# OpenBMB/VisRAG

Hardware: AMD Instinct MI355X
Metric: page-images embedded/sec (VisRAG-Ret encode, 448x448, bf16 MFMA) + queries/sec@top-10 over 100k-page index (higher is better)
Workload: dtype bf16; 1 GPU; VisRAG-Ret (SigLIP-so400m 26 blk + resampler + MiniCPM-2B 40 layers) bf16 encode batch=32 page images 448x448 per GPU; index 100000 rows x 2304 sharded 1 way(s), 1000 queries top-10; batch_per_gpu=32, global_batch=32, parallelism=dp1 (pages sharded, no data-path collective)

## Files before the change

### visrag_amd/csrc/common.h

```cpp
#pragma once
#include <hip/hip_runtime.h>
#include <stdint.h>

typedef __bf16 bf16_t;
typedef __bf16 bf16x2 __attribute__((ext_vector_type(2)));
typedef __bf16 bf16x4 __attribute__((ext_vector_type(4)));
typedef __bf16 bf16x8 __attribute__((ext_vector_type(8)));
typedef float f32x2 __attribute__((ext_vector_type(2)));
typedef float f32x4 __attribute__((ext_vector_type(4)));
typedef uint32_t u32x4 __attribute__((ext_vector_type(4)));
typedef uint32_t u32x2 __attribute__((ext_vector_type(2)));

#define VR_WAVE 64

#define VR_LDS(p) ((__attribute__((address_space(3))) void*)(p))
#define VR_GLOBAL(p) ((const __attribute__((address_space(1))) void*)(p))

__device__ __forceinline__ float bf2f(bf16_t v) { return (float)v; }
__device__ __forceinline__ bf16_t f2bf(float v) { return (bf16_t)v; }

__device__ __forceinline__ float wave_sum(float v) {
#pragma unroll
    for (int o = 32; o > 0; o >>= 1) v += __shfl_xor(v, o, 64);
    return v;
}
__device__ __forceinline__ float wave_max(float v) {
#pragma unroll
    for (int o = 32; o > 0; o >>= 1) v = fmaxf(v, __shfl_xor(v, o, 64));
    return v;
}

__device__ __forceinline__ int xcd_remap(int bid, int nwg) {
    const int xcd = bid & 7, q = nwg >> 3, r = nwg & 7;
    const int base = (xcd < r) ? xcd * (q + 1) : r * (q + 1) + (xcd - r) * q;
    return base + (bid >> 3);
}

inline void set_max_dynamic_lds(const void* fn, int bytes, unsigned long long& done) {
    int dev = 0;
    if (hipGetDevice(&dev) != hipSuccess || dev < 0 || dev > 63) dev = 0;
    if (!((done >> dev) & 1ull)) {
        (void)hipFuncSetAttribute(fn, hipFuncAttributeMaxDynamicSharedMemorySize, bytes);
        done |= 1ull << dev;
    }
}
inline int device_cu_count() {
    static int cu_of[64] = {0};
    int dev = 0;
    if (hipGetDevice(&dev) != hipSuccess || dev < 0 || dev >= 64) dev = 0;
    if (!cu_of[dev]) {
        hipDeviceProp_t prop;
        cu_of[dev] = hipGetDeviceProperties(&prop, dev) == hipSuccess && prop.multiProcessorCount > 0 ? prop.multiProcessorCount : 256;
    }
    return cu_of[dev];
}
#define VR_WAIT_VM_BARRIER(N) asm volatile("s_waitcnt vmcnt(" #N ")\n\ts_barrier" ::: "memory")
```

### visrag_amd/csrc/encode.hip

```cpp
#include <hip/hip_runtime.h>

#include <algorithm>
#include <cmath>
#include <cstring>
#include <vector>

#include "model.h"

static int run_vision_group(vr_model_s* m, const uint8_t* const* dev_imgs_hostarray, int n, int H, int W,
                            const int32_t* rowmap_host , bool first_group, hipStream_t s) {
    const vr_config_t& c = m->c;
    const int P = c.patch_size, gh = H / P, gw = W / P, N = gh * gw;
    const int D = m->D, Dp = m->Dp, E = m->E, Q = m->Q;
    const int M = n * N;
    GridTables* g = nullptr;
    VRCHK(get_grid(m, gh, gw, &g));

    HIPCHK(hipMemcpyAsync(m->w_imgptr.p, dev_imgs_hostarray, (size_t)n * 8, hipMemcpyHostToDevice, s));
    int* cu = (int*)arena_take(m, (size_t)2 * (n + 1) * 4);
    for (int i = 0; i <= n; ++i) { cu[i] = i * N; cu[n + 1 + i] = i * Q; }
    HIPCHK(hipMemcpyAsync(m->w_cu.p, cu, (size_t)2 * (n + 1) * 4, hipMemcpyHostToDevice, s));
    HIPCHK(hipMemcpyAsync(m->w_rowmap.p, rowmap_host, (size_t)n * Q * 4, hipMemcpyHostToDevice, s));
    const int* cu_tok = m->w_cu.as<int>();
    const int* cu_qry = m->w_cu.as<int>() + (n + 1);

    float* h = m->w_hvit.as<float>();
    {
        GemmArgs a = gemm_args(nullptr, 0, m->patch, M, h, Dp);
        a.rowbias = g->vit_pos.as<float>(); a.rowbias_period = N; a.rowbias_ld = Dp; a.rowbias_cols = Dp;
        HIPCHK(launch_patch_embed((const uint8_t* const*)m->w_imgptr.p, n, H, W, P, a, m->Kpe, s));
    }
    if (first_group) VRCHK(tap_store(m, "vit_embed", h, N, D, Dp, false, s));
    const int ldqkv = pad128(3 * D);
    const int vit_hd = c.vit_dim / c.vit_heads;
    const int vit_qscale_n = D % 64 == 0 ? D : 0;
    const float vit_qscale = (1.0f / sqrtf((float)vit_hd)) * 1.44269504088896340736f;
    for (int l = 0; l < c.vit_depth; ++l) {
        const VitBlock& b = m->blocks[l];
        HIPCHK(launch_layernorm(h, M, D, Dp, b.n1w.v.as<float>(), b.n1b.v.as<float>(), c.vit_ln_eps, m->w_xn.p, Dp, s));
        VRCHK(prof_begin(m, VR_PROF_VIT_QKV, s));
        {
            GemmArgs a = gemm_args(m->w_xn.p, Dp, b.qkv, M, m->w_qkv.p, ldqkv);
            a.col_scale = vit_qscale; a.col_scale_n = vit_qscale_n;
            HIPCHK(launch_gemm(a, EPI_BF16, GEMM_VARIANT_AUTO, s));
        }
        VRCHK(prof_end(m, VR_PROF_VIT_QKV, 2.0 * M * D * 3 * D, s));
        {
            AttnArgs a{};
            a.q = m->w_qkv.p; a.ldq = ldqkv;
            a.k = (const char*)m->w_qkv.p + (size_t)D * 2; a.ldk = ldqkv;
            a.v = (const char*)m->w_qkv.p + (size_t)2 * D * 2; a.ldv = ldqkv;
            a.out = m->w_att.p; a.ldo = Dp; a.cu_q = cu_tok; a.cu_kv = cu_tok; a.B = n; a.heads = c.vit_heads;
            a.head_dim = vit_hd; a.max_q = N; a.causal = 0; a.q_shared = 0; a.scale = 1.0f / sqrtf((float)vit_hd); a.q_prescaled = vit_qscale_n > 0;
            VRCHK(prof_begin(m, VR_PROF_VIT_ATTN, s));
            HIPCHK(launch_attention(a, s));
            VRCHK(prof_end(m, VR_PROF_VIT_ATTN, 4.0 * n * (double)N * N * D, s));
        }
        VRCHK(prof_begin(m, VR_PROF_VIT_PROJ, s));
        {
            GemmArgs a = gemm_args(m->w_att.p, Dp, b.proj, M, h, Dp); a.resid = h;
            HIPCHK(launch_gemm(a, EPI_RESID, GEMM_VARIANT_AUTO, s));
        }
        VRCHK(prof_end(m, VR_PROF_VIT_PROJ, 2.0 * M * D * D, s));
        HIPCHK(launch_layernorm(h, M, D, Dp, b.n2w.v.as<float>(), b.n2b.v.as<float>(), c.vit_ln_eps, m->w_xn.p, Dp, s));
        VRCHK(prof_begin(m, VR_PROF_VIT_FC1, s));
        { GemmArgs a = gemm_args(m->w_xn.p, Dp, b.fc1, M, m->w_mlp.p, m->Fp); HIPCHK(launch_gemm(a, EPI_GELU, GEMM_VARIANT_AUTO, s)); }
        VRCHK(prof_end(m, VR_PROF_VIT_FC1, 2.0 * M * D * m->F, s));
        VRCHK(prof_begin(m, VR_PROF_VIT_FC2, s));
        {
            GemmArgs a = gemm_args(m->w_mlp.p, m->Fp, b.fc2, M, h, Dp); a.resid = h;
            HIPCHK(launch_gemm(a, EPI_RESID, GEMM_VARIANT_AUTO, s));
        }
        VRCHK(prof_end(m, VR_PROF_VIT_FC2, 2.0 * M * D * m->F, s));
        if (l == 0 && first_group) VRCHK(tap_store(m, "vit_block0", h, N, D, Dp, false, s));
    }
    HIPCHK(launch_layernorm(h, M, D, Dp, m->vit_nw.v.as<float>(), m->vit_nb.v.as<float>(), c.vit_ln_eps, m->w_xn.p, Dp, s));
    if (first_group) VRCHK(tap_store(m, "vit_out", m->w_xn.p, N, D, Dp, true, s));

    VRCHK(prof_begin(m, VR_PROF_RESAMPLER, s));
    { GemmArgs a = gemm_args(m->w_xn.p, Dp, m->r_kvproj, M, m->w_kv32.p, E); HIPCHK(launch_gemm(a, EPI_F32, GEMM_VARIANT_AUTO, s)); }
    HIPCHK(launch_layernorm(m->w_kv32.as<float>(), M, E, E, m->r_lnkv_w.v.as<float>(), m->r_lnkv_b.v.as<float>(),
                            c.resampler_ln_eps, m->w_xkv.p, E, s));
    {
        GemmArgs a = gemm_args(m->w_xkv.p, E, m->r_kv, M, m->w_KV.p, 2 * E);
        a.rowbias = g->pos_k.as<float>(); a.rowbias_period = N; a.rowbias_ld = E; a.rowbias_cols = E;
        HIPCHK(launch_gemm(a, EPI_BF16, GEMM_VARIANT_AUTO, s));
    }
    {
        AttnArgs a{};
        a.q = m->r_q.p; a.ldq = E; a.k = m->w_KV.p; a.ldk = 2 * E; a.v = (const char*)m->w_KV.p + (size_t)E * 2; a.ldv = 2 * E;
        a.out = m->w_ratt.p; a.ldo = E; a.cu_q = cu_qry; a.cu_kv = cu_tok; a.B = n; a.heads = E / 128; a.head_dim = 128;
        a.max_q = Q; a.causal = 0; a.q_shared = 1; a.scale = 1.0f / sqrtf(128.0f);
        HIPCHK(launch_attention(a, s));
    }
    const int R = n * Q;
    { GemmArgs a = gemm_args(m->w_ratt.p, E, m->r_out, R, m->w_rout.p, E); HIPCHK(launch_gemm(a, EPI_F32, GEMM_VARIANT_AUTO, s)); }
    HIPCHK(launch_layernorm(m->w_rout.as<float>(), R, E, E, m->r_lnpost_w.v.as<float>(), m->r_lnpost_b.v.as<float>(),
                            c.resampler_ln_eps, m->w_rln.p, E, s));
    if (first_group && m->taps_on) {
        GemmArgs a = gemm_args(m->w_rln.p, E, m->r_proj, Q, m->w_rout.p, E);
        HIPCHK(launch_gemm(a, EPI_F32, GEMM_VARIANT_AUTO, s));
        VRCHK(tap_store(m, "resampler_out", m->w_rout.p, Q, E, E, false, s));
    }
    {
        GemmArgs a = gemm_args(m->w_rln.p, E, m->r_proj, R, m->w_h.p, E);
        a.rowmap = m->w_rowmap.as<int>();
        HIPCHK(launch_gemm(a, EPI_F32, GEMM_VARIANT_AUTO, s));
    }
    VRCHK(prof_end(m, VR_PROF_RESAMPLER, 2.0 * M * D * E + 4.0 * M * E * (double)E + 4.0 * R * (double)N * E + 4.0 * R * E * (double)E, s));
    return VR_OK;
}

static int hp_gemm_tiles(vr_model_s* m, const void* a_hi, const void* a_lo, const Linear& L, const Linear& Llo, int lda, int T, float* out,
                         int ldo, bool into_resid, float alpha, hipStream_t s) {
    const size_t plane = (size_t)T * L.n_pad;
    const int n_planes = Llo.has_w ? 3 : 2;
    if (!L.has_b && (const char*)a_lo == (const char*)a_hi + (size_t)T * lda * 2 && m->w_hp_planes.reserve((size_t)n_planes * plane * 4) == VR_OK) {
        float* part = m->w_hp_planes.as<float>();
        {
            GemmArgs a = gemm_args(a_hi, lda, L, 2 * T, part, L.n_pad);
            a.bias = nullptr;
            HIPCHK(launch_gemm(a, EPI_F32, GEMM_VARIANT_AUTO, s));
        }
        if (Llo.has_w) {
            GemmArgs a = gemm_args(a_hi, lda, Llo, T, part + 2 * plane, L.n_pad);
            a.bias = nullptr;
            HIPCHK(launch_gemm(a, EPI_F32, GEMM_VARIANT_AUTO, s));
        }
        HIPCHK(launch_planes_sum(part, n_planes, plane, L.n_pad, T, std::min(L.n_pad, ldo), out, ldo, into_resid ? alpha : 1.0f, into_resid, s));
        return VR_OK;
    }
    {
        GemmArgs a = gemm_args(a_hi, lda, L, T, out, ldo);
        if (into_resid) { a.resid = out; a.alpha = alpha; }
        HIPCHK(launch_gemm(a, into_resid ? EPI_RESID : EPI_F32, GEMM_VARIANT_AUTO, s));
    }
    {
        GemmArgs a = gemm_args(a_lo, lda, L, T, out, ldo);
        a.bias = nullptr;
        a.resid = out; a.alpha = into_resid ? alpha : 1.0f;
        HIPCHK(launch_gemm(a, EPI_RESID, GEMM_VARIANT_AUTO, s));
    }
    if (Llo.has_w) {
        GemmArgs a = gemm_args(a_hi, lda, Llo, T, out, ldo);
        a.bias = nullptr;
        a.resid = out; a.alpha = into_resid ? alpha : 1.0f;
        HIPCHK(launch_gemm(a, EPI_RESID, GEMM_VARIANT_AUTO, s));
    }
    return VR_OK;
}

static int hp_gemm_stream(vr_model_s* m, const void* a_hi, const void* a_lo, const Linear& L, const Linear& Llo, int lda, int T, float* out,
                          int ldo, bool into_resid, float alpha, hipStream_t s) {
    const int ks = stream_ksplit(L.n_pad, L.k_pad);
    const size_t plane = (size_t)T * L.n_pad;
    const int n_pass = Llo.has_w ? 3 : 2;
    if ((size_t)n_pass * ks * plane * 4 > m->w_hp_part.bytes) return fail(VR_ERR_CAPACITY, "split-K planes exceed the workspace");
    float* part = m->w_hp_part.as<float>();
    for (int pass = 0; pass < n_pass; ++pass) {
        GemmArgs a = gemm_args(pass == 1 ? a_lo : a_hi, lda, pass == 2 ? Llo : L, T, part + (size_t)pass * ks * plane, L.n_pad);
        a.bias = nullptr;
        a.ksplit = ks; a.split_stride = plane;
        HIPCHK(launch_gemm_skinny(a, s));
    }
    HIPCHK(launch_planes_sum(part, n_pass * ks, plane, L.n_pad, T, std::min(L.n_pad, ldo), out, ldo, into_resid ? alpha : 1.0f, into_resid, s));
    return VR_OK;
}
static bool hp_stream_ok(const vr_model_s* m, int T) {
    if (T > 32) return false;
    for (const DecLayer& L : m->layers)
        for (const Linear* l : {&L.qkv, &L.o, &L.gu, &L.down})
            if (l->n_pad % 256 || l->k_pad % 64 || l->has_b) return false;
    return true;
}

static int run_decoder_hp(vr_model_s* m, int T, int B, int max_len, hipStream_t s) {
    (void)max_len;
    const vr_config_t& c = m->c;
    const int E = m->E, I = m->I, Ip = m->Ip;
    float* h = m->w_h.as<float>();
    float* qkv = m->w_hp_qkv.as<float>();
    float* att = m->w_hp_att.as<float>();
    float* gu = m->w_hp_gu.as<float>();
    const int ld_gu = pad128(2 * I);
    HIPCHK(launch_seq_of(m->w_seq.as<int>(), B, m->w_seqof.as<int>(), s));
    const bool stream = hp_stream_ok(m, T);
    void* const hi = m->w_hp_hi.p;
    auto lo = [&](int lda) -> void* { return (char*)hi + (size_t)T * lda * 2; };
    auto hp_gemm = [&](vr_model_s* mm, const Linear& L, const Linear& Llo, int lda, int TT, float* out, int ldo, bool into_resid,
                       float alpha, hipStream_t ss) -> int {
        return stream ? hp_gemm_stream(mm, hi, lo(lda), L, Llo, lda, TT, out, ldo, into_resid, alpha, ss)
                      : hp_gemm_tiles(mm, hi, lo(lda), L, Llo, lda, TT, out, ldo, into_resid, alpha, ss);
    };
    for (int l = 0; l < c.num_layers; ++l) {
        const DecLayer& L = m->layers[l];
        HIPCHK(launch_rmsnorm_split(h, T, E, L.ln1.v.as<float>(), c.rms_norm_eps, hi, lo(E), s));
        VRCHK(hp_gemm(m, L.qkv, L.qkv_lo, E, T, qkv, 3 * E, false, 1.0f, s));
        HIPCHK(launch_rope_f32(qkv, T, 3 * E, 2 * E, m->w_pos.as<int>(), m->rope.as<float>(), s));
        HIPCHK(launch_attn_f32(qkv, 3 * E, E, m->w_seqof.as<int>(), m->w_seq.as<int>(), T, c.num_heads, 1.0f / sqrtf(64.0f), att, s));
        HIPCHK(launch_split_bf16(att, hi, lo(E), (size_t)T * E, s));
        VRCHK(hp_gemm(m, L.o, L.o_lo, E, T, h, E, true, c.residual_scale, s));
        HIPCHK(launch_rmsnorm_split(h, T, E, L.ln2.v.as<float>(), c.rms_norm_eps, hi, lo(E), s));
        VRCHK(hp_gemm(m, L.gu, L.gu_lo, E, T, gu, ld_gu, false, 1.0f, s));
        HIPCHK(launch_swiglu_split(gu, T, ld_gu, I, Ip, hi, lo(Ip), s));
        VRCHK(hp_gemm(m, L.down, L.down_lo, Ip, T, h, E, true, c.residual_scale, s));
        if (l == 0) VRCHK(tap_store(m, "dec_layer0", h, T, E, E, false, s));
    }
    return VR_OK;
}


struct DecRoute { int ks; int proj_variant; bool proj_128w; };
static DecRoute dec_route(int T, int E, int Ip, bool taps_on) {
    DecRoute r{1, GEMM_VARIANT_256W, false};
    const long t192 = (long)((T + 255) / 256) * (E / 192);
    if (E % 192 == 0 && t192 * 2 <= 256 && t192 * 2 > 160 && E % 128 == 0 && Ip % 128 == 0) {
        r.ks = 2;
        r.proj_variant = GEMM_VARIANT_192W;
    } else {
        const long tiles = (long)((T + 255) / 256) * ((E + 255) / 256);
        for (int cand = DEC_KSPLIT_MAX; cand > 1; --cand)
            if (tiles * cand <= 256 && E % (cand * 64) == 0 && Ip % (cand * 64) == 0) { r.ks = cand; break; }
    }
    if (taps_on) r.ks = 1;
    const long t128 = (long)((T + 127) / 128) * (E / 192);
    r.proj_128w = E % 192 == 0 && t128 > 128 && t128 <= 256;
    if (r.proj_128w) r.ks = 1;
    return r;
}

extern "C" int vr_encode(vr_model_t m, const uint8_t* const* slices, const int32_t* slice_hw, int32_t n_slices,
                         int32_t slices_on_device, const int32_t* input_ids, const int32_t* seq_offsets, int32_t B,
                         const int32_t* vision_rows, float* out_reps, int32_t out_on_device, void* stream) {
    if (!m) return fail(VR_ERR_INVALID, "NULL model");
    m->arena_open = false;
    const int rc = encode_impl(m, slices, slice_hw, n_slices, slices_on_device, input_ids, seq_offsets, B, vision_rows,
                               out_reps, out_on_device, stream);
    arena_close(m, stream);
    return rc;
}

extern "C" int vr_encode_hidden(vr_model_t m, const uint8_t* const* slices, const int32_t* slice_hw, int32_t n_slices,
                                int32_t slices_on_device, const int32_t* input_ids, const int32_t* seq_offsets, int32_t B,
                                const int32_t* vision_rows, float* out_reps, int32_t out_on_device, float* out_hidden,
                                int32_t hidden_len, void* stream) {
    if (!m) return fail(VR_ERR_INVALID, "NULL model");
    if (!out_hidden || hidden_len <= 0) return fail(VR_ERR_INVALID, "out_hidden is NULL or hidden_len <= 0");
    m->arena_open = false;
    const int rc = encode_impl(m, slices, slice_hw, n_slices, slices_on_device, input_ids, seq_offsets, B, vision_rows,
                               out_reps, out_on_device, stream, out_hidden, hidden_len);
    arena_close(m, stream);
    return rc;
}

int encode_impl(vr_model_t m, const uint8_t* const* slices, const int32_t* slice_hw, int32_t n_slices,
                int32_t slices_on_device, const int32_t* input_ids, const int32_t* seq_offsets, int32_t B,
                const int32_t* vision_rows, float* out_reps, int32_t out_on_device, void* stream,
                float* out_hidden, int32_t hidden_len, const EncodeHook* hook) {
    if (!m->finalized) return fail(VR_ERR_STATE, "vr_model_finalize() has not succeeded");
    if (B <= 0 || !input_ids || !seq_offsets || !out_reps) return fail(VR_ERR_INVALID, "empty batch or NULL argument");
    if (n_slices > 0 && (!slices || !slice_hw || !vision_rows)) return fail(VR_ERR_INVALID, "NULL slice arguments");
    VRCHK(set_dev(m->device));
    hipStream_t s = (hipStream_t)stream;
    const vr_config_t& c = m->c;
    const int E = m->E, Q = m->Q;
    const int T = seq_offsets[B];
    if (seq_offsets[0] != 0) return fail(VR_ERR_INVALID, "seq_offsets[0] must be 0");
    if (B > c.max_seqs) return fail(VR_ERR_CAPACITY, "B=%d exceeds max_seqs=%d", B, c.max_seqs);
    if (T > c.max_tokens) return fail(VR_ERR_CAPACITY, "T=%d tokens exceed max_tokens=%d", T, c.max_tokens);
    for (int i = 0; i < B; ++i)
        if (seq_offsets[i + 1] <= seq_offsets[i]) return fail(VR_ERR_INVALID, "empty sequence %d", i);
    for (int t = 0; t < T; ++t)
        if (input_ids[t] < 0 || input_ids[t] >= c.vocab_size) return fail(VR_ERR_INVALID, "token id %d out of range at %d", input_ids[t], t);
    for (int i = 0; i < n_slices * Q; ++i)
        if (vision_rows[i] >= T) return fail(VR_ERR_INVALID, "vision row %d out of range", vision_rows[i]);

    VRCHK(arena_begin(m, (size_t)T * 4 + (size_t)(B + 1) * 4 + (size_t)n_slices * (Q * 4 + 8 + 64 * 3) + 4096));
    {
        int* a_ids = (int*)arena_take(m, (size_t)T * 4);
        int* a_seq = (int*)arena_take(m, (size_t)(B + 1) * 4);
        memcpy(a_ids, input_ids, (size_t)T * 4);
        memcpy(a_seq, seq_offsets, (size_t)(B + 1) * 4);
        HIPCHK(hipMemcpyAsync(m->w_ids.p, a_ids, (size_t)T * 4, hipMemcpyHostToDevice, s));
        HIPCHK(hipMemcpyAsync(m->w_seq.p, a_seq, (size_t)(B + 1) * 4, hipMemcpyHostToDevice, s));
    }
    int max_len = 0;
    for (int i = 0; i < B; ++i) max_len = std::max(max_len, seq_offsets[i + 1] - seq_offsets[i]);
    const bool hp = n_slices == 0 && c.text_split_precision != 0 && (c.text_split_precision == 1 || max_len <= c.text_split_precision) &&
                    !(hook && hook->bf16_route);
    if (hp && m->has_embed_lo)
        HIPCHK(launch_embed_gather_hp(m->w_ids.as<int>(), T, m->embed.p, m->embed_lo.p, E, c.scale_emb, m->w_h.as<float>(), s));
    else
        HIPCHK(launch_embed_gather(m->w_ids.as<int>(), T, m->embed.p, E, c.scale_emb, m->w_h.as<float>(), s));
    HIPCHK(launch_iota_pos(m->w_seq.as<int>(), B, m->w_pos.as<int>(), s));

    if (n_slices > 0) {
        size_t pix_total = 0;
        std::vector<size_t> pix_off(n_slices);
        for (int i = 0; i < n_slices; ++i) {
            const int H = slice_hw[2 * i], W = slice_hw[2 * i + 1];
            if (H <= 0 || W <= 0 || H % c.patch_size || W % c.patch_size)
                return fail(VR_ERR_INVALID, "slice %d: %dx%d is not a multiple of the patch size", i, H, W);
            if ((H / c.patch_size) * (W / c.patch_size) > c.max_patches)
                return fail(VR_ERR_CAPACITY, "slice %d has more than max_patches=%d patches", i, c.max_patches);
            pix_off[i] = pix_total;
            pix_total += ((size_t)H * W * 3 + 15) / 16 * 16;
        }
        std::vector<const uint8_t*> dev_ptr(n_slices);
        if (slices_on_device) {
            for (int i = 0; i < n_slices; ++i) dev_ptr[i] = slices[i];
        } else {
            if (m->w_pix.bytes < pix_total) VRCHK(m->w_pix.alloc(pix_total));
            for (int i = 0; i < n_slices; ++i) {
                const size_t nb = (size_t)slice_hw[2 * i] * slice_hw[2 * i + 1] * 3;
                HIPCHK(hipMemcpyAsync((char*)m->w_pix.p + pix_off[i], slices[i], nb, hipMemcpyHostToDevice, s));
                dev_ptr[i] = (const uint8_t*)m->w_pix.p + pix_off[i];
            }
        }
        std::vector<char> done(n_slices, 0);
        bool first = true;
        for (int i = 0; i < n_slices; ++i) {
            if (done[i]) continue;
            const int H = slice_hw[2 * i], W = slice_hw[2 * i + 1];
            const int N = (H / c.patch_size) * (W / c.patch_size);
            std::vector<int> idx;
            for (int j = i; j < n_slices; ++j)
                if (!done[j] && slice_hw[2 * j] == H && slice_hw[2 * j + 1] == W) { idx.push_back(j); done[j] = 1; }
            const int per_pass = std::max(1, (int)std::min<int64_t>(c.max_images, ((int64_t)c.max_images * c.max_patches) / N));
            for (size_t lo = 0; lo < idx.size(); lo += per_pass) {
                const int n = (int)std::min<size_t>(per_pass, idx.size() - lo);
                const uint8_t** ptrs = (const uint8_t**)arena_take(m, (size_t)n * 8);
                int32_t* rowmap = (int32_t*)arena_take(m, (size_t)n * Q * 4);
                for (int k = 0; k < n; ++k) {
                    ptrs[k] = dev_ptr[idx[lo + k]];
                    memcpy(rowmap + (size_t)k * Q, vision_rows + (size_t)idx[lo + k] * Q, (size_t)Q * 4);
                }
                VRCHK(run_vision_group(m, ptrs, n, H, W, rowmap, first, s));
                first = false;
            }
        }
    }
    VRCHK(tap_store(m, "inputs_embeds", m->w_h.p, T, E, E, false, s));

    float* h = m->w_h.as<float>();
    const int* seq = m->w_seq.as<int>();
    if (max_len > m->rope_len) return fail(VR_ERR_CAPACITY, "sequence of %d tokens exceeds the RoPE table", max_len);
    VRCHK(prof_begin(m, VR_PROF_DECODER, s));
    if (hp) {
        VRCHK(run_decoder_hp(m, T, B, max_len, s));
    } else {
    const DecRoute route = dec_route(T, E, m->Ip, m->taps_on);
    const int ks = route.ks;
    const size_t pstride = (size_t)T * E;
    float* part = m->w_part.as<float>();
    bool pend = false;
    auto proj = [&](const void* A, int lda, const Linear& L) -> int {
        if (route.proj_128w) {
            GemmArgs a = gemm_args(A, lda, L, T, h, E); a.resid = h; a.alpha = c.residual_scale;
            if (gemm128w_fits(a, 192)) { HIPCHK(launch_gemm(a, EPI_RESID, GEMM_VARIANT_128W_192, s)); return VR_OK; }
        }
        if (ks > 1) {
            GemmArgs a = gemm_args(A, lda, L, T, part, E);
            a.ksplit = ks; a.split_stride = pstride;
            HIPCHK(launch_gemm(a, EPI_F32, gemm256w_fits(a, route.proj_variant == GEMM_VARIANT_192W ? 192 : 256) ? route.proj_variant : GEMM_VARIANT_256IL, s));
            pend = true;
        } else {
            GemmArgs a = gemm_args(A, lda, L, T, h, E); a.resid = h; a.alpha = c.residual_scale;
            HIPCHK(launch_gemm(a, EPI_RESID, GEMM_VARIANT_AUTO, s));
        }
        return VR_OK;
    };
    auto norm = [&](const float* w) -> int {
        VRCHK(prof_begin(m, VR_PROF_DEC_NORM, s));
        struct End { vr_model_s* m; hipStream_t s; ~End() { (void)prof_end(m, VR_PROF_DEC_NORM, 0.0, s); } } end_{m, s};
        if (pend) {
            HIPCHK(launch_rmsnorm_accum(h, T, E, E, part, ks, pstride, E, c.residual_scale, w, c.rms_norm_eps, m->w_dxn.p, E, s));
            pend = false;
        } else {
            HIPCHK(launch_rmsnorm(h, T, E, E, w, c.rms_norm_eps, m->w_dxn.p, E, s));
        }
        return VR_OK;
    };
    double attn_flops = 0;
    for (int i = 0; i < B; ++i) { const double Li = seq_offsets[i + 1] - seq_offsets[i]; attn_flops += 4.0 * Li * Li * E; }
    for (int l = 0; l < c.num_layers; ++l) {
        const DecLayer& L = m->layers[l];
        VRCHK(norm(L.ln1.v.as<float>()));
        {
            GemmArgs a = gemm_args(m->w_dxn.p, E, L.qkv, T, m->w_dqkv.p, 3 * E);
            a.rope_pos = m->w_pos.as<int>(); a.rope_table = m->rope.as<float>(); a.rope_cols = 2 * E;
            VRCHK(prof_begin(m, VR_PROF_DEC_QKV, s));
            HIPCHK(launch_gemm(a, EPI_ROPE, GEMM_VARIANT_AUTO, s));
            VRCHK(prof_end(m, VR_PROF_DEC_QKV, 6.0 * T * (double)E * E, s));
        }
        if (hook && hook->layer) VRCHK(hook->layer(hook->ctx, l, m->w_dqkv.p, 3 * E, T, s));
        {
            VRCHK(prof_begin(m, VR_PROF_DEC_ATTN, s));
            AttnArgs a{};
            a.q = m->w_dqkv.p; a.ldq = 3 * E; a.k = (const char*)m->w_dqkv.p + (size_t)E * 2; a.ldk = 3 * E;
            a.v = (const char*)m->w_dqkv.p + (size_t)2 * E * 2; a.ldv = 3 * E;
            a.out = m->w_datt.p; a.ldo = E; a.cu_q = seq; a.cu_kv = seq; a.B = B; a.heads = c.num_heads; a.head_dim = 64;
            a.max_q = max_len; a.causal = 1; a.q_shared = 0; a.scale = 1.0f / sqrtf(64.0f);
            HIPCHK(launch_attention(a, s));
            VRCHK(prof_end(m, VR_PROF_DEC_ATTN, attn_flops, s));
        }
        VRCHK(prof_begin(m, VR_PROF_DEC_O, s));
        VRCHK(proj(m->w_datt.p, E, L.o));
        VRCHK(prof_end(m, VR_PROF_DEC_O, 2.0 * T * (double)E * E, s));
        VRCHK(norm(L.ln2.v.as<float>()));
        VRCHK(prof_begin(m, VR_PROF_DEC_GU, s));
        {
            GemmArgs a = gemm_args(m->w_dxn.p, E, L.gu, T, m->w_dact.p, m->Ip);
            HIPCHK(launch_gemm(a, EPI_SWIGLU, GEMM_VARIANT_AUTO, s));
        }
        VRCHK(prof_end(m, VR_PROF_DEC_GU, 4.0 * T * (double)E * m->I, s));
        VRCHK(prof_begin(m, VR_PROF_DEC_DOWN, s));
        VRCHK(proj(m->w_dact.p, m->Ip, L.down));
        VRCHK(prof_end(m, VR_PROF_DEC_DOWN, 2.0 * T * (double)E * m->I, s));
        if (l == 0) VRCHK(tap_store(m, "dec_layer0", h, T, E, E, false, s));
    }
    if (pend) {
        HIPCHK(launch_rmsnorm_accum(h, T, E, E, part, ks, pstride, E, c.residual_scale, nullptr, c.rms_norm_eps, nullptr, 0, s));
        pend = false;
    }
    }
    {
        double fl = 0;
        for (int i = 0; i < B; ++i) { const double Li = seq_offsets[i + 1] - seq_offsets[i]; fl += 4.0 * Li * Li * E; }
        fl = c.num_layers * (fl + (double)T * (8.0 * E * E + 6.0 * (double)E * m->I));
        VRCHK(prof_end(m, VR_PROF_DECODER, fl, s));
    }
    float* tap_hidden = nullptr;
    if (m->taps_on && (size_t)T * E * 4 <= m->w_kv32.bytes) tap_hidden = m->w_kv32.as<float>();
    if (out_hidden) {
        if (max_len > hidden_len) return fail(VR_ERR_INVALID, "hidden_len=%d is shorter than the longest sequence (%d)", hidden_len, max_len);
        if (!tap_hidden) {
            if ((size_t)T * E * 4 <= m->w_kv32.bytes) tap_hidden = m->w_kv32.as<float>();
            else { VRCHK(m->w_hidden.reserve((size_t)T * E * 4)); tap_hidden = m->w_hidden.as<float>(); }
        }
    }
    float* dst = out_on_device ? out_reps : m->w_out.as<float>();
    HIPCHK(launch_pool(h, seq, B, E, m->final_norm.v.as<float>(), c.rms_norm_eps, dst, tap_hidden, s, m->pool_mode));
    if (tap_hidden && m->taps_on) VRCHK(tap_store(m, "last_hidden", tap_hidden, T, E, E, false, s));
    if (out_hidden) {
        HIPCHK(hipMemsetAsync(out_hidden, 0, (size_t)B * hidden_len * E * 4, s));
        for (int i = 0; i < B; ++i)
            HIPCHK(hipMemcpyAsync(out_hidden + (size_t)i * hidden_len * E, tap_hidden + (size_t)seq_offsets[i] * E,
                                  (size_t)(seq_offsets[i + 1] - seq_offsets[i]) * E * 4, hipMemcpyDeviceToDevice, s));
    }
    if (!out_on_device) HIPCHK(hipMemcpyAsync(out_reps, dst, (size_t)B * E * 4, hipMemcpyDeviceToHost, s));
    if (!out_on_device || (n_slices > 0 && !slices_on_device)) HIPCHK(hipStreamSynchronize(s));
    return VR_OK;
}
```

### visrag_amd/csrc/engine_common.h

```cpp
#pragma once
#include <hip/hip_runtime.h>

#include <cstdarg>
#include <cstdio>
#include <initializer_list>
#include <string>
#include <vector>

#include "../../include/visrag_hip.h"
#include "kernels.h"
#include "pack.h"

using namespace vr;

inline thread_local std::string g_err;

static inline int fail(int code, const char* fmt, ...) {
    char buf[1024];
    va_list ap;
    va_start(ap, fmt);
    vsnprintf(buf, sizeof(buf), fmt, ap);
    va_end(ap);
    g_err = buf;
    return code;
}

#define HIPCHK(expr)                                                                         \
    do {                                                                                     \
        hipError_t e_ = (expr);                                                              \
        if (e_ != hipSuccess)                                                                \
            return fail(VR_ERR_HIP, "%s failed: %s (%s:%d)", #expr, hipGetErrorString(e_),   \
                        __FILE__, __LINE__);                                                 \
    } while (0)
#define VRCHK(expr)            \
    do {                       \
        int r_ = (expr);       \
        if (r_ != VR_OK) return r_; \
    } while (0)

static inline int skinny_ksplit(int n, int k, int max_split) {
    const int tiles = (n + 255) / 256, nk = k / 64;
    int best = 1;
    for (int d = 2; d <= max_split && tiles * d <= 256; ++d) {
        const int per = (nk + d - 1) / d;
        if (per >= 4 && (d - 1) * per < nk) best = d;
    }
    return best;
}
static inline int stream_ksplit(int n, int k) { return skinny_ksplit(n, k, 32); }

static inline int pad128(int x) { return (x + 127) / 128 * 128; }
static inline int64_t pad128l(int64_t x) { return (x + 127) / 128 * 128; }
static inline int pad256(int x) { return (x + 255) / 256 * 256; }
static inline int64_t pad256l(int64_t x) { return (x + 255) / 256 * 256; }

struct DevBuf {
    void* p = nullptr;
    size_t bytes = 0;
    bool owned = true;
    DevBuf() = default;
    DevBuf(const DevBuf& o) : p(o.p), bytes(o.bytes), owned(false) {}
    DevBuf& operator=(const DevBuf& o) {
        if (this != &o) { free(); p = o.p; bytes = o.bytes; owned = false; }
        return *this;
    }
    DevBuf(DevBuf&& o) noexcept : p(o.p), bytes(o.bytes), owned(o.owned) { o.p = nullptr; o.bytes = 0; o.owned = true; }
    DevBuf& operator=(DevBuf&& o) noexcept {
        if (this != &o) { free(); p = o.p; bytes = o.bytes; owned = o.owned; o.p = nullptr; o.bytes = 0; o.owned = true; }
        return *this;
    }
    ~DevBuf() { free(); }
    int alloc(size_t n) {
        free();
        if (n == 0) n = 16;
        hipError_t e = hipMalloc(&p, n);
        if (e != hipSuccess) { p = nullptr; return fail(VR_ERR_HIP, "hipMalloc(%zu) failed: %s", n, hipGetErrorString(e)); }
        bytes = n;
        e = hipMemset(p, 0, n);
        if (e != hipSuccess) return fail(VR_ERR_HIP, "hipMemset failed: %s", hipGetErrorString(e));
        e = hipStreamSynchronize(nullptr);
        if (e != hipSuccess) return fail(VR_ERR_HIP, "hipStreamSynchronize failed: %s", hipGetErrorString(e));
        return VR_OK;
    }
    int reserve(size_t n) {
        if (p && owned && bytes >= n) return VR_OK;
        free();
        if (n == 0) n = 16;
        hipError_t e = hipMalloc(&p, n);
        if (e != hipSuccess) { p = nullptr; return fail(VR_ERR_HIP, "hipMalloc(%zu) failed: %s", n, hipGetErrorString(e)); }
        bytes = n;
        return VR_OK;
    }
    void free() {
        if (p && owned) (void)hipFree(p);
        p = nullptr;
        bytes = 0;
        owned = true;
    }
    template <typename T> T* as() const { return reinterpret_cast<T*>(p); }
};

struct Linear {
    DevBuf w, b;
    int n = 0, k = 0, n_pad = 0, k_pad = 0;
    bool has_w = false, has_b = false;
};
struct Vec { DevBuf v; bool ok = false; };


static inline int set_dev(int dev) {
    HIPCHK(hipSetDevice(dev));
    return VR_OK;
}


struct Staged { const void* dev = nullptr; DevBuf tmp; };

static inline int stage(const void* data, size_t bytes, int on_device, Staged& st) {
    if (on_device) { st.dev = data; return VR_OK; }
    VRCHK(st.tmp.alloc(bytes));
    HIPCHK(hipMemcpy(st.tmp.p, data, bytes, hipMemcpyHostToDevice));
    st.dev = st.tmp.p;
    return VR_OK;
}

static inline int load_linear_part(Linear& L, int n_total, int k, const void* dev_src, int is_bf16, int rows, int src_ld,
                            int transpose, int blk, int blk_stride, int blk_off, int lo_part = 0) {
    if (!L.w.p) {
        L.n = n_total; L.k = k; L.n_pad = pad128(n_total); L.k_pad = pad128(k);
        VRCHK(L.w.alloc((size_t)pad256(n_total) * L.k_pad * 2));
    } else if (L.n != n_total || L.k != k) {
        return fail(VR_ERR_INVALID, "inconsistent shapes for a packed weight");
    }
    HIPCHK(launch_pack_weight(dev_src, is_bf16, rows, k, src_ld, transpose, L.w.p, L.k_pad, blk, blk_stride, blk_off, 0, lo_part));
    HIPCHK(hipDeviceSynchronize());
    L.has_w = true;
    return VR_OK;
}

static inline int load_bias_part(Linear& L, int n_total, const void* dev_src, int is_bf16, int rows, int off) {
    if (!L.b.p) VRCHK(L.b.alloc((size_t)pad256(n_total) * 4));
    HIPCHK(launch_to_f32(dev_src, is_bf16, L.b.as<float>() + off, rows, 0));
    HIPCHK(hipDeviceSynchronize());
    L.has_b = true;
    return VR_OK;
}

static inline int load_vec(Vec& v, const void* dev_src, int is_bf16, int n, int n_alloc) {
    VRCHK(v.v.alloc((size_t)n_alloc * 4));
    HIPCHK(launch_to_f32(dev_src, is_bf16, v.v.as<float>(), n, 0));
    HIPCHK(hipDeviceSynchronize());
    v.ok = true;
    return VR_OK;
}

static inline int to_host_f32(const void* dev_src, int is_bf16, size_t n, std::vector<float>& out) {
    DevBuf t;
    VRCHK(t.alloc(n * 4));
    HIPCHK(launch_to_f32(dev_src, is_bf16, t.as<float>(), n, 0));
    out.resize(n);
    HIPCHK(hipMemcpy(out.data(), t.p, n * 4, hipMemcpyDeviceToHost));
    t.free();
    return VR_OK;
}

static inline bool shape_is(const int64_t* s, int nd, std::initializer_list<int64_t> want) {
    if (nd != (int)want.size()) return false;
    int i = 0;
    for (int64_t w : want) if (s[i++] != w) return false;
    return true;
}
```

### visrag_amd/csrc/hp_text.hip

```cpp
#include "common.h"
#include "kernels.h"

namespace vr {

constexpr int HP_MAXV = 10;

__device__ __forceinline__ void split_store4(const f32x4 y, bf16_t* hi, bf16_t* lo) {
    bf16x4 h, l;
#pragma unroll
    for (int r = 0; r < 4; ++r) {
        h[r] = f2bf(y[r]);
        l[r] = f2bf(y[r] - bf2f(h[r]));
    }
    *reinterpret_cast<bf16x4*>(hi) = h;
    *reinterpret_cast<bf16x4*>(lo) = l;
}

__global__ __launch_bounds__(256) void rmsnorm_split_kernel(const float* __restrict__ x, int rows, int dim,
                                                            const float* __restrict__ w, float eps,
                                                            bf16_t* __restrict__ hi, bf16_t* __restrict__ lo) {
    const int lane = threadIdx.x & 63;
    const int row = blockIdx.x * 4 + (threadIdx.x >> 6);
    if (row >= rows) return;
    const int nv = dim >> 2;
    const f32x4* xr = reinterpret_cast<const f32x4*>(x + (size_t)row * dim);
    f32x4 v[HP_MAXV];
    float s = 0.f;
#pragma unroll
    for (int i = 0; i < HP_MAXV; ++i) {
        const int c = lane + i * 64;
        v[i] = (c < nv) ? xr[c] : f32x4{0.f, 0.f, 0.f, 0.f};
        s += v[i][0] * v[i][0] + v[i][1] * v[i][1] + v[i][2] * v[i][2] + v[i][3] * v[i][3];
    }
    s = wave_sum(s);
    const float rstd = rsqrtf(s / dim + eps);
#pragma unroll
    for (int i = 0; i < HP_MAXV; ++i) {
        const int c = lane + i * 64;
        if (c < nv) {
            const f32x4 y = v[i] * rstd * reinterpret_cast<const f32x4*>(w)[c];
            split_store4(y, hi + (size_t)row * dim + c * 4, lo + (size_t)row * dim + c * 4);
        }
    }
}

hipError_t launch_rmsnorm_split(const float* x, int rows, int dim, const float* w, float eps, void* hi, void* lo, hipStream_t s) {
    if (rows <= 0) return hipSuccess;
    if (dim % 4 || dim > 64 * 4 * HP_MAXV) return hipErrorInvalidValue;
    hipLaunchKernelGGL(rmsnorm_split_kernel, dim3((rows + 3) / 4), dim3(256), 0, s, x, rows, dim, w, eps, (bf16_t*)hi, (bf16_t*)lo);
    return hipGetLastError();
}

__global__ __launch_bounds__(256) void rope_f32_kernel(float* __restrict__ qkv, int T, int ld, int rope_cols,
                                                       const int* __restrict__ pos, const float* __restrict__ table) {
    const int t = blockIdx.x;
    const float* tab = table + (size_t)pos[t] * 64;
    float* row = qkv + (size_t)t * ld;
    for (int i = threadIdx.x; i < rope_cols / 2; i += 256) {
        const int head = i >> 5, c = i & 31;
        float* p = row + head * 64 + c;
        const float x1 = p[0], x2 = p[32], cs = tab[c], sn = tab[32 + c];
        p[0] = x1 * cs - x2 * sn;
        p[32] = x2 * cs + x1 * sn;
    }
}

hipError_t launch_rope_f32(float* qkv, int T, int ld, int rope_cols, const int* pos, const float* table, hipStream_t s) {
    if (T <= 0) return hipSuccess;
    if (rope_cols % 64) return hipErrorInvalidValue;
    hipLaunchKernelGGL(rope_f32_kernel, dim3(T), dim3(256), 0, s, qkv, T, ld, rope_cols, pos, table);
    return hipGetLastError();
}

__global__ __launch_bounds__(256) void attn_f32_kernel(const float* __restrict__ qkv, int ld, int E,
                                                       const int* __restrict__ seq_of, const int* __restrict__ seq_offsets,
                                                       int T, int heads, float scale, float* __restrict__ out) {
    const int lane = threadIdx.x & 63;
    const int w = blockIdx.x * 4 + (threadIdx.x >> 6);
    if (w >= T * heads) return;
    const int t = w / heads, h = w % heads;
    const int t0 = seq_offsets[seq_of[t]];
    const int n_keys = t - t0 + 1;
    const float* qrow = qkv + (size_t)t * ld + h * 64;
    f32x4 q[16];
#pragma unroll
    for (int i = 0; i < 16; ++i) q[i] = reinterpret_cast<const f32x4*>(qrow)[i];
    float m = -INFINITY, l = 0.f, acc = 0.f;
    for (int j0 = 0; j0 < n_keys; j0 += 64) {
        const int j = j0 + lane;
        float sc = -INFINITY;
        if (j < n_keys) {
            const f32x4* kr = reinterpret_cast<const f32x4*>(qkv + (size_t)(t0 + j) * ld + E + h * 64);
            float a = 0.f;
#pragma unroll
            for (int i = 0; i < 16; ++i) {
                const f32x4 kv = kr[i];
                a += q[i][0] * kv[0] + q[i][1] * kv[1] + q[i][2] * kv[2] + q[i][3] * kv[3];
            }
            sc = a * scale;
        }
        const float mn = fmaxf(m, wave_max(sc));
        const float p = (j < n_keys) ? expf(sc - mn) : 0.f;
        const float corr = expf(m - mn);
        l = l * corr + wave_sum(p);
        acc *= corr;
        const int nj = min(64, n_keys - j0);
        const float* vbase = qkv + (size_t)(t0 + j0) * ld + 2 * E + h * 64 + lane;
        for (int jj = 0; jj < nj; ++jj) acc += __shfl(p, jj, 64) * vbase[(size_t)jj * ld];
        m = mn;
    }
    out[(size_t)t * E + h * 64 + lane] = acc / l;
}

hipError_t launch_attn_f32(const float* qkv, int ld, int E, const int* seq_of, const int* seq_offsets, int T, int heads,
                           float scale, float* out, hipStream_t s) {
    if (T <= 0) return hipSuccess;
    if (E != heads * 64) return hipErrorInvalidValue;
    const long waves = (long)T * heads;
    hipLaunchKernelGGL(attn_f32_kernel, dim3((unsigned)((waves + 3) / 4)), dim3(256), 0, s, qkv, ld, E, seq_of, seq_offsets, T,
                       heads, scale, out);
    return hipGetLastError();
}

__global__ __launch_bounds__(256) void swiglu_split_kernel(const float* __restrict__ gu, int ld_gu, int I, int ld_act,
                                                           bf16_t* __restrict__ hi, bf16_t* __restrict__ lo) {
    const int t = blockIdx.x;
    const float* row = gu + (size_t)t * ld_gu;
    for (int c4 = threadIdx.x; c4 < ld_act / 4; c4 += 256) {
        const int c = c4 * 4;
        f32x4 y = {0.f, 0.f, 0.f, 0.f};
        if (c < I) {
            const int blk = c >> 4, o = c & 15;
            const f32x4 g = *reinterpret_cast<const f32x4*>(row + blk * 32 + o);
            const f32x4 u = *reinterpret_cast<const f32x4*>(row + blk * 32 + 16 + o);
#pragma unroll
            for (int r = 0; r < 4; ++r) y[r] = g[r] / (1.0f + expf(-g[r])) * u[r];
        }
        split_store4(y, hi + (size_t)t * ld_act + c, lo + (size_t)t * ld_act + c);
    }
}

hipError_t launch_swiglu_split(const float* gu, int T, int ld_gu, int I, int ld_act, void* hi, void* lo, hipStream_t s) {
    if (T <= 0) return hipSuccess;
    if (I % 16 || ld_act % 4 || ld_act < I) return hipErrorInvalidValue;
    hipLaunchKernelGGL(swiglu_split_kernel, dim3(T), dim3(256), 0, s, gu, ld_gu, I, ld_act, (bf16_t*)hi, (bf16_t*)lo);
    return hipGetLastError();
}

__global__ __launch_bounds__(256) void embed_gather_hp_kernel(const int* __restrict__ ids, const bf16_t* __restrict__ table_hi,
                                                              const bf16_t* __restrict__ table_lo, int dim, float scale,
                                                              float* __restrict__ out) {
    const int t = blockIdx.x;
    const size_t off = (size_t)ids[t] * dim;
    float* dst = out + (size_t)t * dim;
    for (int c = threadIdx.x * 4; c < dim; c += 1024) {
        const bf16x4 a = *reinterpret_cast<const bf16x4*>(table_hi + off + c);
        const bf16x4 b = *reinterpret_cast<const bf16x4*>(table_lo + off + c);
        f32x4 o;
#pragma unroll
        for (int r = 0; r < 4; ++r) o[r] = (bf2f(a[r]) + bf2f(b[r])) * scale;
        *reinterpret_cast<f32x4*>(dst + c) = o;
    }
}

hipError_t launch_embed_gather_hp(const int* ids, int T, const void* table_hi, const void* table_lo, int dim, float scale,
                                  float* out, hipStream_t s) {
    if (T <= 0) return hipSuccess;
    if (dim % 4) return hipErrorInvalidValue;
    hipLaunchKernelGGL(embed_gather_hp_kernel, dim3(T), dim3(256), 0, s, ids, (const bf16_t*)table_hi, (const bf16_t*)table_lo,
                       dim, scale, out);
    return hipGetLastError();
}

__global__ void seq_of_kernel(const int* __restrict__ seq_offsets, int* __restrict__ seq_of) {
    const int b = blockIdx.x;
    for (int t = seq_offsets[b] + threadIdx.x; t < seq_offsets[b + 1]; t += blockDim.x) seq_of[t] = b;
}

hipError_t launch_seq_of(const int* seq_offsets, int B, int* seq_of, hipStream_t s) {
    if (B <= 0) return hipSuccess;
    hipLaunchKernelGGL(seq_of_kernel, dim3(B), dim3(256), 0, s, seq_offsets, seq_of);
    return hipGetLastError();
}

__global__ __launch_bounds__(256) void planes_sum_kernel(const float* __restrict__ parts, int n_parts, size_t stride, int ldp, int N,
                                                         float* __restrict__ out, int ldo, float alpha, int accumulate) {
    const int t = blockIdx.y;
    const int n = (blockIdx.x * 256 + threadIdx.x) * 4;
    if (n >= N) return;
    const float* p0 = parts + (size_t)t * ldp + n;
    f32x4 a = *reinterpret_cast<const f32x4*>(p0);
    for (int p = 1; p < n_parts; ++p) a += *reinterpret_cast<const f32x4*>(p0 + (size_t)p * stride);
    float* o = out + (size_t)t * ldo + n;
    f32x4 r = a * alpha;
    if (accumulate) r += *reinterpret_cast<const f32x4*>(o);
    *reinterpret_cast<f32x4*>(o) = r;
}

hipError_t launch_planes_sum(const float* parts, int n_parts, size_t stride, int ldp, int T, int N, float* out, int ldo, float alpha,
                             bool accumulate, hipStream_t s) {
    if (T <= 0 || n_parts <= 0) return hipSuccess;
    if (N % 4 || ldp % 4 || ldo % 4) return hipErrorInvalidValue;
    hipLaunchKernelGGL(planes_sum_kernel, dim3((N / 4 + 255) / 256, T), dim3(256), 0, s, parts, n_parts, stride, ldp, N, out, ldo, alpha,
                       accumulate ? 1 : 0);
    return hipGetLastError();
}

}
```

### visrag_amd/csrc/index.hip

```cpp
#include <hip/hip_runtime.h>

#include <algorithm>
#include <cmath>
#include <vector>

#include "engine_common.h"

constexpr int CERT_WORDS = 32, CERT_FLAG = 2, CERT_FLAG2 = 3, CERT_STATS = 4, CERT_NSTATS = 6;
struct vr_index_s {
    int device = 0, dim = 0;
    int64_t cap = 0, n = 0;
    DevBuf f32, bf16;
    DevBuf q32, qbf, cs, ci, ck, os, oi, ok, thr, sbuf;
    int64_t qcap = 0, ccap = 0, kcap = 0;
    DevBuf cert, flags, flagq;
    int64_t fcap = 0;
    int* huge_seen = nullptr;
    float eps_rel = -2.f;
    bool prof_on = false;
    hipEvent_t prof_ev[SEARCH_PROF_EVENTS] = {};
    double prof_ms[SEARCH_PROF_EVENTS - 1] = {};
    int64_t prof_calls = 0;
};

extern "C" int vr_index_create(int device_id, int32_t dim, int64_t capacity, vr_index_t* out) {
    if (!out || dim <= 0 || capacity <= 0) return fail(VR_ERR_INVALID, "bad index arguments");
    if (dim % 64 || dim > 2560) return fail(VR_ERR_INVALID, "dim %d must be a multiple of 64 and <= 2560", dim);
    if (capacity >= ((int64_t)1 << 31) - 256) return fail(VR_ERR_INVALID, "capacity too large for 32-bit row ids");
    VRCHK(set_dev(device_id));
    vr_index_s* ix = new vr_index_s();
    ix->device = device_id; ix->dim = dim; ix->cap = capacity;
    const int64_t cp = pad256l(capacity);
    int r = ix->f32.alloc((size_t)cp * dim * 4);
    if (r == VR_OK) r = ix->bf16.alloc((size_t)cp * dim * 2);
    if (r == VR_OK) r = ix->cert.alloc(CERT_WORDS * 4);
    if (r == VR_OK && hipHostMalloc((void**)&ix->huge_seen, 64, hipHostMallocDefault) != hipSuccess) r = fail(VR_ERR_HIP, "hipHostMalloc");
    if (r != VR_OK) { ix->f32.free(); ix->bf16.free(); ix->cert.free(); delete ix; return r; }
    *ix->huge_seen = 0;
    *out = ix;
    return VR_OK;
}

extern "C" int vr_index_destroy(vr_index_t ix) {
    if (!ix) return VR_OK;
    (void)hipSetDevice(ix->device);
    (void)hipDeviceSynchronize();
    for (DevBuf* b : {&ix->f32, &ix->bf16, &ix->q32, &ix->qbf, &ix->cs, &ix->ci, &ix->ck, &ix->os, &ix->oi, &ix->ok, &ix->thr,
                      &ix->sbuf, &ix->cert, &ix->flags, &ix->flagq})
        b->free();
    for (hipEvent_t e : ix->prof_ev) if (e) (void)hipEventDestroy(e);
    if (ix->huge_seen) (void)hipHostFree(ix->huge_seen);
    delete ix;
    return VR_OK;
}

extern "C" int vr_index_reset(vr_index_t ix) {
    if (!ix) return fail(VR_ERR_INVALID, "NULL index");
    VRCHK(set_dev(ix->device));
    HIPCHK(hipDeviceSynchronize());
    HIPCHK(hipMemset(ix->cert.p, 0, 8));
    ix->n = 0;
    if (ix->huge_seen) *ix->huge_seen = 0;
    return VR_OK;
}

extern "C" int vr_index_size(vr_index_t ix, int64_t* n) {
    if (!ix || !n) return fail(VR_ERR_INVALID, "NULL argument");
    *n = ix->n;
    return VR_OK;
}

extern "C" int vr_index_add(vr_index_t ix, const float* reps, int64_t n, int32_t on_device, void* stream) {
    if (!ix || (!reps && n > 0) || n < 0) return fail(VR_ERR_INVALID, "bad arguments");
    if (n == 0) return VR_OK;
    if (ix->n + n > ix->cap) return fail(VR_ERR_CAPACITY, "index capacity %lld exceeded", (long long)ix->cap);
    VRCHK(set_dev(ix->device));
    hipStream_t s = (hipStream_t)stream;
    float* dst = ix->f32.as<float>() + (size_t)ix->n * ix->dim;
    HIPCHK(hipMemcpyAsync(dst, reps, (size_t)n * ix->dim * 4, on_device ? hipMemcpyDeviceToDevice : hipMemcpyHostToDevice, s));
    HIPCHK(launch_f32_to_bf16(dst, (char*)ix->bf16.p + (size_t)ix->n * ix->dim * 2, (size_t)n * ix->dim, s));
    HIPCHK(launch_row_norm_max(dst, n, ix->dim, ix->cert.as<float>(), s));
    if (!on_device) HIPCHK(hipStreamSynchronize(s));
    ix->n += n;
    return VR_OK;
}

extern "C" int vr_index_set_search_eps(vr_index_t ix, float eps_rel) {
    if (!ix) return fail(VR_ERR_INVALID, "NULL index");
    if (eps_rel != eps_rel) ix->eps_rel = -2.f;
    else ix->eps_rel = eps_rel < 0.f ? -1.f : eps_rel;
    return VR_OK;
}

extern "C" int vr_index_search_stats(vr_index_t ix, int64_t* out6, int32_t reset) {
    if (!ix || !out6) return fail(VR_ERR_INVALID, "NULL argument");
    VRCHK(set_dev(ix->device));
    HIPCHK(hipDeviceSynchronize());
    unsigned w[CERT_NSTATS];
    HIPCHK(hipMemcpy(w, ix->cert.as<unsigned>() + CERT_STATS, CERT_NSTATS * 4, hipMemcpyDeviceToHost));
    for (int i = 0; i < CERT_NSTATS; ++i) out6[i] = w[i];
    if (reset) HIPCHK(hipMemset(ix->cert.as<unsigned>() + CERT_STATS, 0, CERT_NSTATS * 4));
    return VR_OK;
}

struct SearchPlan { bool stream; int own, sweep, n_chunks, tiles_per_chunk; };
static SearchPlan search_plan(int64_t n_docs, int nq, int dim) {
    SearchPlan p{};
    p.stream = search_uses_stream(nq, dim);
    p.own = p.stream ? 0 : search_prepass_owned(n_docs, nq, dim);
    p.sweep = p.stream ? search_stream_chunks() : search_num_chunks(n_docs - (p.own ? (int64_t)SEARCH_PRE_SPOTS * 256 : 0), nq);
    p.n_chunks = p.sweep + p.own;
    const int64_t tile = search_uses_256(nq) ? 256 : 128;
    const int64_t tiles = (n_docs + tile - 1) / tile - (p.own ? SEARCH_PRE_SPOTS : 0);
    p.tiles_per_chunk = p.stream ? 0 : (int)((tiles + p.sweep - 1) / p.sweep);
    return p;
}

extern "C" int vr_index_search_plan(vr_index_t ix, int32_t nq, int32_t* out5) {
    if (!ix || !out5 || nq <= 0) return fail(VR_ERR_INVALID, "bad arguments");
    const SearchPlan p = search_plan(ix->n, nq, ix->dim);
    out5[0] = p.n_chunks; out5[1] = p.own; out5[2] = p.sweep; out5[3] = p.tiles_per_chunk;
    out5[4] = (ix->huge_seen && __atomic_load_n(ix->huge_seen, __ATOMIC_RELAXED) != 0) ? 1 : 0;
    return VR_OK;
}

extern "C" int vr_index_error_model(vr_index_t ix, float* out4) {
    if (!ix || !out4) return fail(VR_ERR_INVALID, "NULL argument");
    VRCHK(set_dev(ix->device));
    HIPCHK(hipDeviceSynchronize());
    HIPCHK(hipMemcpy(out4, ix->cert.p, 8, hipMemcpyDeviceToHost));
    out4[2] = search_acc_rel(ix->dim);
    out4[3] = search_default_eps_rel(ix->dim);
    return VR_OK;
}

extern "C" int vr_index_set_search_profile(vr_index_t ix, int32_t enable) {
    if (!ix) return fail(VR_ERR_INVALID, "NULL index");
    VRCHK(set_dev(ix->device));
    if (enable)
        for (hipEvent_t& e : ix->prof_ev) if (!e) HIPCHK(hipEventCreate(&e));
    ix->prof_on = enable != 0;
    for (double& m : ix->prof_ms) m = 0;
    ix->prof_calls = 0;
    return VR_OK;
}

extern "C" int vr_index_get_search_profile(vr_index_t ix, double* ms5, int64_t* calls) {
    if (!ix || !ms5 || !calls) return fail(VR_ERR_INVALID, "NULL argument");
    for (int i = 0; i < SEARCH_PROF_EVENTS - 1; ++i) ms5[i] = ix->prof_ms[i];
    *calls = ix->prof_calls;
    return VR_OK;
}

static int search_impl(vr_index_t ix, const float* queries, int32_t nq, int32_t k, float* out_scores, int64_t* out_ids,
                       unsigned long long* out_keys, int64_t id_offset, int32_t on_device, void* stream) {
    const bool keys_out = out_keys != nullptr;
    if (!ix || !queries || nq <= 0 || (!keys_out && (!out_scores || !out_ids))) return fail(VR_ERR_INVALID, "bad arguments");
    const bool bigk = k > 26;
    if (k <= 0 || k > search_bigk_max()) return fail(VR_ERR_INVALID, "k=%d unsupported (1..%d)", k, search_bigk_max());
    if (keys_out && (id_offset < 0 || id_offset + ix->n >= ((int64_t)1 << 32) - 1))
        return fail(VR_ERR_INVALID, "id_offset %lld + %lld rows do not fit 32-bit global ids", (long long)id_offset, (long long)ix->n);
    const int kp = bigk ? 0 : search_kprime(k);
    VRCHK(set_dev(ix->device));
    hipStream_t s = (hipStream_t)stream;
    const int dim = ix->dim;
    const int64_t ldS = pad256l(std::max<int64_t>(ix->n, 1));
    int64_t qblk = bigk ? 256 : 4096;
    const int64_t nqp = pad256l(std::min<int64_t>(nq, qblk));
    const int64_t slots = bigk ? 256 : std::min<int64_t>(nqp, std::max<int64_t>(16, (((int64_t)1 << 27) / ldS) / 16 * 16));
    if (ix->qcap < nqp) {
        VRCHK(ix->qbf.alloc((size_t)nqp * dim * 2));
        VRCHK(ix->thr.alloc((size_t)nqp * 8));
        ix->qcap = nqp;
    }
    const float* q32 = queries;
    if (!on_device) {
        VRCHK(ix->q32.reserve((size_t)nq * dim * 4));
        HIPCHK(hipMemcpyAsync(ix->q32.p, queries, (size_t)nq * dim * 4, hipMemcpyHostToDevice, s));
        q32 = ix->q32.as<float>();
    }
    float* os = out_scores; int64_t* oi = out_ids; unsigned long long* ok = out_keys;
    if (!on_device) {
        if (keys_out) { VRCHK(ix->ok.reserve((size_t)nq * k * 8)); ok = ix->ok.as<unsigned long long>(); }
        else {
            VRCHK(ix->os.reserve((size_t)nq * k * 4));
            VRCHK(ix->oi.reserve((size_t)nq * k * 8));
            os = ix->os.as<float>(); oi = ix->oi.as<int64_t>();
        }
    }
    if (ix->n == 0) {
        if (keys_out) HIPCHK(hipMemsetAsync(ok, 0, (size_t)nq * k * 8, s));
        else {
            std::vector<float> sc((size_t)nq * k, -INFINITY);
            std::vector<int64_t> id((size_t)nq * k, -1);
            HIPCHK(hipMemcpyAsync(os, sc.data(), sc.size() * 4, hipMemcpyHostToDevice, s));
            HIPCHK(hipMemcpyAsync(oi, id.data(), id.size() * 8, hipMemcpyHostToDevice, s));
            HIPCHK(hipStreamSynchronize(s));
        }
    } else {
        if (ix->fcap < nqp) {
            VRCHK(ix->flags.alloc((size_t)nqp * 12));
            VRCHK(ix->flagq.alloc((size_t)(nqp + 256) * dim * 2));
            ix->fcap = nqp;
        }
        VRCHK(ix->sbuf.reserve((size_t)slots * ldS * 4));
        for (int64_t q0 = 0; q0 < nq; q0 += qblk) {
            const int nb = (int)std::min<int64_t>(qblk, nq - q0);
            const int64_t nbp = pad256l(nb);
            const bool prof = ix->prof_on && !bigk;
            if (prof) HIPCHK(hipEventRecord(ix->prof_ev[0], s));
            const bool conv_in_kernel = !bigk && search_uses_stream(nb, dim);
            if (!conv_in_kernel)
                HIPCHK(launch_f32_to_bf16_pad(q32 + (size_t)q0 * dim, ix->qbf.p, (size_t)nb * dim, (size_t)nbp * dim, s,
                                              ix->cert.as<int>() + CERT_FLAG));
            if (prof) HIPCHK(hipEventRecord(ix->prof_ev[1], s));
            SearchArgs a{};
            a.index_bf16 = ix->bf16.p; a.index_f32 = ix->f32.as<float>(); a.n_docs = ix->n; a.dim = dim;
            a.q_bf16 = ix->qbf.p; a.q_f32 = q32 + (size_t)q0 * dim; a.nq = nb; a.k = k;
            a.convert_q = conv_in_kernel ? 1 : 0;
            if (conv_in_kernel) { a.score_rows = ix->sbuf.as<float>(); a.ld_scores = (size_t)ldS; }
            const bool huge_seen = ix->huge_seen && __atomic_load_n(ix->huge_seen, __ATOMIC_RELAXED) != 0;
            const bool exact_small = conv_in_kernel && huge_seen;
            const bool exact_big = !conv_in_kernel && (bigk || huge_seen || !ix->huge_seen);
            a.exact_follows = (exact_small || exact_big) ? 1 : 0;
            a.huge_seen = ix->huge_seen;
            a.eps_data = ix->eps_rel == -2.f ? 1 : 0;
            a.eps_rel = a.eps_data ? 0.f : ix->eps_rel;
            a.acc_rel = search_acc_rel(dim);
            a.dmax = ix->cert.as<float>();
            a.flag_count = ix->cert.as<int>() + CERT_FLAG; a.flag_list = ix->flags.as<int>();
            a.flag2_count = ix->cert.as<int>() + CERT_FLAG2; a.flag2_list = ix->flags.as<int>() + ix->fcap;
            a.flag_tau = ix->flags.as<float>() + 2 * ix->fcap; a.flag_q = ix->flagq.p;
            a.stats = ix->cert.as<unsigned>() + CERT_STATS;
            if (keys_out) { a.out_keys = ok + (size_t)q0 * k; a.id_offset = id_offset; }
            else { a.out_scores = os + (size_t)q0 * k; a.out_ids = oi + (size_t)q0 * k; }
            a.prof_ev = prof ? ix->prof_ev : nullptr;
            if (bigk) {
                GemmArgs g{};
                g.A = ix->qbf.p; g.lda = dim;
                g.W = ix->bf16.p; g.ldw = dim; g.M = nb; g.N = (int)pad128l(ix->n); g.K = dim;
                g.out = ix->sbuf.p; g.ldo = (int)ldS; g.alpha = 1.0f;
                HIPCHK(launch_gemm(g, EPI_F32, GEMM_VARIANT_AUTO, s));
                HIPCHK(launch_search_bigk(a, ix->sbuf.as<float>(), (size_t)ldS, 0, nb, s));
            } else {
                const SearchPlan plan = search_plan(ix->n, nb, dim);
                a.pre_own_chunks = plan.own;
                a.n_chunks = plan.n_chunks;
                a.thr_init = ix->thr.as<float>();
                a.thr_cert = ix->thr.as<float>() + ix->qcap;
                const int64_t need = std::max<int64_t>(nbp * a.n_chunks * kp, nbp * search_prepass_floats());
                if (ix->ccap < need) {
                    VRCHK(ix->cs.alloc((size_t)need * 4));
                    VRCHK(ix->ci.alloc((size_t)need * 4));
                    ix->ccap = need;
                }
                a.cand_scores = ix->cs.as<float>(); a.cand_ids = ix->ci.as<int>();
                if (search_uses_256(nb)) {
                    const int64_t kneed = nbp * a.n_chunks * 128;
                    if (ix->kcap < kneed) { VRCHK(ix->ck.alloc((size_t)kneed * 8)); ix->kcap = kneed; }
                    a.cand_keys = ix->ck.as<unsigned long long>();
                }
                HIPCHK(launch_search(a, s));
            }
            if (prof) HIPCHK(hipEventRecord(ix->prof_ev[4], s));
            if ((a.eps_data || a.eps_rel >= 0.f) && !a.score_rows) {
                for (int64_t f0 = 0; f0 < nb; f0 += slots) {
                    const int ns = (int)std::min<int64_t>(slots, nb - f0);
                    GemmArgs g{};
                    g.A = (const char*)ix->flagq.p + (size_t)f0 * dim * 2; g.lda = dim;
                    g.W = ix->bf16.p; g.ldw = dim; g.M = ns; g.N = (int)pad128l(ix->n); g.K = dim;
                    g.out = ix->sbuf.p; g.ldo = (int)ldS; g.alpha = 1.0f;
                    g.m_dev = a.flag_count; g.m_sub = (int)f0;
                    HIPCHK(launch_gemm(g, EPI_F32, GEMM_VARIANT_256IL, s));
                    HIPCHK(launch_band_select(a, ix->sbuf.as<float>(), (size_t)ldS, (int)f0, ns, s));
                }
                SearchArgs ax = a;
                ax.flag_count = a.flag2_count; ax.flag_list = a.flag2_list;
                for (int64_t f0 = 0; exact_big && f0 < nb; f0 += slots) {
                    const int ns = (int)std::min<int64_t>(slots, nb - f0);
                    HIPCHK(launch_exact_scores(a.index_f32, a.n_docs, dim, a.q_f32, ax.flag_list, ax.flag_count, (int)f0, ns,
                                               ix->sbuf.as<float>(), (size_t)ldS, s));
                    HIPCHK(launch_exact_select(ax, ix->sbuf.as<float>(), (size_t)ldS, (int)f0, ns, s));
                }
            }
            if ((a.eps_data || a.eps_rel >= 0.f) && a.score_rows && exact_small) {
                SearchArgs ax = a;
                ax.flag_count = a.flag2_count; ax.flag_list = a.flag2_list;
                HIPCHK(launch_exact_scores(a.index_f32, a.n_docs, dim, a.q_f32, ax.flag_list, ax.flag_count, 0, nb, ix->sbuf.as<float>(), (size_t)ldS, s));
                HIPCHK(launch_exact_select(ax, ix->sbuf.as<float>(), (size_t)ldS, 0, nb, s));
            }
            if (prof) {
                HIPCHK(hipEventRecord(ix->prof_ev[5], s));
                HIPCHK(hipEventSynchronize(ix->prof_ev[5]));
                for (int i = 0; i + 1 < SEARCH_PROF_EVENTS; ++i) {
                    float ms = 0.f;
                    HIPCHK(hipEventElapsedTime(&ms, ix->prof_ev[i], ix->prof_ev[i + 1]));
                    ix->prof_ms[i] += ms;
                }
                ix->prof_calls += 1;
            }
        }
    }
    if (!on_device) {
        if (keys_out) HIPCHK(hipMemcpyAsync(out_keys, ok, (size_t)nq * k * 8, hipMemcpyDeviceToHost, s));
        else {
            HIPCHK(hipMemcpyAsync(out_scores, os, (size_t)nq * k * 4, hipMemcpyDeviceToHost, s));
            HIPCHK(hipMemcpyAsync(out_ids, oi, (size_t)nq * k * 8, hipMemcpyDeviceToHost, s));
        }
        HIPCHK(hipStreamSynchronize(s));
    }
    return VR_OK;
}

extern "C" int vr_index_search(vr_index_t ix, const float* queries, int32_t nq, int32_t k, float* out_scores,
                               int64_t* out_ids, int32_t on_device, void* stream) {
    return search_impl(ix, queries, nq, k, out_scores, out_ids, nullptr, 0, on_device, stream);
}

extern "C" int vr_index_search_keys(vr_index_t ix, const float* queries, int32_t nq, int32_t k, int64_t id_offset,
                                    uint64_t* out_keys, int32_t on_device, void* stream) {
    if (!out_keys) return fail(VR_ERR_INVALID, "out_keys is NULL");
    return search_impl(ix, queries, nq, k, nullptr, nullptr, (unsigned long long*)out_keys, id_offset, on_device, stream);
}

extern "C" int vr_topk_merge(int device_id, const float* scores, const int64_t* ids, int32_t n_parts, int32_t nq,
                             int32_t k, float* out_scores, int64_t* out_ids, void* stream) {
    if (!scores || !ids || !out_scores || !out_ids || n_parts <= 0 || nq <= 0) return fail(VR_ERR_INVALID, "bad arguments");
    VRCHK(set_dev(device_id));
    HIPCHK(launch_topk_merge(scores, ids, n_parts, nq, k, out_scores, out_ids, (hipStream_t)stream));
    return VR_OK;
}

extern "C" int vr_topk_merge_keys(int device_id, const uint64_t* keys, int32_t n_parts, int32_t nq, int32_t k,
                                  float* out_scores, int64_t* out_ids, void* stream) {
    if (!keys || !out_scores || !out_ids || n_parts <= 0 || nq <= 0) return fail(VR_ERR_INVALID, "bad arguments");
    VRCHK(set_dev(device_id));
    HIPCHK(launch_topk_merge_keys((const unsigned long long*)keys, n_parts, nq, k, out_scores, out_ids, (hipStream_t)stream));
    return VR_OK;
}
```

### visrag_amd/csrc/kernels.h

```cpp
#pragma once
#include <hip/hip_runtime.h>
#include <stdint.h>

namespace vr {

enum GemmEpilogue { EPI_BF16 = 0, EPI_GELU = 1, EPI_F32 = 2, EPI_RESID = 3, EPI_SWIGLU = 4, EPI_ROPE = 5 };
enum GemmVariant { GEMM_VARIANT_GLDS = 0, GEMM_VARIANT_AUTO = 3, GEMM_VARIANT_192 = 7, GEMM_VARIANT_256IL = 9, GEMM_VARIANT_256W = 12,
                   GEMM_VARIANT_192W = 13, GEMM_VARIANT_128W_192 = 14, GEMM_VARIANT_128W_256 = 15 };

struct GemmArgs {
    const void* A; int lda;
    const void* W; int ldw;
    int M, N, K;
    const float* bias;
    const float* resid;
    float alpha;
    void* out; int ldo;
    const int* rowmap;
    const float* rowbias;
    int rowbias_period, rowbias_ld, rowbias_cols;
    const int* rope_pos;
    const float* rope_table;
    int rope_cols;
    int raster_gm;
    int ksplit;
    size_t split_stride;
    float col_scale; int col_scale_n;
    const int* m_dev; int m_sub;
};
hipError_t launch_gemm(const GemmArgs& a, int epilogue, int variant, hipStream_t s);
hipError_t launch_gemm192(const GemmArgs& a, int epilogue, hipStream_t s);
hipError_t launch_gemm256w(const GemmArgs& a, int epilogue, hipStream_t s);
bool gemm256w_fits(const GemmArgs& a, int tile_cols);
hipError_t launch_gemm192w(const GemmArgs& a, int epilogue, hipStream_t s);
hipError_t launch_gemm128w(const GemmArgs& a, int epilogue, int tile_cols, hipStream_t s);
bool gemm128w_fits(const GemmArgs& a, int tile_cols);

struct SkinnyCombine { const void* part; const float* lse; int S; int heads; int group; const int* S_dev; };
hipError_t launch_gemm_skinny(const GemmArgs& a, hipStream_t s, bool swiglu = false, const struct SkinnyCombine* combine = nullptr);
hipError_t launch_swiglu_sum(const float* parts, int n_parts, size_t plane_stride, int ldp, int M, int I, void* act, int lda,
                             hipStream_t s);

hipError_t launch_layernorm(const float* x, int rows, int dim, int ldx, const float* w, const float* b,
                            float eps, void* out, int ldo, hipStream_t s);
hipError_t launch_rmsnorm_accum(float* x, int rows, int dim, int ldx, const float* partial, int nsplit,
                                size_t split_stride, int ldp, float alpha, const float* w, float eps, void* out,
                                int ldo, hipStream_t s);
hipError_t launch_rmsnorm(const float* x, int rows, int dim, int ldx, const float* w, float eps,
                          void* out, int ldo, hipStream_t s);

struct AttnArgs {
    const void* q; int ldq;
    const void* k; int ldk;
    const void* v; int ldv;
    void* out; int ldo;
    const int* cu_q;
    const int* cu_kv;
    int B, heads, head_dim, max_q;
    int causal, q_shared;
    float scale;
    int kv_group;
    const int* kv_end;
    const int* q_in_rows;
    int q_head_stride;
    int q_prescaled;
    float* lse;
};
hipError_t launch_attention(const AttnArgs& a, hipStream_t s);

constexpr int CHAT_MAX_ROWS = 16;
constexpr int CHAT_ATT_SPLITS = 8;
constexpr int CHAT_KEYS = 256;
constexpr int CHAT_SEL_WGS = 64;
constexpr int CHAT_TOPK_MAX = 64;
enum ChatSelMode { CHAT_SEL_GREEDY = 0, CHAT_SEL_BEAM = 1, CHAT_SEL_SAMPLE = 2 };
struct ChatStep {
    int n, groups;
    int row[CHAT_MAX_ROWS], slot[CHAT_MAX_ROWS], tail[CHAT_MAX_ROWS], pos[CHAT_MAX_ROWS], token[CHAT_MAX_ROWS];
    int g_lo[CHAT_MAX_ROWS + 1], plen[CHAT_MAX_ROWS];
    int gsplit[CHAT_MAX_ROWS], rsplit[CHAT_MAX_ROWS];
};
struct ChatCaps { int slots, len, rows, tail; };
struct ChatMove { int n; int src[CHAT_MAX_ROWS], dst[CHAT_MAX_ROWS], len[CHAT_MAX_ROWS]; };
struct ChatSel {
    int n, groups;
    int lrow[CHAT_MAX_ROWS], srow[CHAT_MAX_ROWS], g_lo[CHAT_MAX_ROWS + 1];
    float bscore[CHAT_MAX_ROWS];
};
hipError_t launch_chat_embed(const ChatStep& st, const void* table, int E, float scale, float* h, unsigned* seen, int words, hipStream_t s);
hipError_t launch_chat_qkv(const ChatStep& st, const float* parts, int n_parts, size_t plane, int ldp, const float* rope, int E, int heads,
                           void* q_out, void* tails, int l, int max_rows, int max_new, hipStream_t s);
hipError_t launch_chat_attn(const ChatStep& st, const void* q, const void* prompt, const void* tails, int l, int E, int heads,
                            const ChatCaps& cap, int S_max, float* po, float* pml, void* att, hipStream_t s);
hipError_t launch_chat_prompt_kv(const void* qkv, int ld, int T, int E, void* kdst, void* vdst, hipStream_t s);
hipError_t launch_chat_move(const ChatMove& mv, void* tails, void* scratch, int layers, int max_rows, int max_new, int E, int max_tail,
                            unsigned* seen, unsigned* seen_scratch, int words, hipStream_t s);
hipError_t launch_chat_select(const ChatSel& sel, int mode, const float* logits, int ld, int V, const unsigned* seen, int words, float pen,
                              float temperature, int K, int kout, unsigned long long seed, unsigned step, float* lse,
                              unsigned long long* part, float* o_score, int* o_tok, int* o_par, hipStream_t s);

constexpr int GEN_ATT_SPLITS = 16;
struct GenState {
    int token;
    int pos[3];
    int len;
    int step;
    int splits;
    int pad;
    int cu_q[GEN_ATT_SPLITS + 1], cu_kv[GEN_ATT_SPLITS + 1];
};
struct GenBatch {
    int token[16];
    int pos[3][16];
    int cache_row[16];
    int splits[16];
    int cu_q[16 * GEN_ATT_SPLITS + 1];
    int kv_lo[16 * GEN_ATT_SPLITS], kv_hi[16 * GEN_ATT_SPLITS];
    int q_in[16 * GEN_ATT_SPLITS];
    int sampled[16];
};
hipError_t launch_decode_begin(GenState* st, int q_rows, hipStream_t s);
struct PersistLayer {
    const void *wqkv, *wo, *wgu, *wd;
    const float* bqkv;
    const float *g1, *g2;
    void *kc, *vc;
};
struct PersistArgs {
    const PersistLayer* layers; int n_layers;
    int E, QKV, QD, KVD, H, KV, Ip, N2;
    int ldw_qkv, ldw_o, ldw_gu, ldw_d;
    int ks_qkv, ks_o, ks_d;
    float eps;
    const float* g_final;
    float* h; void* xn;
    float* planes; void* act; void* attp; float* lse; float* ss;
    const GenState* st; const float* inv_freq; int sec_t, sec_h;
    unsigned long long* sync;
    unsigned* abort_host;
};
hipError_t launch_decode_persist(const PersistArgs& a, int grid, hipStream_t s);
int decode_persist_occupancy();
hipError_t launch_mrope_cache(const void* src_bf16, const float* parts, int n_parts, size_t plane_stride, const float* bias,
                              int ld, int T, int H, int KV, const int* pos3, int pos_stride, int sec_t, int sec_h,
                              const float* inv_freq, void* q_out, int ldq, void* k_cache, void* v_cache, int ld_cache,
                              int cache_row0, int* cu_kv, hipStream_t s, const int* row0_dev = nullptr,
                              const int* cache_rows = nullptr);
hipError_t launch_rope2d_table(const int* pos_h, const int* pos_w, int T, int sec_h, const float* freq, void* cs, hipStream_t s);
hipError_t launch_rope2d_inplace(void* qkv, int ld, int T, int n_slots, int hh, const void* cs, hipStream_t s);
hipError_t launch_mark_seen(const int* ids, int n, unsigned* seen, int vocab, hipStream_t s);
hipError_t launch_sample(const float* logits, int vocab, unsigned* seen, float penalty, float temperature,
                         unsigned long long seed, unsigned step, int* token_out, unsigned long long* scratch64, hipStream_t s,
                         GenState* st = nullptr, int step_from_state = 0, int advance = 0);
hipError_t launch_scatter_rows(const float* src, const int* row_idx, int n, int dim, float* dst, int ld, hipStream_t s);
hipError_t launch_gather_rows_bf16(const float* src, const int* row_idx, int n, int dim, void* dst, int ld, hipStream_t s);
hipError_t launch_patch_rows_u8(const uint8_t* const* pages, const int* page_w, const int* img, const int* ph, const int* pw, int n,
                                int P, int tp, const float* mean3, const float* std3, void* dst, int ld, hipStream_t s);
hipError_t launch_attn_combine(const void* part, const float* lse, int S, int heads, int group, void* out, hipStream_t s,
                               const int* S_dev = nullptr,
                               int n_rows = 1, int ld_out = 0);

hipError_t launch_patch_embed(const uint8_t* const* imgs, int n_imgs, int H, int W, int P, const GemmArgs& g, int Kreal,
                              hipStream_t s);
hipError_t launch_embed_gather(const int* ids, int T, const void* table, int dim, float scale,
                               float* out, hipStream_t s);
hipError_t launch_pool(const float* h, const int* seq_offsets, int B, int dim, const float* norm_w,
                       float eps, float* out, float* tap_hidden, hipStream_t s, int mode = 0);
hipError_t launch_f32_to_bf16(const float* in, void* out, size_t n, hipStream_t s);
hipError_t launch_f32_to_bf16_pad(const float* in, void* out, size_t n, size_t n_total, hipStream_t s,
                                  int* zero_word = nullptr);
hipError_t launch_split_bf16(const float* in, void* hi, void* lo, size_t n, hipStream_t s);
hipError_t launch_iota_pos(const int* seq_offsets, int B, int* pos, hipStream_t s);
hipError_t launch_any_nonzero16(const void* p, size_t n, int* flag, hipStream_t s);

hipError_t launch_rmsnorm_split(const float* x, int rows, int dim, const float* w, float eps, void* hi, void* lo, hipStream_t s);
hipError_t launch_rope_f32(float* qkv, int T, int ld, int rope_cols, const int* pos, const float* table, hipStream_t s);
hipError_t launch_attn_f32(const float* qkv, int ld, int E, const int* seq_of, const int* seq_offsets, int T, int heads,
                           float scale, float* out, hipStream_t s);
hipError_t launch_swiglu_split(const float* gu, int T, int ld_gu, int I, int ld_act, void* hi, void* lo, hipStream_t s);
hipError_t launch_embed_gather_hp(const int* ids, int T, const void* table_hi, const void* table_lo, int dim, float scale,
                                  float* out, hipStream_t s);
hipError_t launch_seq_of(const int* seq_offsets, int B, int* seq_of, hipStream_t s);
hipError_t launch_planes_sum(const float* parts, int n_parts, size_t stride, int ldp, int T, int N, float* out, int ldo, float alpha,
                             bool accumulate, hipStream_t s);

hipError_t launch_synth_pages(uint8_t* out, int n, int size, long long seed, long long first, hipStream_t s);

}
#include <vector>
namespace vr {
int resize_coeffs(int in_size, int out_size, std::vector<int>& bounds, std::vector<int>& kk);
hipError_t launch_resize_h(const uint8_t* in, int in_w, int rows, uint8_t* out, int out_w, const int* bounds,
                           const int* kk, int ksize, hipStream_t s);
hipError_t launch_resize_v(const uint8_t* in, int w, uint8_t* out, int out_h, const int* bounds, const int* kk,
                           int ksize, hipStream_t s);

struct SearchArgs {
    const void* index_bf16;
    const float* index_f32;
    int64_t n_docs;
    int dim;
    const void* q_bf16;
    int convert_q;
    const float* q_f32;
    int nq, k;
    float* cand_scores; int* cand_ids; int n_chunks;
    float* out_scores; int64_t* out_ids;
    float* thr_init;
    int pre_own_chunks;
    float* thr_cert;
    unsigned long long* cand_keys;
    float* score_rows; size_t ld_scores;
    int exact_follows;
    int* huge_seen;
    const float* thr_used;
    float eps_rel;
    int eps_data;
    float acc_rel;
    const float* dmax;
    int* flag_count; int* flag_list;
    float* flag_tau;
    void* flag_q;
    int* flag2_count; int* flag2_list;
    unsigned* stats;
    unsigned long long* out_keys; int64_t id_offset;
    hipEvent_t* prof_ev;
};
constexpr int SEARCH_PROF_EVENTS = 6;
int search_kprime(int k);
int search_num_chunks(int64_t n_docs, int nq);
int search_prepass_owned(int64_t n_docs, int nq, int dim);
constexpr int SEARCH_PRE_SPOTS = 16;
int search_prepass_floats();
hipError_t launch_search(const SearchArgs& a, hipStream_t s);
bool search_uses_stream(int nq, int dim);
int search_stream_chunks();
hipError_t launch_search_stream(const SearchArgs& a, int kp, hipStream_t s);
bool search_uses_256(int nq);
hipError_t launch_sweep256(const SearchArgs& a, int kp, const float* thr, hipStream_t s);
bool sweep256w_ok(const SearchArgs& a);
hipError_t launch_sweep256w(const SearchArgs& a, int kp, const float* thr, hipStream_t s);
int search_bigk_max();
hipError_t launch_search_bigk(const SearchArgs& a, const float* S, size_t ldS, int q0, int nq_block, hipStream_t s);
hipError_t launch_topk_merge_big(const float* scores, const int64_t* ids, int n_parts, int nq, int k,
                                 float* out_scores, int64_t* out_ids, hipStream_t s);
hipError_t launch_topk_merge(const float* scores, const int64_t* ids, int n_parts, int nq, int k,
                             float* out_scores, int64_t* out_ids, hipStream_t s);
hipError_t launch_topk_merge_keys(const unsigned long long* keys, int n_parts, int nq, int k, float* out_scores,
                                  int64_t* out_ids, hipStream_t s);
hipError_t launch_exact_scores(const float* index_f32, int64_t n_docs, int dim, const float* q_f32, const int* flag_list,
                               const int* flag_count, int sub, int max_slots, float* S, size_t ldS, hipStream_t s);
hipError_t launch_exact_select(const SearchArgs& a, const float* S, size_t ldS, int sub, int max_slots, hipStream_t s);
int search_band_max();
hipError_t launch_band_select(const SearchArgs& a, const float* S, size_t ldS, int sub, int max_slots, hipStream_t s);
hipError_t launch_row_norm_max(const float* rows, int64_t n, int dim, float* dmax, hipStream_t s);
float search_default_eps_rel(int dim);
float search_acc_rel(int dim);

}
```

### visrag_amd/csrc/misc.hip

```cpp
#include "common.h"
#include "kernels.h"

namespace vr {

__global__ __launch_bounds__(256) void embed_gather_kernel(const int* __restrict__ ids, int T,
                                                           const bf16_t* __restrict__ table, int dim,
                                                           float scale, float* __restrict__ out) {
    const int t = blockIdx.x;
    const bf16_t* src = table + (size_t)ids[t] * dim;
    float* dst = out + (size_t)t * dim;
    for (int c = threadIdx.x * 4; c < dim; c += 1024) {
        const bf16x4 v = *reinterpret_cast<const bf16x4*>(src + c);
        f32x4 o;
#pragma unroll
        for (int r = 0; r < 4; ++r) o[r] = bf2f(v[r]) * scale;
        *reinterpret_cast<f32x4*>(dst + c) = o;
    }
}

hipError_t launch_embed_gather(const int* ids, int T, const void* table, int dim, float scale,
                               float* out, hipStream_t s) {
    if (T <= 0) return hipSuccess;
    if (dim % 4) return hipErrorInvalidValue;
    hipLaunchKernelGGL(embed_gather_kernel, dim3(T), dim3(256), 0, s, ids, T, (const bf16_t*)table, dim,
                       scale, out);
    return hipGetLastError();
}

constexpr int POOL_MAXV = 10;

__global__ __launch_bounds__(256) void pool_kernel(const float* __restrict__ h,
                                                   const int* __restrict__ seq_offsets, int dim,
                                                   const float* __restrict__ norm_w, float eps,
                                                   float* __restrict__ out, float* __restrict__ tap, int mode) {
    __shared__ float red[4][64 * 4 * POOL_MAXV];
    __shared__ float red_s[4];
    const int b = blockIdx.x, lane = threadIdx.x & 63, wave = threadIdx.x >> 6;
    const int t0 = seq_offsets[b], L = seq_offsets[b + 1] - t0;
    const int nv = dim >> 2;
    f32x4 acc[POOL_MAXV], ww[POOL_MAXV];
#pragma unroll
    for (int i = 0; i < POOL_MAXV; ++i) {
        acc[i] = f32x4{0.f, 0.f, 0.f, 0.f};
        const int c = lane + i * 64;
        ww[i] = (c < nv) ? reinterpret_cast<const f32x4*>(norm_w)[c] : f32x4{0.f, 0.f, 0.f, 0.f};
    }
    for (int t = wave; t < L; t += 4) {
        const f32x4* xr = reinterpret_cast<const f32x4*>(h + (size_t)(t0 + t) * dim);
        f32x4 v[POOL_MAXV];
        float ss = 0.f;
#pragma unroll
        for (int i = 0; i < POOL_MAXV; ++i) {
            const int c = lane + i * 64;
            v[i] = (c < nv) ? xr[c] : f32x4{0.f, 0.f, 0.f, 0.f};
            ss += v[i][0] * v[i][0] + v[i][1] * v[i][1] + v[i][2] * v[i][2] + v[i][3] * v[i][3];
        }
        ss = wave_sum(ss);
        const float rstd = rsqrtf(ss / dim + eps);
        const float wt = mode == 0 ? (float)(t + 1) : mode == 1 ? 1.0f : mode == 2 ? (t == L - 1 ? 1.0f : 0.0f) : (t == 0 ? 1.0f : 0.0f);
#pragma unroll
        for (int i = 0; i < POOL_MAXV; ++i) {
            const f32x4 y = v[i] * rstd * ww[i];
            acc[i] += y * wt;
            const int c = lane + i * 64;
            if (tap && c < nv) reinterpret_cast<f32x4*>(tap + (size_t)(t0 + t) * dim)[c] = y;
        }
    }
#pragma unroll
    for (int i = 0; i < POOL_MAXV; ++i)
#pragma unroll
        for (int r = 0; r < 4; ++r) red[wave][(lane + i * 64) * 4 + r] = acc[i][r];
    __syncthreads();
    const float denom = mode == 0 ? 0.5f * (float)L * (float)(L + 1) : mode == 1 ? (float)L : 1.0f;
    float sq = 0.f;
    float vals[POOL_MAXV];
#pragma unroll
    for (int i = 0; i < POOL_MAXV; ++i) {
        const int c = threadIdx.x + i * 256;
        float v = 0.f;
        if (c < dim) v = (red[0][c] + red[1][c] + red[2][c] + red[3][c]) / denom;
        vals[i] = v;
        sq += v * v;
    }
    sq = wave_sum(sq);
    if (lane == 0) red_s[wave] = sq;
    __syncthreads();
    const float nrm = fmaxf(sqrtf(red_s[0] + red_s[1] + red_s[2] + red_s[3]), 1e-12f);
#pragma unroll
    for (int i = 0; i < POOL_MAXV; ++i) {
        const int c = threadIdx.x + i * 256;
        if (c < dim) out[(size_t)b * dim + c] = vals[i] / nrm;
    }
}

hipError_t launch_pool(const float* h, const int* seq_offsets, int B, int dim, const float* norm_w,
                       float eps, float* out, float* tap_hidden, hipStream_t s, int mode) {
    if (B <= 0) return hipSuccess;
    if (dim % 4 || dim > 64 * 4 * POOL_MAXV || mode < 0 || mode > 3) return hipErrorInvalidValue;
    hipLaunchKernelGGL(pool_kernel, dim3(B), dim3(256), 0, s, h, seq_offsets, dim, norm_w, eps, out,
                       tap_hidden, mode);
    return hipGetLastError();
}

__global__ void f32_to_bf16_kernel(const float* __restrict__ in, bf16_t* __restrict__ out, size_t n) {
    size_t i = ((size_t)blockIdx.x * blockDim.x + threadIdx.x) * 4;
    const size_t stride = (size_t)gridDim.x * blockDim.x * 4;
    for (; i + 3 < n; i += stride) {
        const f32x4 v = *reinterpret_cast<const f32x4*>(in + i);
        bf16x4 o;
#pragma unroll
        for (int r = 0; r < 4; ++r) o[r] = f2bf(v[r]);
        *reinterpret_cast<bf16x4*>(out + i) = o;
    }
    if (blockIdx.x == 0 && threadIdx.x == 0)
        for (size_t j = n & ~(size_t)3; j < n; ++j) out[j] = f2bf(in[j]);
}

hipError_t launch_f32_to_bf16(const float* in, void* out, size_t n, hipStream_t s) {
    if (n == 0) return hipSuccess;
    const int blocks = (int)min((size_t)2048, (n / 4 + 255) / 256 + 1);
    hipLaunchKernelGGL(f32_to_bf16_kernel, dim3(blocks), dim3(256), 0, s, in, (bf16_t*)out, n);
    return hipGetLastError();
}

__global__ void f32_to_bf16_pad_kernel(const float* __restrict__ in, bf16_t* __restrict__ out, size_t n, size_t n_total,
                                       int* __restrict__ zero_word) {
    if (zero_word && blockIdx.x == 0 && threadIdx.x < 2) zero_word[threadIdx.x] = 0;
    size_t i = ((size_t)blockIdx.x * blockDim.x + threadIdx.x) * 4;
    const size_t stride = (size_t)gridDim.x * blockDim.x * 4;
    for (; i < n_total; i += stride) {
        bf16x4 o = {(bf16_t)0.f, (bf16_t)0.f, (bf16_t)0.f, (bf16_t)0.f};
        if (i < n) {
            const f32x4 v = *reinterpret_cast<const f32x4*>(in + i);
#pragma unroll
            for (int r = 0; r < 4; ++r) o[r] = f2bf(v[r]);
        }
        *reinterpret_cast<bf16x4*>(out + i) = o;
    }
}

hipError_t launch_f32_to_bf16_pad(const float* in, void* out, size_t n, size_t n_total, hipStream_t s, int* zero_word) {
    if (n_total == 0) return hipSuccess;
    if ((n | n_total) & 3) return hipErrorInvalidValue;
    const int blocks = (int)min((size_t)2048, (n_total / 4 + 255) / 256);
    hipLaunchKernelGGL(f32_to_bf16_pad_kernel, dim3(blocks), dim3(256), 0, s, in, (bf16_t*)out, n, n_total, zero_word);
    return hipGetLastError();
}

__global__ void split_bf16_kernel(const float* __restrict__ in, bf16_t* __restrict__ hi,
                                  bf16_t* __restrict__ lo, size_t n) {
    size_t i = (size_t)blockIdx.x * blockDim.x + threadIdx.x;
    const size_t stride = (size_t)gridDim.x * blockDim.x;
    for (; i < n; i += stride) {
        const float v = in[i];
        const bf16_t h = f2bf(v);
        hi[i] = h;
        lo[i] = f2bf(v - bf2f(h));
    }
}

hipError_t launch_split_bf16(const float* in, void* hi, void* lo, size_t n, hipStream_t s) {
    if (n == 0) return hipSuccess;
    const int blocks = (int)min((size_t)2048, (n + 255) / 256);
    hipLaunchKernelGGL(split_bf16_kernel, dim3(blocks), dim3(256), 0, s, in, (bf16_t*)hi, (bf16_t*)lo, n);
    return hipGetLastError();
}

__global__ void iota_pos_kernel(const int* __restrict__ seq_offsets, int* __restrict__ pos) {
    const int b = blockIdx.x;
    const int t0 = seq_offsets[b], L = seq_offsets[b + 1] - t0;
    for (int t = threadIdx.x; t < L; t += blockDim.x) pos[t0 + t] = t;
}

hipError_t launch_iota_pos(const int* seq_offsets, int B, int* pos, hipStream_t s) {
    if (B <= 0) return hipSuccess;
    hipLaunchKernelGGL(iota_pos_kernel, dim3(B), dim3(256), 0, s, seq_offsets, pos);
    return hipGetLastError();
}

__global__ void any_nonzero16_kernel(const uint16_t* __restrict__ p, size_t n, int* __restrict__ flag) {
    int any = 0;
    for (size_t i = (size_t)blockIdx.x * blockDim.x + threadIdx.x; i < n; i += (size_t)gridDim.x * blockDim.x)
        any |= (p[i] & 0x7FFFu) != 0;
    if (__any(any) && (threadIdx.x & 63) == 0) atomicOr(flag, 1);
}

hipError_t launch_any_nonzero16(const void* p, size_t n, int* flag, hipStream_t s) {
    if (n == 0) return hipSuccess;
    const int blocks = (int)min((size_t)2048, (n + 255) / 256);
    hipLaunchKernelGGL(any_nonzero16_kernel, dim3(blocks), dim3(256), 0, s, (const uint16_t*)p, n, flag);
    return hipGetLastError();
}

}
```

### visrag_amd/csrc/model.h

```cpp
#pragma once
#include <algorithm>
#include <map>
#include <string>
#include <utility>
#include <vector>

#include "engine_common.h"

struct VitBlock {
    Vec n1w, n1b, n2w, n2b; Linear qkv, proj, fc1, fc2;
};
struct DecLayer {
    Vec ln1, ln2; Linear qkv, o, gu, down; int parts_qkv = 0, parts_gu = 0;
    Linear qkv_lo, o_lo, gu_lo, down_lo;
};

struct GridTables {
    int gh = 0, gw = 0;
    DevBuf vit_pos;
    DevBuf pos_k;
};

struct Tap { std::vector<float> data; int64_t rows = 0, cols = 0; };

struct vr_model_s {
    int device = 0;
    vr_config_t c{};
    bool finalized = false, taps_on = false;
    int pool_mode = 0;
    bool borrowed = false;
    int D = 0, Dp = 0, F = 0, Fp = 0, E = 0, I = 0, Ip = 0, Kpe = 0, Kpe_p = 0, Q = 0;
    Linear patch;
    std::vector<float> pos_embed_host;
    std::vector<VitBlock> blocks;
    Vec vit_nw, vit_nb;
    Linear r_kvproj, r_kv, r_out, r_proj;
    Vec r_lnq_w, r_lnq_b, r_lnkv_w, r_lnkv_b, r_lnpost_w, r_lnpost_b;
    std::vector<float> r_query_host, r_wq_host, r_bq_host;
    bool has_query = false, has_inproj = false, has_inproj_b = false, has_pos = false;
    DevBuf r_q;
    DevBuf embed;  bool has_embed = false;
    DevBuf embed_lo; bool has_embed_lo = false;
    std::vector<DecLayer> layers;
    Vec final_norm;
    DevBuf rope;
    int rope_len = 0;
    std::map<std::pair<int, int>, GridTables> grids;
    int64_t Mcap = 0, Tcap = 0, Rcap = 0;
    DevBuf w_hvit, w_xn, w_qkv, w_att, w_mlp, w_kv32, w_xkv, w_KV, w_ratt, w_rout, w_rln;
    DevBuf w_h, w_dxn, w_dqkv, w_datt, w_dact, w_part;
    DevBuf w_cu, w_ids, w_seq, w_pos, w_rowmap, w_imgptr, w_pix, w_out;
    DevBuf w_hp_hi, w_hp_planes, w_hp_qkv, w_hp_att, w_hp_gu, w_seqof;
    DevBuf w_hp_part;
    DevBuf w_hidden;
    std::map<std::string, Tap> taps;
    bool prof_on = false;
    int prof_level = 0;
    struct ProfClass { std::vector<hipEvent_t> ev; size_t used = 0; double ms = 0, flops = 0; int64_t launches = 0; };
    ProfClass prof[VR_PROF_CLASSES];
    char* arena = nullptr; size_t arena_cap = 0, arena_used = 0;
    hipEvent_t arena_ev = nullptr; bool arena_pending = false, arena_open = false;
};

static inline int arena_begin(vr_model_s* m, size_t need) {
    if (m->arena_pending) { HIPCHK(hipEventSynchronize(m->arena_ev)); m->arena_pending = false; }
    if (!m->arena_ev) HIPCHK(hipEventCreateWithFlags(&m->arena_ev, hipEventDisableTiming));
    if (m->arena_cap < need) {
        if (m->arena) (void)hipHostFree(m->arena);
        m->arena = nullptr; m->arena_cap = 0;
        const size_t cap = std::max(need, (size_t)4 << 20);
        HIPCHK(hipHostMalloc((void**)&m->arena, cap, hipHostMallocDefault));
        m->arena_cap = cap;
    }
    m->arena_used = 0;
    m->arena_open = true;
    return VR_OK;
}
static inline void arena_close(vr_model_s* m, void* stream) {
    if (m->arena_open && m->arena_ev) {
        if (hipEventRecord(m->arena_ev, (hipStream_t)stream) == hipSuccess) m->arena_pending = true;
        else (void)hipStreamSynchronize((hipStream_t)stream);
    }
    m->arena_open = false;
}
static inline void* arena_take(vr_model_s* m, size_t bytes) {
    void* p = m->arena + m->arena_used;
    m->arena_used += (bytes + 63) / 64 * 64;
    return p;
}

static inline int prof_begin(vr_model_s* m, int cls, hipStream_t s) {
    if (!m->prof_on || (cls >= VR_PROF_DEC_QKV) != (m->prof_level == 2)) return VR_OK;
    auto& p = m->prof[cls];
    if (p.used + 2 > p.ev.size()) {
        for (int i = 0; i < 64; ++i) { hipEvent_t e; HIPCHK(hipEventCreate(&e)); p.ev.push_back(e); }
    }
    HIPCHK(hipEventRecord(p.ev[p.used], s));
    return VR_OK;
}
static inline int prof_end(vr_model_s* m, int cls, double flops, hipStream_t s) {
    if (!m->prof_on || (cls >= VR_PROF_DEC_QKV) != (m->prof_level == 2)) return VR_OK;
    auto& p = m->prof[cls];
    HIPCHK(hipEventRecord(p.ev[p.used + 1], s));
    p.used += 2; p.launches += 1; p.flops += flops;
    return VR_OK;
}
static inline int prof_collect(vr_model_s* m) {
    HIPCHK(hipDeviceSynchronize());
    for (auto& p : m->prof) {
        for (size_t i = 0; i + 1 < p.used; i += 2) {
            float ms = 0.f;
            HIPCHK(hipEventElapsedTime(&ms, p.ev[i], p.ev[i + 1]));
            p.ms += ms;
        }
        p.used = 0;
    }
    return VR_OK;
}

constexpr int DEC_KSPLIT_MAX = 3;

static inline GemmArgs gemm_args(const void* A, int lda, const Linear& L, int M, void* out, int ldo) {
    GemmArgs a{};
    a.A = A; a.lda = lda; a.W = L.w.p; a.ldw = L.k_pad; a.M = M; a.N = L.n_pad; a.K = L.k_pad;
    a.bias = L.has_b ? L.b.as<float>() : nullptr;
    a.out = out; a.ldo = ldo; a.alpha = 1.0f;
    return a;
}

struct EncodeHook {
    bool bf16_route = false;
    int (*layer)(void* ctx, int l, const void* qkv, int ldqkv, int T, hipStream_t s) = nullptr;
    void* ctx = nullptr;
};

std::vector<float> rope_table_host(float theta, int len);
int get_grid(vr_model_s* m, int gh, int gw, GridTables** out);
int tap_store(vr_model_s* m, const char* name, const void* dev, int64_t rows, int64_t cols, int64_t ld, bool is_bf16, hipStream_t s);
int encode_impl(vr_model_t m, const uint8_t* const* slices, const int32_t* slice_hw, int32_t n_slices,
                int32_t slices_on_device, const int32_t* input_ids, const int32_t* seq_offsets, int32_t B,
                const int32_t* vision_rows, float* out_reps, int32_t out_on_device, void* stream,
                float* out_hidden = nullptr, int32_t hidden_len = 0, const EncodeHook* hook = nullptr);
```

### visrag_amd/csrc/model.hip

```cpp
#include <hip/hip_runtime.h>

#include <algorithm>
#include <cmath>
#include <cstdio>
#include <cstring>

#include "model.h"

extern "C" const char* vr_version(void) { return "visrag_hip 0.1.0 (gfx950)"; }
extern "C" const char* vr_last_error(void) { return g_err.c_str(); }
extern "C" int vr_device_count(int* count) {
    if (!count) return fail(VR_ERR_INVALID, "count is NULL");
    HIPCHK(hipGetDeviceCount(count));
    return VR_OK;
}

extern "C" int vr_model_create(int device_id, const vr_config_t* cfg, vr_model_t* out) {
    if (!cfg || !out) return fail(VR_ERR_INVALID, "cfg/out is NULL");
    const vr_config_t& c = *cfg;
    if (c.vit_dim % c.vit_heads || c.vit_dim / c.vit_heads != 72)
        return fail(VR_ERR_INVALID, "ViT head_dim must be 72 (vit_dim %d / heads %d)", c.vit_dim, c.vit_heads);
    if (c.hidden_size % 128) return fail(VR_ERR_INVALID, "hidden_size %d must be a multiple of 128", c.hidden_size);
    if (c.hidden_size % c.num_heads || c.hidden_size / c.num_heads != 64)
        return fail(VR_ERR_INVALID, "decoder head_dim must be 64");
    if (c.intermediate_size % 64) return fail(VR_ERR_INVALID, "intermediate_size must be a multiple of 64");
    if (c.query_num != 64) return fail(VR_ERR_INVALID, "query_num must be 64");
    if (c.vit_dim % 4 || c.hidden_size > 2560 || c.vit_dim > 2560) return fail(VR_ERR_INVALID, "dims out of range");
    if (c.max_images <= 0 || c.max_patches <= 0 || c.max_tokens <= 0 || c.max_seqs <= 0)
        return fail(VR_ERR_INVALID, "workspace limits must be positive");
    VRCHK(set_dev(device_id));
    vr_model_s* m = new vr_model_s();
    m->device = device_id;
    m->c = c;
    m->D = c.vit_dim; m->Dp = pad128(c.vit_dim);
    m->F = c.vit_hidden; m->Fp = pad128(c.vit_hidden);
    m->E = c.hidden_size; m->I = c.intermediate_size; m->Ip = pad128(c.intermediate_size);
    m->Kpe = 3 * c.patch_size * c.patch_size; m->Kpe_p = pad128(m->Kpe);
    m->Q = c.query_num;
    m->blocks.resize(c.vit_depth);
    m->layers.resize(c.num_layers);
    *out = m;
    return VR_OK;
}

extern "C" int vr_model_destroy(vr_model_t m) {
    if (!m) return VR_OK;
    (void)hipSetDevice(m->device);
    (void)hipDeviceSynchronize();
    if (!m->borrowed) {
        auto fl = [](Linear& l) { l.w.free(); l.b.free(); };
        fl(m->patch); fl(m->r_kvproj); fl(m->r_kv); fl(m->r_out); fl(m->r_proj);
        for (auto& b : m->blocks) {
            fl(b.qkv); fl(b.proj); fl(b.fc1); fl(b.fc2); b.n1w.v.free(); b.n1b.v.free(); b.n2w.v.free(); b.n2b.v.free();
        }
        for (auto& l : m->layers) { fl(l.qkv); fl(l.o); fl(l.gu); fl(l.down); fl(l.qkv_lo); fl(l.o_lo); fl(l.gu_lo); fl(l.down_lo); l.ln1.v.free(); l.ln2.v.free(); }
        for (Vec* v : {&m->vit_nw, &m->vit_nb, &m->r_lnq_w, &m->r_lnq_b, &m->r_lnkv_w, &m->r_lnkv_b, &m->r_lnpost_w, &m->r_lnpost_b, &m->final_norm}) v->v.free();
        for (DevBuf* b : {&m->r_q, &m->embed, &m->embed_lo, &m->rope}) b->free();
    }
    for (auto& g : m->grids) { g.second.vit_pos.free(); g.second.pos_k.free(); }
    for (auto& pc : m->prof) for (hipEvent_t e : pc.ev) (void)hipEventDestroy(e);
    if (m->arena) (void)hipHostFree(m->arena);
    if (m->arena_ev) (void)hipEventDestroy(m->arena_ev);
    for (DevBuf* b : {&m->w_hvit, &m->w_xn, &m->w_qkv, &m->w_att, &m->w_mlp,
                      &m->w_kv32, &m->w_xkv, &m->w_KV, &m->w_ratt, &m->w_rout, &m->w_rln, &m->w_h, &m->w_dxn, &m->w_part, &m->w_dqkv,
                      &m->w_datt, &m->w_dact, &m->w_cu, &m->w_ids, &m->w_seq, &m->w_pos, &m->w_rowmap, &m->w_imgptr,
                      &m->w_pix, &m->w_out, &m->w_hp_hi, &m->w_hp_planes, &m->w_hp_qkv, &m->w_hp_att, &m->w_hp_gu, &m->w_seqof, &m->w_hp_part, &m->w_hidden})
        b->free();
    delete m;
    return VR_OK;
}

extern "C" int vr_model_load_weight(vr_model_t m, const char* name_c, const void* data, const int64_t* shape,
                                    int32_t ndim, int32_t dtype, int32_t on_device) {
    if (!m || !name_c || !data || !shape) return fail(VR_ERR_INVALID, "NULL argument");
    if (dtype != VR_DTYPE_F32 && dtype != VR_DTYPE_BF16) return fail(VR_ERR_INVALID, "bad dtype %d", dtype);
    VRCHK(set_dev(m->device));
    const std::string name(name_c);
    const int bf = dtype == VR_DTYPE_BF16;
    size_t numel = 1;
    for (int i = 0; i < ndim; ++i) numel *= (size_t)shape[i];
    const vr_config_t& c = m->c;
    const int D = m->D, F = m->F, E = m->E, I = m->I;
    auto bad_shape = [&]() { return fail(VR_ERR_INVALID, "unexpected shape for %s", name_c); };

    if (name.rfind("llm.lm_head.", 0) == 0 || name.rfind("vpm.attn_pool.", 0) == 0 ||
        name == "resampler.pos_embed" || name.find("rotary_emb") != std::string::npos)
        return VR_OK;

    Staged st;
    VRCHK(stage(data, numel * (bf ? 2 : 4), on_device, st));
    const void* src = st.dev;
    m->finalized = false;

    if (name == "vpm.patch_embed.proj.weight") {
        if (!shape_is(shape, ndim, {D, 3, c.patch_size, c.patch_size})) return bad_shape();
        Linear& L = m->patch;
        if (!L.w.p) { L.n = D; L.k = m->Kpe; L.n_pad = pad128(D); L.k_pad = pad128(m->Kpe); VRCHK(L.w.alloc((size_t)pad256(D) * L.k_pad * 2)); }
        HIPCHK(launch_pack_patch_weight(src, bf, D, c.patch_size, L.w.p, L.k_pad, 0));
        HIPCHK(hipDeviceSynchronize());
        L.has_w = true;
        return VR_OK;
    }
    if (name == "vpm.patch_embed.proj.bias") { if (numel != (size_t)D) return bad_shape(); return load_bias_part(m->patch, D, src, bf, D, 0); }
    if (name == "vpm.pos_embed") {
        if (numel != (size_t)c.vit_pos_grid * c.vit_pos_grid * D) return bad_shape();
        m->has_pos = true;
        m->grids.clear();
        return to_host_f32(src, bf, numel, m->pos_embed_host);
    }
    if (name == "vpm.norm.weight") { if (numel != (size_t)D) return bad_shape(); return load_vec(m->vit_nw, src, bf, D, m->Dp); }
    if (name == "vpm.norm.bias") { if (numel != (size_t)D) return bad_shape(); return load_vec(m->vit_nb, src, bf, D, m->Dp); }
    if (name.rfind("vpm.blocks.", 0) == 0) {
        int n = -1, off = 0;
        if (sscanf(name.c_str(), "vpm.blocks.%d.%n", &n, &off) < 1) return fail(VR_ERR_INVALID, "bad key %s", name_c);
        if (n >= c.vit_depth) return VR_OK;
        const std::string sub = name.substr(off);
        VitBlock& b = m->blocks[n];
        if (sub == "norm1.weight") { if (numel != (size_t)D) return bad_shape(); return load_vec(b.n1w, src, bf, D, m->Dp); }
        if (sub == "norm1.bias") { if (numel != (size_t)D) return bad_shape(); return load_vec(b.n1b, src, bf, D, m->Dp); }
        if (sub == "norm2.weight") { if (numel != (size_t)D) return bad_shape(); return load_vec(b.n2w, src, bf, D, m->Dp); }
        if (sub == "norm2.bias") { if (numel != (size_t)D) return bad_shape(); return load_vec(b.n2b, src, bf, D, m->Dp); }
        if (sub == "attn.qkv.weight") { if (!shape_is(shape, ndim, {3 * D, D})) return bad_shape(); return load_linear_part(b.qkv, 3 * D, D, src, bf, 3 * D, D, 0, 3 * D, 0, 0); }
        if (sub == "attn.qkv.bias") { if (numel != (size_t)3 * D) return bad_shape(); return load_bias_part(b.qkv, 3 * D, src, bf, 3 * D, 0); }
        if (sub == "attn.proj.weight") { if (!shape_is(shape, ndim, {D, D})) return bad_shape(); return load_linear_part(b.proj, D, D, src, bf, D, D, 0, D, 0, 0); }
        if (sub == "attn.proj.bias") { if (numel != (size_t)D) return bad_shape(); return load_bias_part(b.proj, D, src, bf, D, 0); }
        if (sub == "mlp.fc1.weight") { if (!shape_is(shape, ndim, {F, D})) return bad_shape(); return load_linear_part(b.fc1, F, D, src, bf, F, D, 0, F, 0, 0); }
        if (sub == "mlp.fc1.bias") { if (numel != (size_t)F) return bad_shape(); return load_bias_part(b.fc1, F, src, bf, F, 0); }
        if (sub == "mlp.fc2.weight") { if (!shape_is(shape, ndim, {D, F})) return bad_shape(); return load_linear_part(b.fc2, D, F, src, bf, D, F, 0, D, 0, 0); }
        if (sub == "mlp.fc2.bias") { if (numel != (size_t)D) return bad_shape(); return load_bias_part(b.fc2, D, src, bf, D, 0); }
        return fail(VR_ERR_INVALID, "unknown ViT key %s", name_c);
    }
    if (name.rfind("resampler.", 0) == 0) {
        const std::string sub = name.substr(10);
        if (sub == "query") { if (!shape_is(shape, ndim, {m->Q, E})) return bad_shape(); m->has_query = true; return to_host_f32(src, bf, numel, m->r_query_host); }
        if (sub == "kv_proj.weight") { if (!shape_is(shape, ndim, {E, D})) return bad_shape(); return load_linear_part(m->r_kvproj, E, D, src, bf, E, D, 0, E, 0, 0); }
        if (sub == "attn.in_proj_weight") {
            if (!shape_is(shape, ndim, {3 * E, E})) return bad_shape();
            std::vector<float> all;
            VRCHK(to_host_f32(src, bf, (size_t)E * E, all));
            m->r_wq_host.swap(all);
            m->has_inproj = true;
            const char* kv_src = (const char*)src + (size_t)E * E * (bf ? 2 : 4);
            return load_linear_part(m->r_kv, 2 * E, E, kv_src, bf, 2 * E, E, 0, 2 * E, 0, 0);
        }
        if (sub == "attn.in_proj_bias") {
            if (numel != (size_t)3 * E) return bad_shape();
            VRCHK(to_host_f32(src, bf, (size_t)E, m->r_bq_host));
            m->has_inproj_b = true;
            const char* kv_src = (const char*)src + (size_t)E * (bf ? 2 : 4);
            return load_bias_part(m->r_kv, 2 * E, kv_src, bf, 2 * E, 0);
        }
        if (sub == "attn.out_proj.weight") { if (!shape_is(shape, ndim, {E, E})) return bad_shape(); return load_linear_part(m->r_out, E, E, src, bf, E, E, 0, E, 0, 0); }
        if (sub == "attn.out_proj.bias") { if (numel != (size_t)E) return bad_shape(); return load_bias_part(m->r_out, E, src, bf, E, 0); }
        if (sub == "proj") { if (!shape_is(shape, ndim, {E, E})) return bad_shape(); return load_linear_part(m->r_proj, E, E, src, bf, E, E, 1, E, 0, 0); }
        Vec* v = nullptr;
        if (sub == "ln_q.weight") v = &m->r_lnq_w; else if (sub == "ln_q.bias") v = &m->r_lnq_b;
        else if (sub == "ln_kv.weight") v = &m->r_lnkv_w; else if (sub == "ln_kv.bias") v = &m->r_lnkv_b;
        else if (sub == "ln_post.weight") v = &m->r_lnpost_w; else if (sub == "ln_post.bias") v = &m->r_lnpost_b;
        if (!v) return fail(VR_ERR_INVALID, "unknown resampler key %s", name_c);
        if (numel != (size_t)E) return bad_shape();
        return load_vec(*v, src, bf, E, E);
    }
    if (name == "llm.model.embed_tokens.weight") {
        if (!shape_is(shape, ndim, {c.vocab_size, E})) return bad_shape();
        VRCHK(m->embed.alloc(numel * 2));
        HIPCHK(launch_pack_weight(src, bf, c.vocab_size, E, E, 0, m->embed.p, E, c.vocab_size, 0, 0, 0));
        m->has_embed_lo = false;
        if (!bf && c.text_split_precision) {
            VRCHK(m->embed_lo.alloc(numel * 2));
            HIPCHK(launch_pack_weight(src, bf, c.vocab_size, E, E, 0, m->embed_lo.p, E, c.vocab_size, 0, 0, 0, 1));
            m->has_embed_lo = true;
        }
        HIPCHK(hipDeviceSynchronize());
        m->has_embed = true;
        return VR_OK;
    }
    if (name == "llm.model.norm.weight") { if (numel != (size_t)E) return bad_shape(); return load_vec(m->final_norm, src, bf, E, E); }
    if (name.rfind("llm.model.layers.", 0) == 0) {
        int n = -1, off = 0;
        if (sscanf(name.c_str(), "llm.model.layers.%d.%n", &n, &off) < 1) return fail(VR_ERR_INVALID, "bad key %s", name_c);
        if (n >= c.num_layers) return fail(VR_ERR_INVALID, "layer index %d out of range", n);
        const std::string sub = name.substr(off);
        DecLayer& l = m->layers[n];
        if (sub == "input_layernorm.weight") { if (numel != (size_t)E) return bad_shape(); return load_vec(l.ln1, src, bf, E, E); }
        if (sub == "post_attention_layernorm.weight") { if (numel != (size_t)E) return bad_shape(); return load_vec(l.ln2, src, bf, E, E); }
        const bool lo = !bf && c.text_split_precision;
        for (int part = 0; part < 3; ++part) {
            static const char* nm[3] = {"self_attn.q_proj.weight", "self_attn.k_proj.weight", "self_attn.v_proj.weight"};
            if (sub == nm[part]) {
                if (!shape_is(shape, ndim, {E, E})) return bad_shape();
                l.parts_qkv |= 1 << part;
                if (lo) VRCHK(load_linear_part(l.qkv_lo, 3 * E, E, src, bf, E, E, 0, E, 0, part * E, 1));
                return load_linear_part(l.qkv, 3 * E, E, src, bf, E, E, 0, E, 0, part * E);
            }
        }
        if (sub == "self_attn.o_proj.weight") {
            if (!shape_is(shape, ndim, {E, E})) return bad_shape();
            if (lo) VRCHK(load_linear_part(l.o_lo, E, E, src, bf, E, E, 0, E, 0, 0, 1));
            return load_linear_part(l.o, E, E, src, bf, E, E, 0, E, 0, 0);
        }
        if (sub == "mlp.gate_proj.weight" || sub == "mlp.up_proj.weight") {
            if (!shape_is(shape, ndim, {I, E})) return bad_shape();
            const int up = sub == "mlp.up_proj.weight";
            l.parts_gu |= 1 << up;
            if (lo) VRCHK(load_linear_part(l.gu_lo, 2 * I, E, src, bf, I, E, 0, 16, 32, up * 16, 1));
            return load_linear_part(l.gu, 2 * I, E, src, bf, I, E, 0, 16, 32, up * 16);
        }
        if (sub == "mlp.down_proj.weight") {
            if (!shape_is(shape, ndim, {E, I})) return bad_shape();
            if (lo) VRCHK(load_linear_part(l.down_lo, E, I, src, bf, E, I, 0, E, 0, 0, 1));
            return load_linear_part(l.down, E, I, src, bf, E, I, 0, E, 0, 0);
        }
        return fail(VR_ERR_INVALID, "unknown decoder key %s", name_c);
    }
    return fail(VR_ERR_INVALID, "unknown weight key %s", name_c);
}

static void sincos_2d_host(int E, int gh, int gw, std::vector<float>& out) {
    const int half = E / 2, quarter = half / 2;
    out.assign((size_t)gh * gw * E, 0.f);
    std::vector<float> omega(quarter);
    for (int i = 0; i < quarter; ++i) {
        float o = (float)i / ((float)half / 2.0f);
        omega[i] = 1.0f / powf(10000.0f, o);
    }
    for (int y = 0; y < gh; ++y)
        for (int x = 0; x < gw; ++x) {
            float* row = out.data() + ((size_t)y * gw + x) * E;
            for (int i = 0; i < quarter; ++i) {
                const float a = (float)x * omega[i], b = (float)y * omega[i];
                row[i] = sinf(a); row[quarter + i] = cosf(a);
                row[half + i] = sinf(b); row[half + quarter + i] = cosf(b);
            }
        }
}

static inline float cubic_aa(float x) {
    const float a = -0.5f;
    x = fabsf(x);
    if (x < 1.0f) return ((a + 2.0f) * x - (a + 3.0f)) * x * x + 1.0f;
    if (x < 2.0f) return (((x - 5.0f) * x + 8.0f) * x - 4.0f) * a;
    return 0.0f;
}
static void aa_weights(int in, int out, std::vector<int>& xmin, std::vector<int>& xsize, std::vector<float>& w, int& maxk) {
    const float scale = (float)in / (float)out;
    const float support = (scale >= 1.0f) ? 2.0f * scale : 2.0f;
    const float invscale = (scale >= 1.0f) ? 1.0f / scale : 1.0f;
    maxk = (int)ceilf(support) * 2 + 1;
    xmin.resize(out); xsize.resize(out); w.assign((size_t)out * maxk, 0.f);
    for (int i = 0; i < out; ++i) {
        const float center = scale * ((float)i + 0.5f);
        int lo = std::max(0, (int)(center - support + 0.5f));
        int hi = std::min(in, (int)(center + support + 0.5f));
        xmin[i] = lo; xsize[i] = hi - lo;
        float tot = 0.f;
        for (int j = 0; j < xsize[i]; ++j) {
            const float ww = cubic_aa(((float)(j + lo) - center + 0.5f) * invscale);
            w[(size_t)i * maxk + j] = ww; tot += ww;
        }
        for (int j = 0; j < xsize[i]; ++j) w[(size_t)i * maxk + j] /= tot;
    }
}
static void resample_pos_host(const std::vector<float>& pe, int gi, int D, int gh, int gw, std::vector<float>& out) {
    out.assign((size_t)gh * gw * D, 0.f);
    if (gh == gi && gw == gi) { out = pe; return; }
    std::vector<int> xm, xs, ym, ys; std::vector<float> xw, yw; int xk, yk;
    aa_weights(gi, gw, xm, xs, xw, xk);
    aa_weights(gi, gh, ym, ys, yw, yk);
    std::vector<float> tmp((size_t)gi * gw * D, 0.f);
    for (int y = 0; y < gi; ++y)
        for (int x = 0; x < gw; ++x) {
            float* o = tmp.data() + ((size_t)y * gw + x) * D;
            for (int j = 0; j < xs[x]; ++j) {
                const float ww = xw[(size_t)x * xk + j];
                const float* s = pe.data() + ((size_t)y * gi + xm[x] + j) * D;
                for (int d = 0; d < D; ++d) o[d] += ww * s[d];
            }
        }
    for (int y = 0; y < gh; ++y)
        for (int x = 0; x < gw; ++x) {
            float* o = out.data() + ((size_t)y * gw + x) * D;
            for (int j = 0; j < ys[y]; ++j) {
                const float ww = yw[(size_t)y * yk + j];
                const float* s = tmp.data() + ((size_t)(ym[y] + j) * gw + x) * D;
                for (int d = 0; d < D; ++d) o[d] += ww * s[d];
            }
        }
}

std::vector<float> rope_table_host(float theta, int len) {
    std::vector<float> tab((size_t)len * 64);
    float inv[32];
    for (int i = 0; i < 32; ++i) inv[i] = 1.0f / powf(theta, (float)(2 * i) / 64.0f);
    for (int p = 0; p < len; ++p)
        for (int i = 0; i < 32; ++i) {
            const float a = (float)p * inv[i];
            tab[(size_t)p * 64 + i] = cosf(a);
            tab[(size_t)p * 64 + 32 + i] = sinf(a);
        }
    return tab;
}

static int alloc_workspace(vr_model_s* m) {
    const vr_config_t& c = m->c;
    const int64_t M = pad256l((int64_t)c.max_images * c.max_patches);
    const int64_t T = pad256l(c.max_tokens);
    const int64_t R = pad256l((int64_t)c.max_images * m->Q);
    m->Mcap = M; m->Tcap = T; m->Rcap = R;
    const int E = m->E, Dp = m->Dp;
    VRCHK(m->w_hvit.alloc((size_t)M * Dp * 4));
    VRCHK(m->w_xn.alloc((size_t)M * Dp * 2));
    VRCHK(m->w_qkv.alloc((size_t)M * pad128(3 * m->D) * 2));
    VRCHK(m->w_att.alloc((size_t)M * Dp * 2));
    VRCHK(m->w_mlp.alloc((size_t)M * m->Fp * 2));
    VRCHK(m->w_kv32.alloc((size_t)M * E * 4));
    VRCHK(m->w_xkv.alloc((size_t)M * E * 2));
    VRCHK(m->w_KV.alloc((size_t)M * 2 * E * 2));
    VRCHK(m->w_ratt.alloc((size_t)R * E * 2));
    VRCHK(m->w_rout.alloc((size_t)R * E * 4));
    VRCHK(m->w_rln.alloc((size_t)R * E * 2));
    VRCHK(m->w_h.alloc((size_t)T * E * 4));
    VRCHK(m->w_dxn.alloc((size_t)T * E * 2));
    VRCHK(m->w_part.alloc((size_t)DEC_KSPLIT_MAX * T * E * 4));
    VRCHK(m->w_dqkv.alloc((size_t)T * 3 * E * 2));
    VRCHK(m->w_datt.alloc((size_t)T * E * 2));
    VRCHK(m->w_dact.alloc((size_t)T * m->Ip * 2));
    VRCHK(m->w_cu.alloc((size_t)(c.max_images + c.max_seqs + 8) * 2 * 4));
    VRCHK(m->w_ids.alloc((size_t)T * 4));
    VRCHK(m->w_seq.alloc((size_t)(c.max_seqs + 1) * 4));
    VRCHK(m->w_pos.alloc((size_t)T * 4));
    VRCHK(m->w_rowmap.alloc((size_t)R * 4));
    VRCHK(m->w_imgptr.alloc((size_t)c.max_images * 8));
    VRCHK(m->w_out.alloc((size_t)c.max_seqs * E * 4));
    if (c.text_split_precision) {
        const int Kmax = std::max(E, m->Ip);
        VRCHK(m->w_hp_hi.alloc((size_t)2 * T * Kmax * 2));
        VRCHK(m->w_hp_qkv.alloc((size_t)T * 3 * E * 4));
        VRCHK(m->w_hp_att.alloc((size_t)T * E * 4));
        VRCHK(m->w_hp_gu.alloc((size_t)T * pad128(2 * m->I) * 4));
        VRCHK(m->w_seqof.alloc((size_t)T * 4));
        VRCHK(m->w_hp_part.alloc((size_t)3 * 32 * 65536 * 4));
    }
    return VR_OK;
}

extern "C" int vr_model_finalize(vr_model_t m) {
    if (!m) return fail(VR_ERR_INVALID, "NULL model");
    VRCHK(set_dev(m->device));
    const vr_config_t& c = m->c;
    const int E = m->E;
    auto need = [&](bool ok, const char* what) { return ok ? VR_OK : fail(VR_ERR_STATE, "missing weight: %s", what); };
    VRCHK(need(m->patch.has_w && m->patch.has_b, "vpm.patch_embed.proj"));
    VRCHK(need(m->has_pos, "vpm.pos_embed"));
    VRCHK(need(m->vit_nw.ok && m->vit_nb.ok, "vpm.norm"));
    for (int n = 0; n < c.vit_depth; ++n) {
        const VitBlock& b = m->blocks[n];
        const bool ok = b.n1w.ok && b.n1b.ok && b.n2w.ok && b.n2b.ok && b.qkv.has_w && b.qkv.has_b && b.proj.has_w &&
                        b.proj.has_b && b.fc1.has_w && b.fc1.has_b && b.fc2.has_w && b.fc2.has_b;
        if (!ok) return fail(VR_ERR_STATE, "missing weight in vpm.blocks.%d", n);
    }
    VRCHK(need(m->has_query && m->has_inproj && m->has_inproj_b, "resampler.query / attn.in_proj"));
    VRCHK(need(m->r_kvproj.has_w && m->r_kv.has_w && m->r_kv.has_b && m->r_out.has_w && m->r_out.has_b && m->r_proj.has_w,
               "resampler linear weights"));
    VRCHK(need(m->r_lnq_w.ok && m->r_lnq_b.ok && m->r_lnkv_w.ok && m->r_lnkv_b.ok && m->r_lnpost_w.ok && m->r_lnpost_b.ok,
               "resampler layer norms"));
    VRCHK(need(m->has_embed && m->final_norm.ok, "llm.model.embed_tokens / norm"));
    for (int n = 0; n < c.num_layers; ++n) {
        const DecLayer& l = m->layers[n];
        const bool ok = l.ln1.ok && l.ln2.ok && l.parts_qkv == 7 && l.parts_gu == 3 && l.o.has_w && l.down.has_w;
        if (!ok) return fail(VR_ERR_STATE, "missing weight in llm.model.layers.%d", n);
    }
    {
        const int Q = m->Q;
        std::vector<float> lw(E), lb(E), pq;
        HIPCHK(hipMemcpy(lw.data(), m->r_lnq_w.v.p, (size_t)E * 4, hipMemcpyDeviceToHost));
        HIPCHK(hipMemcpy(lb.data(), m->r_lnq_b.v.p, (size_t)E * 4, hipMemcpyDeviceToHost));
        const int g = (int)lround(sqrt((double)Q));
        sincos_2d_host(E, g, g, pq);
        std::vector<float> x((size_t)Q * E), out((size_t)Q * E);
        for (int q = 0; q < Q; ++q) {
            const float* s = m->r_query_host.data() + (size_t)q * E;
            double mu = 0; for (int i = 0; i < E; ++i) mu += s[i]; mu /= E;
            double var = 0; for (int i = 0; i < E; ++i) { const double d = s[i] - mu; var += d * d; } var /= E;
            const float rstd = (float)(1.0 / sqrt(var + (double)c.resampler_ln_eps));
            for (int i = 0; i < E; ++i) x[(size_t)q * E + i] = ((float)(s[i] - mu)) * rstd * lw[i] + lb[i] + pq[(size_t)q * E + i];
        }
        for (int q = 0; q < Q; ++q)
            for (int n = 0; n < E; ++n) {
                const float* wr = m->r_wq_host.data() + (size_t)n * E;
                const float* xr = x.data() + (size_t)q * E;
                float acc = 0.f;
                for (int i = 0; i < E; ++i) acc += xr[i] * wr[i];
                out[(size_t)q * E + n] = acc + m->r_bq_host[n];
            }
        DevBuf t;
        VRCHK(t.alloc(out.size() * 4));
        HIPCHK(hipMemcpy(t.p, out.data(), out.size() * 4, hipMemcpyHostToDevice));
        VRCHK(m->r_q.alloc((size_t)pad128(Q) * E * 2));
        HIPCHK(launch_f32_to_bf16(t.as<float>(), m->r_q.p, out.size(), 0));
        HIPCHK(hipDeviceSynchronize());
        t.free();
    }
    {
        m->rope_len = std::max(c.max_tokens, 16);
        const std::vector<float> tab = rope_table_host(c.rope_theta, m->rope_len);
        VRCHK(m->rope.alloc(tab.size() * 4));
        HIPCHK(hipMemcpy(m->rope.p, tab.data(), tab.size() * 4, hipMemcpyHostToDevice));
    }
    if (c.text_split_precision) {
        DevBuf flag;
        VRCHK(flag.alloc(4));
        for (auto& l : m->layers)
            for (Linear* L : {&l.qkv_lo, &l.o_lo, &l.gu_lo, &l.down_lo})
                if (L->has_w) HIPCHK(launch_any_nonzero16(L->w.p, L->w.bytes / 2, flag.as<int>(), 0));
        int any = 0;
        HIPCHK(hipMemcpy(&any, flag.p, 4, hipMemcpyDeviceToHost));
        if (!any)
            for (auto& l : m->layers)
                for (Linear* L : {&l.qkv_lo, &l.o_lo, &l.gu_lo, &l.down_lo}) { L->w.free(); L->has_w = false; }
        if (m->has_embed_lo) {
            HIPCHK(hipMemset(flag.p, 0, 4));
            HIPCHK(launch_any_nonzero16(m->embed_lo.p, m->embed_lo.bytes / 2, flag.as<int>(), 0));
            HIPCHK(hipMemcpy(&any, flag.p, 4, hipMemcpyDeviceToHost));
            if (!any) { m->embed_lo.free(); m->has_embed_lo = false; }
        }
    }
    if (!m->w_h.p) VRCHK(alloc_workspace(m));
    m->finalized = true;
    return VR_OK;
}


int get_grid(vr_model_s* m, int gh, int gw, GridTables** out) {
    auto key = std::make_pair(gh, gw);
    auto it = m->grids.find(key);
    if (it != m->grids.end()) { *out = &it->second; return VR_OK; }
    const int N = gh * gw, D = m->D, Dp = m->Dp, E = m->E;
    GridTables g;
    g.gh = gh; g.gw = gw;
    {
        std::vector<float> rs, padded((size_t)N * Dp, 0.f);
        resample_pos_host(m->pos_embed_host, m->c.vit_pos_grid, D, gh, gw, rs);
        for (int r = 0; r < N; ++r) memcpy(padded.data() + (size_t)r * Dp, rs.data() + (size_t)r * D, (size_t)D * 4);
        VRCHK(g.vit_pos.alloc(padded.size() * 4));
        HIPCHK(hipMemcpy(g.vit_pos.p, padded.data(), padded.size() * 4, hipMemcpyHostToDevice));
    }
    {
        std::vector<float> sc;
        sincos_2d_host(E, gh, gw, sc);
        const int Np = pad128(N);
        DevBuf f32, hi, lo, tmp;
        VRCHK(f32.alloc((size_t)Np * E * 4));
        VRCHK(hi.alloc((size_t)Np * E * 2));
        VRCHK(lo.alloc((size_t)Np * E * 2));
        VRCHK(tmp.alloc((size_t)Np * E * 4));
        VRCHK(g.pos_k.alloc((size_t)Np * E * 4));
        HIPCHK(hipMemcpy(f32.p, sc.data(), sc.size() * 4, hipMemcpyHostToDevice));
        HIPCHK(launch_split_bf16(f32.as<float>(), hi.p, lo.p, (size_t)N * E, 0));
        GemmArgs a{};
        a.A = hi.p; a.lda = E; a.W = m->r_kv.w.p; a.ldw = m->r_kv.k_pad; a.M = N; a.N = E; a.K = E;
        a.out = tmp.p; a.ldo = E; a.alpha = 1.f;
        HIPCHK(launch_gemm(a, EPI_F32, GEMM_VARIANT_GLDS, 0));
        a.A = lo.p; a.resid = tmp.as<float>(); a.out = g.pos_k.p;
        HIPCHK(launch_gemm(a, EPI_RESID, GEMM_VARIANT_GLDS, 0));
        HIPCHK(hipDeviceSynchronize());
        f32.free(); hi.free(); lo.free(); tmp.free();
    }
    auto ins = m->grids.emplace(key, std::move(g));
    *out = &ins.first->second;
    return VR_OK;
}

int tap_store(vr_model_s* m, const char* name, const void* dev, int64_t rows, int64_t cols, int64_t ld, bool is_bf16, hipStream_t s) {
    if (!m->taps_on) return VR_OK;
    HIPCHK(hipStreamSynchronize(s));
    Tap& t = m->taps[name];
    t.rows = rows; t.cols = cols;
    t.data.resize((size_t)rows * cols);
    const size_t esz = is_bf16 ? 2 : 4;
    std::vector<char> raw((size_t)rows * ld * esz);
    HIPCHK(hipMemcpy(raw.data(), dev, raw.size(), hipMemcpyDeviceToHost));
    for (int64_t r = 0; r < rows; ++r)
        for (int64_t cc = 0; cc < cols; ++cc) {
            if (is_bf16) {
                uint16_t b; memcpy(&b, raw.data() + ((size_t)r * ld + cc) * 2, 2);
                uint32_t u = (uint32_t)b << 16; float f; memcpy(&f, &u, 4);
                t.data[(size_t)r * cols + cc] = f;
            } else {
                float f; memcpy(&f, raw.data() + ((size_t)r * ld + cc) * 4, 4);
                t.data[(size_t)r * cols + cc] = f;
            }
        }
    return VR_OK;
}

extern "C" int vr_model_set_pooling(vr_model_t m, int32_t mode) {
    if (!m) return fail(VR_ERR_INVALID, "NULL model");
    if (mode < VR_POOL_WMEAN || mode > VR_POOL_CLS) return fail(VR_ERR_INVALID, "pooling mode %d: 0 wmean, 1 mean, 2 lasttoken, 3 cls", mode);
    m->pool_mode = mode;
    return VR_OK;
}

extern "C" int vr_model_set_taps(vr_model_t m, int32_t enable) {
    if (!m) return fail(VR_ERR_INVALID, "NULL model");
    m->taps_on = enable != 0;
    if (!enable) m->taps.clear();
    return VR_OK;
}

extern "C" int vr_model_tap(vr_model_t m, const char* name, float* out, int64_t rows, int64_t cols) {
    if (!m || !name || !out) return fail(VR_ERR_INVALID, "NULL argument");
    auto it = m->taps.find(name);
    if (it == m->taps.end()) return fail(VR_ERR_STATE, "tap %s not recorded (enable taps, then encode)", name);
    const Tap& t = it->second;
    if (rows > t.rows || cols != t.cols) return fail(VR_ERR_INVALID, "tap %s is [%lld][%lld]", name, (long long)t.rows, (long long)t.cols);
    memcpy(out, t.data.data(), (size_t)rows * cols * 4);
    return VR_OK;
}

extern "C" int vr_model_clone(vr_model_t src, vr_model_t* out) {
    if (!src || !out) return fail(VR_ERR_INVALID, "src/out is NULL");
    if (!src->finalized) return fail(VR_ERR_STATE, "vr_model_clone before vr_model_finalize");
    VRCHK(set_dev(src->device));
    vr_model_s* m = new vr_model_s(*src);
    m->borrowed = true;
    for (DevBuf* b : {&m->w_hvit, &m->w_xn, &m->w_qkv, &m->w_att, &m->w_mlp, &m->w_kv32, &m->w_xkv, &m->w_KV,
                      &m->w_ratt, &m->w_rout, &m->w_rln, &m->w_h, &m->w_dxn, &m->w_part, &m->w_dqkv, &m->w_datt, &m->w_dact,
                      &m->w_cu, &m->w_ids, &m->w_seq, &m->w_pos, &m->w_rowmap, &m->w_imgptr, &m->w_pix, &m->w_out,
                      &m->w_hp_hi, &m->w_hp_planes, &m->w_hp_qkv, &m->w_hp_att, &m->w_hp_gu, &m->w_seqof, &m->w_hp_part, &m->w_hidden}) {
        b->free();
    }
    m->grids.clear();
    m->taps.clear(); m->taps_on = false;
    m->prof_on = false;
    for (auto& pc : m->prof) { pc.ev.clear(); pc.used = 0; pc.ms = 0; pc.flops = 0; pc.launches = 0; }
    m->arena = nullptr; m->arena_cap = 0; m->arena_used = 0; m->arena_ev = nullptr; m->arena_pending = false; m->arena_open = false;
    const int r = alloc_workspace(m);
    if (r != VR_OK) { (void)vr_model_destroy(m); return r; }
    *out = m;
    return VR_OK;
}

extern "C" int vr_model_set_profile(vr_model_t m, int32_t enable) {
    if (!m) return fail(VR_ERR_INVALID, "NULL model");
    VRCHK(set_dev(m->device));
    VRCHK(prof_collect(m));
    m->prof_on = enable != 0;
    m->prof_level = enable == 2 ? 2 : (enable ? 1 : 0);
    for (auto& p : m->prof) { p.ms = 0; p.flops = 0; p.launches = 0; p.used = 0; }
    return VR_OK;
}

extern "C" int vr_model_get_profile(vr_model_t m, int32_t cls, double* total_ms, int64_t* launches, double* total_flops) {
    if (!m || cls < 0 || cls >= VR_PROF_CLASSES || !total_ms || !launches || !total_flops)
        return fail(VR_ERR_INVALID, "bad profile arguments");
    VRCHK(set_dev(m->device));
    VRCHK(prof_collect(m));
    *total_ms = m->prof[cls].ms; *launches = m->prof[cls].launches; *total_flops = m->prof[cls].flops;
    return VR_OK;
}
```

### visrag_amd/csrc/patch_embed.hip

```cpp
#include "gemm_core.h"
#include "gemm_epilogue.h"
#include "kernels.h"

namespace vr {

struct PatchArgs {
    const uint8_t* const* imgs;
    int H, W, P, gw, N;
    GemmArgs g;
    int Kreal;
};

__global__ __launch_bounds__(256) void patch_embed_kernel(PatchArgs a) {
    extern __shared__ __attribute__((aligned(16))) char smem[];
    const GemmArgs& p = a.g;
    const int tiles_n = p.N / GEMM_BN;
    const int tiles_m = (p.M + GEMM_BM - 1) / GEMM_BM;
    const int t = xcd_remap(blockIdx.x, tiles_m * tiles_n);
    const int m0 = (t / tiles_n) * GEMM_BM, n0 = (t % tiles_n) * GEMM_BN;
    const int tid = threadIdx.x, lane = tid & 63, wave = tid >> 6;
    const int wm = wave >> 1, wn = wave & 1;
    const int rowbytes = a.W * 3, seg = a.P * 3;

    const int kc = tid & 7;
    const uint8_t* pbase[4];
    bool rok[4];
#pragma unroll
    for (int i = 0; i < 4; ++i) {
        const int row = (tid >> 3) + 32 * i;
        const int m = min(m0 + row, p.M - 1);
        rok[i] = m0 + row < p.M;
        const int img = m / a.N, pp = m % a.N;
        const int py = pp / a.gw, px = pp % a.gw;
        pbase[i] = a.imgs[img] + (size_t)(py * a.P) * rowbytes + px * seg;
    }
    uint8_t px8[4][8];
    auto load_pixels = [&](int k0) {
#pragma unroll
        for (int e = 0; e < 8; ++e) {
            const int k = k0 + kc * 8 + e;
            const int kk = min(k, a.Kreal - 1);
            const int off = (kk / seg) * rowbytes + (kk % seg);
#pragma unroll
            for (int i = 0; i < 4; ++i) px8[i][e] = pbase[i][off];
        }
    };
    auto write_tile = [&](char* tile, int k0) {
#pragma unroll
        for (int i = 0; i < 4; ++i) {
            const int row = (tid >> 3) + 32 * i;
            bf16x8 v;
#pragma unroll
            for (int e = 0; e < 8; ++e) {
                const float f = ((float)px8[i][e] / 255.0f - 0.5f) / 0.5f;
                v[e] = (rok[i] && k0 + kc * 8 + e < a.Kreal) ? f2bf(f) : (bf16_t)0.f;
            }
            *reinterpret_cast<bf16x8*>(tile + row * 128 + ((kc ^ (row & 7)) << 4)) = v;
        }
    };

    gemm_acc_t acc;
    gemm_zero(acc);
    const bf16_t* Wp = (const bf16_t*)p.W;
    const int nk = p.K / GEMM_BK;
    load_pixels(0);
    stage_glds(Wp, p.ldw, n0, 0, smem + GEMM_TILE_BYTES, wave, lane);
    write_tile(smem, 0);
    for (int kt = 0; kt < nk; ++kt) {
        char* cur = smem + (kt & 1) * 2 * GEMM_TILE_BYTES;
        char* nxt = smem + ((kt + 1) & 1) * 2 * GEMM_TILE_BYTES;
        __syncthreads();
        if (kt + 1 < nk) {
            load_pixels((kt + 1) * GEMM_BK);
            stage_glds(Wp, p.ldw, n0, (kt + 1) * GEMM_BK, nxt + GEMM_TILE_BYTES, wave, lane);
        }
        gemm_compute_tile(acc, cur, cur + GEMM_TILE_BYTES, wm, wn, lane);
        if (kt + 1 < nk) write_tile(nxt, (kt + 1) * GEMM_BK);
    }
#pragma unroll
    for (int i = 0; i < 4; ++i)
        gemm_epilogue_row<EPI_F32>(acc[i], p, m0 + wm * 64 + i * 16 + (lane & 15), n0 + wn * 64, lane >> 4);
}

hipError_t launch_patch_embed(const uint8_t* const* imgs, int n_imgs, int H, int W, int P, const GemmArgs& g, int Kreal,
                              hipStream_t s) {
    if (n_imgs <= 0) return hipSuccess;
    if (H % P || W % P || g.N % GEMM_BN || g.K % GEMM_BK || Kreal != 3 * P * P || Kreal > g.K || g.rowmap || g.ksplit > 1)
        return hipErrorInvalidValue;
    PatchArgs a{};
    a.imgs = imgs; a.H = H; a.W = W; a.P = P; a.gw = W / P; a.N = (H / P) * (W / P); a.g = g; a.Kreal = Kreal;
    const int tiles = (g.N / GEMM_BN) * ((g.M + GEMM_BM - 1) / GEMM_BM);
    static unsigned long long attr = 0;
    set_max_dynamic_lds((const void*)patch_embed_kernel, GEMM_SMEM_BYTES, attr);
    hipLaunchKernelGGL(patch_embed_kernel, dim3(tiles), dim3(256), GEMM_SMEM_BYTES, s, a);
    return hipGetLastError();
}

}
```

### visrag_amd/csrc/search_exact.hip

```cpp
#include "kernels.h"
#include "search_common.h"

namespace vr {

constexpr int EX_QB = 8;
constexpr int EX_ROWS = 64;

__global__ __launch_bounds__(256) void exact_scores_kernel(const float* __restrict__ index_f32, int64_t n_docs, int dim,
                                                           const float* __restrict__ q_f32,
                                                           const int* __restrict__ flag_list,
                                                           const int* __restrict__ flag_count, int sub, int max_slots,
                                                           float* __restrict__ S, size_t ldS) {
    extern __shared__ __attribute__((aligned(16))) char smem[];
    const int nf = min(flag_count[0] - sub, max_slots);
    if (nf <= 0) return;
    flag_list += sub;
    f32x4* qs = reinterpret_cast<f32x4*>(smem);
    const int tid = threadIdx.x, lane = tid & 63, wave = tid >> 6;
    const int nv = dim >> 2;
    for (int f0 = 0; f0 < nf; f0 += EX_QB) {
        const int nb = min(EX_QB, nf - f0);
        __syncthreads();
        for (int e = tid; e < nb * nv; e += 256) {
            const int b = e / nv, c = e % nv;
            qs[b * nv + c] = reinterpret_cast<const f32x4*>(q_f32 + (size_t)flag_list[f0 + b] * dim)[c];
        }
        __syncthreads();
        auto row_at = [&](int i) -> int64_t {
            return ((int64_t)blockIdx.x + (int64_t)(i >> 4) * gridDim.x) * EX_ROWS + wave * 16 + (i & 15);
        };
        auto load_row = [&](f32x4 (&dv)[MERGE_MAXV], int64_t row) {
            if (row >= n_docs) return;
            const f32x4* dr = reinterpret_cast<const f32x4*>(index_f32 + (size_t)row * dim);
#pragma unroll
            for (int i = 0; i < MERGE_MAXV; ++i) {
                const int c = lane + i * 64;
                dv[i] = (c < nv) ? dr[c] : f32x4{0.f, 0.f, 0.f, 0.f};
            }
        };
        auto score_row = [&](const f32x4 (&dv)[MERGE_MAXV], int64_t row) {
            for (int b = 0; b < nb; ++b) {
                float a = 0.f;
#pragma unroll
                for (int i = 0; i < MERGE_MAXV; ++i) {
                    const int c = lane + i * 64;
                    if (c < nv) a = dot_chunk(qs[b * nv + c], dv[i], a);
                }
                a = wave_sum(a);
                if (lane == 0) S[(size_t)(f0 + b) * ldS + row] = a;
            }
        };
        f32x4 dA[MERGE_MAXV], dB[MERGE_MAXV];
        load_row(dA, row_at(0));
        for (int i = 0; row_at(i) < n_docs; i += 2) {
            load_row(dB, row_at(i + 1));
            score_row(dA, row_at(i));
            if (row_at(i + 1) >= n_docs) break;
            load_row(dA, row_at(i + 2));
            score_row(dB, row_at(i + 1));
        }
    }
}

hipError_t launch_exact_scores(const float* index_f32, int64_t n_docs, int dim, const float* q_f32, const int* flag_list,
                               const int* flag_count, int sub, int max_slots, float* S, size_t ldS, hipStream_t s) {
    if (n_docs <= 0 || max_slots <= 0) return hipSuccess;
    if (dim % 4 || dim > 64 * 4 * MERGE_MAXV) return hipErrorInvalidValue;
    const int lds = EX_QB * dim * 4;
    static unsigned long long attr = 0;
    set_max_dynamic_lds((const void*)exact_scores_kernel, EX_QB * 64 * 4 * MERGE_MAXV * 4, attr);
    int64_t blocks = (n_docs + EX_ROWS - 1) / EX_ROWS;
    if (blocks > 512) blocks = 512;
    hipLaunchKernelGGL(exact_scores_kernel, dim3((unsigned)blocks), dim3(256), lds, s, index_f32, n_docs, dim, q_f32,
                       flag_list, flag_count, sub, max_slots, S, ldS);
    return hipGetLastError();
}

__global__ __launch_bounds__(256) void row_norm_max_kernel(const float* __restrict__ rows, int64_t n, int dim,
                                                           float* __restrict__ dmax) {
    const int lane = threadIdx.x & 63, wave = threadIdx.x >> 6;
    const int nv = dim >> 2;
    float m = 0.f, mr = 0.f;
    for (int64_t r = (int64_t)blockIdx.x * 4 + wave; r < n; r += (int64_t)gridDim.x * 4) {
        const f32x4* x = reinterpret_cast<const f32x4*>(rows + (size_t)r * dim);
        float ss = 0.f, rr = 0.f;
        for (int c = lane; c < nv; c += 64) {
            const f32x4 v = x[c];
#pragma unroll
            for (int e = 0; e < 4; ++e) {
                const float d = bf16_resid(v[e]);
                ss = __builtin_fmaf(v[e], v[e], ss);
                rr = __builtin_fmaf(d, d, rr);
            }
        }
        m = fmaxf(m, wave_sum(ss));
        mr = fmaxf(mr, wave_sum(rr));
    }
    if (lane == 0 && m > 0.f) atomicMax(reinterpret_cast<unsigned*>(dmax), __float_as_uint(sqrtf(m) * 1.00001f));
    if (lane == 0 && mr > 0.f) atomicMax(reinterpret_cast<unsigned*>(dmax) + 1, __float_as_uint(sqrtf(mr) * 1.00001f));
}

hipError_t launch_row_norm_max(const float* rows, int64_t n, int dim, float* dmax, hipStream_t s) {
    if (n <= 0) return hipSuccess;
    if (dim % 4) return hipErrorInvalidValue;
    const int64_t nb4 = (n + 3) / 4;
    const int blocks = (int)(nb4 < 2048 ? nb4 : 2048);
    hipLaunchKernelGGL(row_norm_max_kernel, dim3(blocks), dim3(256), 0, s, rows, n, dim, dmax);
    return hipGetLastError();
}

float search_acc_rel(int dim) { return (float)(2 * dim + 128) * 0x1p-24f; }
float search_default_eps_rel(int dim) {
    return 0x1p-7f + 0x1p-16f + search_acc_rel(dim) * (1.f + 0x1p-8f) * (1.f + 0x1p-8f);
}

}
```

Measured before the change: 713.8 pages/s.

## Batch front-end uploads, fuse iota into embed gather, rewrite patch-embed kernel

Packs token ids, sequence offsets, image pointers, cu tables and rowmaps into one host staging buffer and uploads them with a single copy, so several small H2D copies per call go away. Pixel uploads now happen after the embed gather is queued. The position iota kernel is folded into the embed-gather launch as extra blocks, and index row-add fuses copy, bf16 conversion and norm-max into one kernel. The patch-embed GEMM is rewritten to keep the whole pixel A-panel in LDS and stream multi-stage weight tiles across all N tiles, with templated bias and position-bias epilogues. This adds LDS pressure and some new size constraints.

```diff
diff --git a/visrag_amd/csrc/common.h b/visrag_amd/csrc/common.h
--- a/visrag_amd/csrc/common.h
+++ b/visrag_amd/csrc/common.h
@@ -30,6 +30,11 @@
     return v;
 }
 
+__device__ __forceinline__ void iota_pos_block(const int* __restrict__ seq_offsets, int b, int* __restrict__ pos) {
+    const int t0 = seq_offsets[b], L = seq_offsets[b + 1] - t0;
+    for (int t = threadIdx.x; t < L; t += blockDim.x) pos[t0 + t] = t;
+}
+
 __device__ __forceinline__ int xcd_remap(int bid, int nwg) {
     const int xcd = bid & 7, q = nwg >> 3, r = nwg & 7;
     const int base = (xcd < r) ? xcd * (q + 1) : r * (q + 1) + (xcd - r) * q;
diff --git a/visrag_amd/csrc/encode.hip b/visrag_amd/csrc/encode.hip
--- a/visrag_amd/csrc/encode.hip
+++ b/visrag_amd/csrc/encode.hip
@@ -7,20 +7,33 @@
 
 #include "model.h"
 
-static int run_vision_group(vr_model_s* m, const uint8_t* const* dev_imgs_hostarray, int n, int H, int W,
-                            const int32_t* rowmap_host , bool first_group, hipStream_t s) {
+struct VisionPass { int H, W; std::vector<int> idx; };
+static void fill_vision_front(char* host, const FrontLayout& f, const VisionPass& vp, const std::vector<const uint8_t*>& dev_ptr,
+                              const int32_t* vision_rows, int N, int Q) {
+    const int n = (int)vp.idx.size();
+    const uint8_t** ptrs = (const uint8_t**)(host + f.imgptr);
+    int* cu = (int*)(host + f.cu);
+    int32_t* rowmap = (int32_t*)(host + f.rowmap);
+    for (int k = 0; k < n; ++k) {
+        ptrs[k] = dev_ptr[vp.idx[k]];
+        memcpy(rowmap + (size_t)k * Q, vision_rows + (size_t)vp.idx[k] * Q, (size_t)Q * 4);
+    }
+    for (int i = 0; i <= n; ++i) { cu[i] = i * N; cu[n + 1 + i] = i * Q; }
+}
+static void view_vision_front(vr_model_s* m, const FrontLayout& f, int n, int Q) {
+    char* d = (char*)m->w_front.p;
+    m->w_imgptr.view(d + f.imgptr, (size_t)n * 8);
+    m->w_cu.view(d + f.cu, (size_t)2 * (n + 1) * 4);
+    m->w_rowmap.view(d + f.rowmap, (size_t)n * Q * 4);
+}
+
+static int run_vision_group(vr_model_s* m, int n, int H, int W, bool first_group, hipStream_t s) {
     const vr_config_t& c = m->c;
     const int P = c.patch_size, gh = H / P, gw = W / P, N = gh * gw;
     const int D = m->D, Dp = m->Dp, E = m->E, Q = m->Q;
     const int M = n * N;
     GridTables* g = nullptr;
     VRCHK(get_grid(m, gh, gw, &g));
-
-    HIPCHK(hipMemcpyAsync(m->w_imgptr.p, dev_imgs_hostarray, (size_t)n * 8, hipMemcpyHostToDevice, s));
-    int* cu = (int*)arena_take(m, (size_t)2 * (n + 1) * 4);
-    for (int i = 0; i <= n; ++i) { cu[i] = i * N; cu[n + 1 + i] = i * Q; }
-    HIPCHK(hipMemcpyAsync(m->w_cu.p, cu, (size_t)2 * (n + 1) * 4, hipMemcpyHostToDevice, s));
-    HIPCHK(hipMemcpyAsync(m->w_rowmap.p, rowmap_host, (size_t)n * Q * 4, hipMemcpyHostToDevice, s));
     const int* cu_tok = m->w_cu.as<int>();
     const int* cu_qry = m->w_cu.as<int>() + (n + 1);
 
@@ -275,28 +288,11 @@
     for (int i = 0; i < n_slices * Q; ++i)
         if (vision_rows[i] >= T) return fail(VR_ERR_INVALID, "vision row %d out of range", vision_rows[i]);
 
-    VRCHK(arena_begin(m, (size_t)T * 4 + (size_t)(B + 1) * 4 + (size_t)n_slices * (Q * 4 + 8 + 64 * 3) + 4096));
-    {
-        int* a_ids = (int*)arena_take(m, (size_t)T * 4);
-        int* a_seq = (int*)arena_take(m, (size_t)(B + 1) * 4);
-        memcpy(a_ids, input_ids, (size_t)T * 4);
-        memcpy(a_seq, seq_offsets, (size_t)(B + 1) * 4);
-        HIPCHK(hipMemcpyAsync(m->w_ids.p, a_ids, (size_t)T * 4, hipMemcpyHostToDevice, s));
-        HIPCHK(hipMemcpyAsync(m->w_seq.p, a_seq, (size_t)(B + 1) * 4, hipMemcpyHostToDevice, s));
-    }
-    int max_len = 0;
-    for (int i = 0; i < B; ++i) max_len = std::max(max_len, seq_offsets[i + 1] - seq_offsets[i]);
-    const bool hp = n_slices == 0 && c.text_split_precision != 0 && (c.text_split_precision == 1 || max_len <= c.text_split_precision) &&
-                    !(hook && hook->bf16_route);
-    if (hp && m->has_embed_lo)
-        HIPCHK(launch_embed_gather_hp(m->w_ids.as<int>(), T, m->embed.p, m->embed_lo.p, E, c.scale_emb, m->w_h.as<float>(), s));
-    else
-        HIPCHK(launch_embed_gather(m->w_ids.as<int>(), T, m->embed.p, E, c.scale_emb, m->w_h.as<float>(), s));
-    HIPCHK(launch_iota_pos(m->w_seq.as<int>(), B, m->w_pos.as<int>(), s));
-
+    std::vector<VisionPass> passes;
+    std::vector<const uint8_t*> dev_ptr(n_slices);
+    std::vector<size_t> pix_off(n_slices);
     if (n_slices > 0) {
         size_t pix_total = 0;
-        std::vector<size_t> pix_off(n_slices);
         for (int i = 0; i < n_slices; ++i) {
             const int H = slice_hw[2 * i], W = slice_hw[2 * i + 1];
             if (H <= 0 || W <= 0 || H % c.patch_size || W % c.patch_size)
@@ -306,19 +302,13 @@
             pix_off[i] = pix_total;
             pix_total += ((size_t)H * W * 3 + 15) / 16 * 16;
         }
-        std::vector<const uint8_t*> dev_ptr(n_slices);
         if (slices_on_device) {
             for (int i = 0; i < n_slices; ++i) dev_ptr[i] = slices[i];
         } else {
             if (m->w_pix.bytes < pix_total) VRCHK(m->w_pix.alloc(pix_total));
-            for (int i = 0; i < n_slices; ++i) {
-                const size_t nb = (size_t)slice_hw[2 * i] * slice_hw[2 * i + 1] * 3;
-                HIPCHK(hipMemcpyAsync((char*)m->w_pix.p + pix_off[i], slices[i], nb, hipMemcpyHostToDevice, s));
-                dev_ptr[i] = (const uint8_t*)m->w_pix.p + pix_off[i];
-            }
+            for (int i = 0; i < n_slices; ++i) dev_ptr[i] = (const uint8_t*)m->w_pix.p + pix_off[i];
         }
         std::vector<char> done(n_slices, 0);
-        bool first = true;
         for (int i = 0; i < n_slices; ++i) {
             if (done[i]) continue;
             const int H = slice_hw[2 * i], W = slice_hw[2 * i + 1];
@@ -328,17 +318,60 @@
                 if (!done[j] && slice_hw[2 * j] == H && slice_hw[2 * j + 1] == W) { idx.push_back(j); done[j] = 1; }
             const int per_pass = std::max(1, (int)std::min<int64_t>(c.max_images, ((int64_t)c.max_images * c.max_patches) / N));
             for (size_t lo = 0; lo < idx.size(); lo += per_pass) {
-                const int n = (int)std::min<size_t>(per_pass, idx.size() - lo);
-                const uint8_t** ptrs = (const uint8_t**)arena_take(m, (size_t)n * 8);
-                int32_t* rowmap = (int32_t*)arena_take(m, (size_t)n * Q * 4);
-                for (int k = 0; k < n; ++k) {
-                    ptrs[k] = dev_ptr[idx[lo + k]];
-                    memcpy(rowmap + (size_t)k * Q, vision_rows + (size_t)idx[lo + k] * Q, (size_t)Q * 4);
-                }
-                VRCHK(run_vision_group(m, ptrs, n, H, W, rowmap, first, s));
-                first = false;
+                const size_t n = std::min<size_t>(per_pass, idx.size() - lo);
+                passes.push_back(VisionPass{H, W, std::vector<int>(idx.begin() + lo, idx.begin() + lo + n)});
             }
         }
+    }
+
+    const size_t n_first = passes.empty() ? 0 : passes[0].idx.size();
+    const FrontLayout f0 = front_layout((size_t)T, (size_t)B, n_first, (size_t)Q);
+    const size_t front_bytes = passes.empty() ? f0.imgptr : f0.end;
+    size_t arena_need = front_bytes + 64;
+    for (size_t i = 1; i < passes.size(); ++i) {
+        const FrontLayout f = front_layout((size_t)T, (size_t)B, passes[i].idx.size(), (size_t)Q);
+        arena_need += f.end - f.imgptr;
+    }
+    VRCHK(arena_begin(m, arena_need));
+    auto patches_of = [&](const VisionPass& vp) { return (vp.H / c.patch_size) * (vp.W / c.patch_size); };
+    {
+        char* fh = (char*)arena_take(m, front_bytes);
+        char* fd = (char*)m->w_front.p;
+        memcpy(fh, input_ids, (size_t)T * 4);
+        memcpy(fh + f0.seq, seq_offsets, (size_t)(B + 1) * 4);
+        if (!passes.empty()) fill_vision_front(fh, f0, passes[0], dev_ptr, vision_rows, patches_of(passes[0]), Q);
+        HIPCHK(hipMemcpyAsync(fd, fh, front_bytes, hipMemcpyHostToDevice, s));
+        m->w_ids.view(fd, (size_t)T * 4);
+        m->w_seq.view(fd + f0.seq, (size_t)(B + 1) * 4);
+    }
+    int max_len = 0;
+    for (int i = 0; i < B; ++i) max_len = std::max(max_len, seq_offsets[i + 1] - seq_offsets[i]);
+    const bool hp = n_slices == 0 && c.text_split_precision != 0 && (c.text_split_precision == 1 || max_len <= c.text_split_precision) &&
+                    !(hook && hook->bf16_route);
+    if (hp && m->has_embed_lo)
+        HIPCHK(launch_embed_gather_hp(m->w_ids.as<int>(), T, m->embed.p, m->embed_lo.p, E, c.scale_emb, m->w_h.as<float>(), s,
+                                      m->w_seq.as<int>(), B, m->w_pos.as<int>()));
+    else
+        HIPCHK(launch_embed_gather(m->w_ids.as<int>(), T, m->embed.p, E, c.scale_emb, m->w_h.as<float>(), s, m->w_seq.as<int>(), B,
+                                   m->w_pos.as<int>()));
+
+    if (n_slices > 0 && !slices_on_device) {
+        for (int i = 0; i < n_slices; ++i) {
+            const size_t nb = (size_t)slice_hw[2 * i] * slice_hw[2 * i + 1] * 3;
+            HIPCHK(hipMemcpyAsync((char*)m->w_pix.p + pix_off[i], slices[i], nb, hipMemcpyHostToDevice, s));
+        }
+    }
+    for (size_t i = 0; i < passes.size(); ++i) {
+        const VisionPass& vp = passes[i];
+        const int n = (int)vp.idx.size();
+        const FrontLayout f = front_layout((size_t)T, (size_t)B, (size_t)n, (size_t)Q);
+        if (i > 0) {
+            char* gh = (char*)arena_take(m, f.end - f.imgptr) - f.imgptr;
+            fill_vision_front(gh, f, vp, dev_ptr, vision_rows, patches_of(vp), Q);
+            HIPCHK(hipMemcpyAsync((char*)m->w_front.p + f.imgptr, gh + f.imgptr, f.end - f.imgptr, hipMemcpyHostToDevice, s));
+        }
+        view_vision_front(m, f, n, Q);
+        VRCHK(run_vision_group(m, n, vp.H, vp.W, i == 0, s));
     }
     VRCHK(tap_store(m, "inputs_embeds", m->w_h.p, T, E, E, false, s));
 
diff --git a/visrag_amd/csrc/engine_common.h b/visrag_amd/csrc/engine_common.h
--- a/visrag_amd/csrc/engine_common.h
+++ b/visrag_amd/csrc/engine_common.h
@@ -97,6 +97,7 @@
         bytes = 0;
         owned = true;
     }
+    void view(void* q, size_t n) { free(); p = q; bytes = n; owned = false; }
     template <typename T> T* as() const { return reinterpret_cast<T*>(p); }
 };
 
diff --git a/visrag_amd/csrc/hp_text.hip b/visrag_amd/csrc/hp_text.hip
--- a/visrag_amd/csrc/hp_text.hip
+++ b/visrag_amd/csrc/hp_text.hip
@@ -149,8 +149,10 @@
 
 __global__ __launch_bounds__(256) void embed_gather_hp_kernel(const int* __restrict__ ids, const bf16_t* __restrict__ table_hi,
                                                               const bf16_t* __restrict__ table_lo, int dim, float scale,
-                                                              float* __restrict__ out) {
+                                                              float* __restrict__ out, int T, const int* __restrict__ seq_offsets,
+                                                              int* __restrict__ pos) {
     const int t = blockIdx.x;
+    if (t >= T) { iota_pos_block(seq_offsets, t - T, pos); return; }
     const size_t off = (size_t)ids[t] * dim;
     float* dst = out + (size_t)t * dim;
     for (int c = threadIdx.x * 4; c < dim; c += 1024) {
@@ -164,11 +166,11 @@
 }
 
 hipError_t launch_embed_gather_hp(const int* ids, int T, const void* table_hi, const void* table_lo, int dim, float scale,
-                                  float* out, hipStream_t s) {
-    if (T <= 0) return hipSuccess;
-    if (dim % 4) return hipErrorInvalidValue;
-    hipLaunchKernelGGL(embed_gather_hp_kernel, dim3(T), dim3(256), 0, s, ids, (const bf16_t*)table_hi, (const bf16_t*)table_lo,
-                       dim, scale, out);
+                                  float* out, hipStream_t s, const int* seq_offsets, int B, int* pos) {
+    if (T <= 0) return hipSuccess;
+    if (dim % 4 || (pos && (!seq_offsets || B <= 0))) return hipErrorInvalidValue;
+    hipLaunchKernelGGL(embed_gather_hp_kernel, dim3(T + (pos ? B : 0)), dim3(256), 0, s, ids, (const bf16_t*)table_hi, (const bf16_t*)table_lo,
+                       dim, scale, out, T, seq_offsets, pos);
     return hipGetLastError();
 }
 
diff --git a/visrag_amd/csrc/index.hip b/visrag_amd/csrc/index.hip
--- a/visrag_amd/csrc/index.hip
+++ b/visrag_amd/csrc/index.hip
@@ -77,9 +77,8 @@
     VRCHK(set_dev(ix->device));
     hipStream_t s = (hipStream_t)stream;
     float* dst = ix->f32.as<float>() + (size_t)ix->n * ix->dim;
-    HIPCHK(hipMemcpyAsync(dst, reps, (size_t)n * ix->dim * 4, on_device ? hipMemcpyDeviceToDevice : hipMemcpyHostToDevice, s));
-    HIPCHK(launch_f32_to_bf16(dst, (char*)ix->bf16.p + (size_t)ix->n * ix->dim * 2, (size_t)n * ix->dim, s));
-    HIPCHK(launch_row_norm_max(dst, n, ix->dim, ix->cert.as<float>(), s));
+    if (!on_device) HIPCHK(hipMemcpyAsync(dst, reps, (size_t)n * ix->dim * 4, hipMemcpyHostToDevice, s));
+    HIPCHK(launch_index_add_rows(on_device ? reps : dst, dst, (char*)ix->bf16.p + (size_t)ix->n * ix->dim * 2, n, ix->dim, ix->cert.as<float>(), s));
     if (!on_device) HIPCHK(hipStreamSynchronize(s));
     ix->n += n;
     return VR_OK;
diff --git a/visrag_amd/csrc/kernels.h b/visrag_amd/csrc/kernels.h
--- a/visrag_amd/csrc/kernels.h
+++ b/visrag_amd/csrc/kernels.h
@@ -163,14 +163,14 @@
 hipError_t launch_patch_embed(const uint8_t* const* imgs, int n_imgs, int H, int W, int P, const GemmArgs& g, int Kreal,
                               hipStream_t s);
 hipError_t launch_embed_gather(const int* ids, int T, const void* table, int dim, float scale,
-                               float* out, hipStream_t s);
+                               float* out, hipStream_t s, const int* seq_offsets = nullptr, int B = 0, int* pos = nullptr);
 hipError_t launch_pool(const float* h, const int* seq_offsets, int B, int dim, const float* norm_w,
                        float eps, float* out, float* tap_hidden, hipStream_t s, int mode = 0);
 hipError_t launch_f32_to_bf16(const float* in, void* out, size_t n, hipStream_t s);
 hipError_t launch_f32_to_bf16_pad(const float* in, void* out, size_t n, size_t n_total, hipStream_t s,
                                   int* zero_word = nullptr);
 hipError_t launch_split_bf16(const float* in, void* hi, void* lo, size_t n, hipStream_t s);
-hipError_t launch_iota_pos(const int* seq_offsets, int B, int* pos, hipStream_t s);
+hipError_t launch_index_add_rows(const float* src, float* dst32, void* dst16, int64_t n, int dim, float* dmax, hipStream_t s);
 hipError_t launch_any_nonzero16(const void* p, size_t n, int* flag, hipStream_t s);
 
 hipError_t launch_rmsnorm_split(const float* x, int rows, int dim, const float* w, float eps, void* hi, void* lo, hipStream_t s);
@@ -179,7 +179,7 @@
                            float scale, float* out, hipStream_t s);
 hipError_t launch_swiglu_split(const float* gu, int T, int ld_gu, int I, int ld_act, void* hi, void* lo, hipStream_t s);
 hipError_t launch_embed_gather_hp(const int* ids, int T, const void* table_hi, const void* table_lo, int dim, float scale,
-                                  float* out, hipStream_t s);
+                                  float* out, hipStream_t s, const int* seq_offsets = nullptr, int B = 0, int* pos = nullptr);
 hipError_t launch_seq_of(const int* seq_offsets, int B, int* seq_of, hipStream_t s);
 hipError_t launch_planes_sum(const float* parts, int n_parts, size_t stride, int ldp, int T, int N, float* out, int ldo, float alpha,
                              bool accumulate, hipStream_t s);
@@ -253,7 +253,6 @@
 hipError_t launch_exact_select(const SearchArgs& a, const float* S, size_t ldS, int sub, int max_slots, hipStream_t s);
 int search_band_max();
 hipError_t launch_band_select(const SearchArgs& a, const float* S, size_t ldS, int sub, int max_slots, hipStream_t s);
-hipError_t launch_row_norm_max(const float* rows, int64_t n, int dim, float* dmax, hipStream_t s);
 float search_default_eps_rel(int dim);
 float search_acc_rel(int dim);
 
diff --git a/visrag_amd/csrc/misc.hip b/visrag_amd/csrc/misc.hip
--- a/visrag_amd/csrc/misc.hip
+++ b/visrag_amd/csrc/misc.hip
@@ -5,8 +5,10 @@
 
 __global__ __launch_bounds__(256) void embed_gather_kernel(const int* __restrict__ ids, int T,
                                                            const bf16_t* __restrict__ table, int dim,
-                                                           float scale, float* __restrict__ out) {
+                                                           float scale, float* __restrict__ out,
+                                                           const int* __restrict__ seq_offsets, int* __restrict__ pos) {
     const int t = blockIdx.x;
+    if (t >= T) { iota_pos_block(seq_offsets, t - T, pos); return; }
     const bf16_t* src = table + (size_t)ids[t] * dim;
     float* dst = out + (size_t)t * dim;
     for (int c = threadIdx.x * 4; c < dim; c += 1024) {
@@ -19,11 +21,11 @@
 }
 
 hipError_t launch_embed_gather(const int* ids, int T, const void* table, int dim, float scale,
-                               float* out, hipStream_t s) {
+                               float* out, hipStream_t s, const int* seq_offsets, int B, int* pos) {
     if (T <= 0) return hipSuccess;
-    if (dim % 4) return hipErrorInvalidValue;
-    hipLaunchKernelGGL(embed_gather_kernel, dim3(T), dim3(256), 0, s, ids, T, (const bf16_t*)table, dim,
-                       scale, out);
+    if (dim % 4 || (pos && (!seq_offsets || B <= 0))) return hipErrorInvalidValue;
+    hipLaunchKernelGGL(embed_gather_kernel, dim3(T + (pos ? B : 0)), dim3(256), 0, s, ids, T, (const bf16_t*)table, dim,
+                       scale, out, seq_offsets, pos);
     return hipGetLastError();
 }
 
@@ -123,6 +125,45 @@
     return hipGetLastError();
 }
 
+__global__ __launch_bounds__(256) void index_add_rows_kernel(const float* src, float* dst32, bf16_t* __restrict__ dst16,
+                                                             int64_t n, int dim, float* __restrict__ dmax) {
+    const int lane = threadIdx.x & 63, wave = threadIdx.x >> 6;
+    const int nv = dim >> 2;
+    float m = 0.f, mr = 0.f;
+    for (int64_t r = (int64_t)blockIdx.x * 4 + wave; r < n; r += (int64_t)gridDim.x * 4) {
+        const f32x4* x = reinterpret_cast<const f32x4*>(src + (size_t)r * dim);
+        f32x4* y = reinterpret_cast<f32x4*>(dst32 + (size_t)r * dim);
+        bf16x4* z = reinterpret_cast<bf16x4*>(dst16 + (size_t)r * dim);
+        float ss = 0.f, rr = 0.f;
+        for (int c = lane; c < nv; c += 64) {
+            const f32x4 v = x[c];
+            bf16x4 b;
+#pragma unroll
+            for (int e = 0; e < 4; ++e) {
+                b[e] = f2bf(v[e]);
+                const float d = v[e] - bf2f(b[e]);
+                ss = __builtin_fmaf(v[e], v[e], ss);
+                rr = __builtin_fmaf(d, d, rr);
+            }
+            if (y != x) y[c] = v;
+            z[c] = b;
+        }
+        m = fmaxf(m, wave_sum(ss));
+        mr = fmaxf(mr, wave_sum(rr));
+    }
+    if (lane == 0 && m > 0.f) atomicMax(reinterpret_cast<unsigned*>(dmax), __float_as_uint(sqrtf(m) * 1.00001f));
+    if (lane == 0 && mr > 0.f) atomicMax(reinterpret_cast<unsigned*>(dmax) + 1, __float_as_uint(sqrtf(mr) * 1.00001f));
+}
+
+hipError_t launch_index_add_rows(const float* src, float* dst32, void* dst16, int64_t n, int dim, float* dmax, hipStream_t s) {
+    if (n <= 0) return hipSuccess;
+    if (dim % 4) return hipErrorInvalidValue;
+    const int64_t nb4 = (n + 3) / 4;
+    const int blocks = (int)(nb4 < 2048 ? nb4 : 2048);
+    hipLaunchKernelGGL(index_add_rows_kernel, dim3(blocks), dim3(256), 0, s, src, dst32, (bf16_t*)dst16, n, dim, dmax);
+    return hipGetLastError();
+}
+
 __global__ void f32_to_bf16_pad_kernel(const float* __restrict__ in, bf16_t* __restrict__ out, size_t n, size_t n_total,
                                        int* __restrict__ zero_word) {
     if (zero_word && blockIdx.x == 0 && threadIdx.x < 2) zero_word[threadIdx.x] = 0;
@@ -166,18 +207,6 @@
     return hipGetLastError();
 }
 
-__global__ void iota_pos_kernel(const int* __restrict__ seq_offsets, int* __restrict__ pos) {
-    const int b = blockIdx.x;
-    const int t0 = seq_offsets[b], L = seq_offsets[b + 1] - t0;
-    for (int t = threadIdx.x; t < L; t += blockDim.x) pos[t0 + t] = t;
-}
-
-hipError_t launch_iota_pos(const int* seq_offsets, int B, int* pos, hipStream_t s) {
-    if (B <= 0) return hipSuccess;
-    hipLaunchKernelGGL(iota_pos_kernel, dim3(B), dim3(256), 0, s, seq_offsets, pos);
-    return hipGetLastError();
-}
-
 __global__ void any_nonzero16_kernel(const uint16_t* __restrict__ p, size_t n, int* __restrict__ flag) {
     int any = 0;
     for (size_t i = (size_t)blockIdx.x * blockDim.x + threadIdx.x; i < n; i += (size_t)gridDim.x * blockDim.x)
diff --git a/visrag_amd/csrc/model.h b/visrag_amd/csrc/model.h
--- a/visrag_amd/csrc/model.h
+++ b/visrag_amd/csrc/model.h
@@ -58,33 +58,50 @@
     int prof_level = 0;
     struct ProfClass { std::vector<hipEvent_t> ev; size_t used = 0; double ms = 0, flops = 0; int64_t launches = 0; };
     ProfClass prof[VR_PROF_CLASSES];
-    char* arena = nullptr; size_t arena_cap = 0, arena_used = 0;
-    hipEvent_t arena_ev = nullptr; bool arena_pending = false, arena_open = false;
+    DevBuf w_front;
+    struct ArenaHalf { char* base = nullptr; size_t cap = 0; hipEvent_t ev = nullptr; bool pending = false; };
+    ArenaHalf arena[2];
+    int arena_cur = 0; size_t arena_used = 0; bool arena_open = false;
 };
 
+static inline size_t front_align(size_t n) { return (n + 63) / 64 * 64; }
+struct FrontLayout { size_t seq, imgptr, cu, rowmap, end; };
+static inline FrontLayout front_layout(size_t T, size_t B, size_t n, size_t Q) {
+    FrontLayout f;
+    f.seq = front_align(T * 4);
+    f.imgptr = f.seq + front_align((B + 1) * 4);
+    f.cu = f.imgptr + front_align(n * 8);
+    f.rowmap = f.cu + front_align(2 * (n + 1) * 4);
+    f.end = f.rowmap + front_align(n * Q * 4);
+    return f;
+}
+
 static inline int arena_begin(vr_model_s* m, size_t need) {
-    if (m->arena_pending) { HIPCHK(hipEventSynchronize(m->arena_ev)); m->arena_pending = false; }
-    if (!m->arena_ev) HIPCHK(hipEventCreateWithFlags(&m->arena_ev, hipEventDisableTiming));
-    if (m->arena_cap < need) {
-        if (m->arena) (void)hipHostFree(m->arena);
-        m->arena = nullptr; m->arena_cap = 0;
+    m->arena_cur ^= 1;
+    vr_model_s::ArenaHalf& h = m->arena[m->arena_cur];
+    if (h.pending) { HIPCHK(hipEventSynchronize(h.ev)); h.pending = false; }
+    if (!h.ev) HIPCHK(hipEventCreateWithFlags(&h.ev, hipEventDisableTiming));
+    if (h.cap < need) {
+        if (h.base) (void)hipHostFree(h.base);
+        h.base = nullptr; h.cap = 0;
         const size_t cap = std::max(need, (size_t)4 << 20);
-        HIPCHK(hipHostMalloc((void**)&m->arena, cap, hipHostMallocDefault));
-        m->arena_cap = cap;
+        HIPCHK(hipHostMalloc((void**)&h.base, cap, hipHostMallocDefault));
+        h.cap = cap;
     }
     m->arena_used = 0;
     m->arena_open = true;
     return VR_OK;
 }
 static inline void arena_close(vr_model_s* m, void* stream) {
-    if (m->arena_open && m->arena_ev) {
-        if (hipEventRecord(m->arena_ev, (hipStream_t)stream) == hipSuccess) m->arena_pending = true;
+    vr_model_s::ArenaHalf& h = m->arena[m->arena_cur];
+    if (m->arena_open && h.ev) {
+        if (hipEventRecord(h.ev, (hipStream_t)stream) == hipSuccess) h.pending = true;
         else (void)hipStreamSynchronize((hipStream_t)stream);
     }
     m->arena_open = false;
 }
 static inline void* arena_take(vr_model_s* m, size_t bytes) {
-    void* p = m->arena + m->arena_used;
+    void* p = m->arena[m->arena_cur].base + m->arena_used;
     m->arena_used += (bytes + 63) / 64 * 64;
     return p;
 }
diff --git a/visrag_amd/csrc/model.hip b/visrag_amd/csrc/model.hip
--- a/visrag_amd/csrc/model.hip
+++ b/visrag_amd/csrc/model.hip
@@ -59,8 +59,11 @@
     }
     for (auto& g : m->grids) { g.second.vit_pos.free(); g.second.pos_k.free(); }
     for (auto& pc : m->prof) for (hipEvent_t e : pc.ev) (void)hipEventDestroy(e);
-    if (m->arena) (void)hipHostFree(m->arena);
-    if (m->arena_ev) (void)hipEventDestroy(m->arena_ev);
+    for (auto& h : m->arena) {
+        if (h.base) (void)hipHostFree(h.base);
+        if (h.ev) (void)hipEventDestroy(h.ev);
+    }
+    m->w_front.free();
     for (DevBuf* b : {&m->w_hvit, &m->w_xn, &m->w_qkv, &m->w_att, &m->w_mlp,
                       &m->w_kv32, &m->w_xkv, &m->w_KV, &m->w_ratt, &m->w_rout, &m->w_rln, &m->w_h, &m->w_dxn, &m->w_part, &m->w_dqkv,
                       &m->w_datt, &m->w_dact, &m->w_cu, &m->w_ids, &m->w_seq, &m->w_pos, &m->w_rowmap, &m->w_imgptr,
@@ -325,12 +328,8 @@
     VRCHK(m->w_dqkv.alloc((size_t)T * 3 * E * 2));
     VRCHK(m->w_datt.alloc((size_t)T * E * 2));
     VRCHK(m->w_dact.alloc((size_t)T * m->Ip * 2));
-    VRCHK(m->w_cu.alloc((size_t)(c.max_images + c.max_seqs + 8) * 2 * 4));
-    VRCHK(m->w_ids.alloc((size_t)T * 4));
-    VRCHK(m->w_seq.alloc((size_t)(c.max_seqs + 1) * 4));
+    VRCHK(m->w_front.alloc(front_layout((size_t)T, (size_t)c.max_seqs, (size_t)c.max_images, (size_t)m->Q).end));
     VRCHK(m->w_pos.alloc((size_t)T * 4));
-    VRCHK(m->w_rowmap.alloc((size_t)R * 4));
-    VRCHK(m->w_imgptr.alloc((size_t)c.max_images * 8));
     VRCHK(m->w_out.alloc((size_t)c.max_seqs * E * 4));
     if (c.text_split_precision) {
         const int Kmax = std::max(E, m->Ip);
@@ -534,7 +533,9 @@
     m->taps.clear(); m->taps_on = false;
     m->prof_on = false;
     for (auto& pc : m->prof) { pc.ev.clear(); pc.used = 0; pc.ms = 0; pc.flops = 0; pc.launches = 0; }
-    m->arena = nullptr; m->arena_cap = 0; m->arena_used = 0; m->arena_ev = nullptr; m->arena_pending = false; m->arena_open = false;
+    m->w_front.free();
+    for (auto& h : m->arena) h = vr_model_s::ArenaHalf{};
+    m->arena_cur = 0; m->arena_used = 0; m->arena_open = false;
     const int r = alloc_workspace(m);
     if (r != VR_OK) { (void)vr_model_destroy(m); return r; }
     *out = m;
diff --git a/visrag_amd/csrc/patch_embed.hip b/visrag_amd/csrc/patch_embed.hip
--- a/visrag_amd/csrc/patch_embed.hip
+++ b/visrag_amd/csrc/patch_embed.hip
@@ -1,8 +1,12 @@
 #include "gemm_core.h"
-#include "gemm_epilogue.h"
 #include "kernels.h"
 
 namespace vr {
+
+constexpr int PE_BM = 64;
+constexpr int PE_ATILE_BYTES = PE_BM * GEMM_BK * 2;
+constexpr int PE_WSTAGES = 4;
+constexpr int PE_MAX_LDS = 160 * 1024;
 
 struct PatchArgs {
     const uint8_t* const* imgs;
@@ -11,75 +15,195 @@
     int Kreal;
 };
 
+struct PieceRaw { uint32_t w0, w1, w2; };
+__device__ __forceinline__ PieceRaw piece_load(const uint8_t* p, int n) {
+    const uintptr_t a = (uintptr_t)p;
+    const __attribute__((address_space(1))) uint32_t* q = (const __attribute__((address_space(1))) uint32_t*)(a & ~(uintptr_t)3);
+    const int last = (int)(a & 3) + n - 1;
+    PieceRaw r;
+    r.w0 = q[0];
+    r.w1 = q[last >= 4 ? 1 : 0];
+    r.w2 = q[last >= 8 ? 2 : 0];
+    return r;
+}
+__device__ __forceinline__ uint64_t piece_bytes(const PieceRaw& r, const uint8_t* p) {
+    const int sh = (int)((uintptr_t)p & 3) * 8;
+    const uint64_t lo = ((uint64_t)r.w1 << 32) | r.w0;
+    return sh ? (lo >> sh) | ((uint64_t)r.w2 << (64 - sh)) : lo;
+}
+
+typedef f32x4 pe_acc_t[2][4];
+__device__ __forceinline__ void pe_compute_tile(pe_acc_t& acc, const char* tA, const char* tW, int wm, int wn, int lane) {
+    const int fr = lane & 15, fq = lane >> 4;
+#pragma unroll
+    for (int kk = 0; kk < 2; ++kk) {
+        bf16x8 a[2], w[4];
+#pragma unroll
+        for (int i = 0; i < 2; ++i) {
+            const int row = wm * 32 + i * 16 + fr;
+            a[i] = *reinterpret_cast<const bf16x8*>(tA + row * 128 + (((kk * 4 + fq) ^ (row & 7)) << 4));
+        }
+#pragma unroll
+        for (int j = 0; j < 4; ++j) {
+            const int row = wn * 64 + j * 16 + fr;
+            w[j] = *reinterpret_cast<const bf16x8*>(tW + row * 128 + (((kk * 4 + fq) ^ (row & 7)) << 4));
+        }
+#pragma unroll
+        for (int i = 0; i < 2; ++i)
+#pragma unroll
+            for (int j = 0; j < 4; ++j)
+                acc[i][j] = __builtin_amdgcn_mfma_f32_16x16x32_bf16(w[j], a[i], acc[i][j], 0, 0, 0);
+    }
+}
+
+template <int N>
+__device__ __forceinline__ void pe_wait_vm_barrier() { asm volatile("s_waitcnt vmcnt(%0)\n\ts_barrier" ::"n"(N) : "memory"); }
+
+template <bool BIAS, bool POS>
 __global__ __launch_bounds__(256) void patch_embed_kernel(PatchArgs a) {
     extern __shared__ __attribute__((aligned(16))) char smem[];
     const GemmArgs& p = a.g;
     const int tiles_n = p.N / GEMM_BN;
-    const int tiles_m = (p.M + GEMM_BM - 1) / GEMM_BM;
-    const int t = xcd_remap(blockIdx.x, tiles_m * tiles_n);
-    const int m0 = (t / tiles_n) * GEMM_BM, n0 = (t % tiles_n) * GEMM_BN;
+    const int nk = p.K / GEMM_BK;
+    const int m0 = blockIdx.x * PE_BM;
     const int tid = threadIdx.x, lane = tid & 63, wave = tid >> 6;
     const int wm = wave >> 1, wn = wave & 1;
     const int rowbytes = a.W * 3, seg = a.P * 3;
-
-    const int kc = tid & 7;
-    const uint8_t* pbase[4];
-    bool rok[4];
-#pragma unroll
-    for (int i = 0; i < 4; ++i) {
-        const int row = (tid >> 3) + 32 * i;
-        const int m = min(m0 + row, p.M - 1);
-        rok[i] = m0 + row < p.M;
-        const int img = m / a.N, pp = m % a.N;
-        const int py = pp / a.gw, px = pp % a.gw;
-        pbase[i] = a.imgs[img] + (size_t)(py * a.P) * rowbytes + px * seg;
-    }
-    uint8_t px8[4][8];
-    auto load_pixels = [&](int k0) {
-#pragma unroll
-        for (int e = 0; e < 8; ++e) {
-            const int k = k0 + kc * 8 + e;
-            const int kk = min(k, a.Kreal - 1);
-            const int off = (kk / seg) * rowbytes + (kk % seg);
-#pragma unroll
-            for (int i = 0; i < 4; ++i) px8[i][e] = pbase[i][off];
-        }
-    };
-    auto write_tile = [&](char* tile, int k0) {
-#pragma unroll
-        for (int i = 0; i < 4; ++i) {
-            const int row = (tid >> 3) + 32 * i;
-            bf16x8 v;
-#pragma unroll
-            for (int e = 0; e < 8; ++e) {
-                const float f = ((float)px8[i][e] / 255.0f - 0.5f) / 0.5f;
-                v[e] = (rok[i] && k0 + kc * 8 + e < a.Kreal) ? f2bf(f) : (bf16_t)0.f;
+    char* const panel = smem;
+    char* const wbuf = smem + nk * PE_ATILE_BYTES;
+    const bf16_t* Wp = (const bf16_t*)p.W;
+
+    for (int t = 0; t < PE_WSTAGES - 1; ++t) stage_glds(Wp, p.ldw, 0, t * GEMM_BK, wbuf + t * GEMM_TILE_BYTES, wave, lane);
+
+    {
+        const int kc = tid & 7;
+        const uint8_t* pbase[2];
+        bool rok[2];
+#pragma unroll
+        for (int h = 0; h < 2; ++h) {
+            const int row = (tid >> 3) + 32 * h;
+            const int m = min(m0 + row, p.M - 1);
+            rok[h] = m0 + row < p.M;
+            const int img = m / a.N, pp = m % a.N;
+            const int py = pp / a.gw, px = pp % a.gw;
+            pbase[h] = a.imgs[img] + (size_t)(py * a.P) * rowbytes + px * seg;
+        }
+        for (int kt0 = 0; kt0 < nk; kt0 += 2) {
+            PieceRaw raw[2][2][2];
+            const uint8_t* src[2][2][2];
+            int n1[2], nv[2];
+#pragma unroll
+            for (int u = 0; u < 2; ++u) {
+                const int k = min(kt0 + u, nk - 1) * GEMM_BK + kc * 8;
+                nv[u] = max(0, min(8, a.Kreal - k));
+                const int kk = min(k, a.Kreal - 1);
+                const int ky = kk / seg, off = kk % seg;
+                n1[u] = max(1, min(nv[u], seg - off));
+                const int n2 = nv[u] - n1[u];
+                const size_t o1 = (size_t)ky * rowbytes + off;
+                const size_t o2 = n2 > 0 ? (size_t)(ky + 1) * rowbytes : o1;
+#pragma unroll
+                for (int h = 0; h < 2; ++h) {
+                    src[u][h][0] = pbase[h] + o1;
+                    src[u][h][1] = pbase[h] + o2;
+                    raw[u][h][0] = piece_load(src[u][h][0], n1[u]);
+                    raw[u][h][1] = piece_load(src[u][h][1], max(1, n2));
+                }
             }
-            *reinterpret_cast<bf16x8*>(tile + row * 128 + ((kc ^ (row & 7)) << 4)) = v;
-        }
-    };
-
-    gemm_acc_t acc;
-    gemm_zero(acc);
-    const bf16_t* Wp = (const bf16_t*)p.W;
-    const int nk = p.K / GEMM_BK;
-    load_pixels(0);
-    stage_glds(Wp, p.ldw, n0, 0, smem + GEMM_TILE_BYTES, wave, lane);
-    write_tile(smem, 0);
-    for (int kt = 0; kt < nk; ++kt) {
-        char* cur = smem + (kt & 1) * 2 * GEMM_TILE_BYTES;
-        char* nxt = smem + ((kt + 1) & 1) * 2 * GEMM_TILE_BYTES;
-        __syncthreads();
-        if (kt + 1 < nk) {
-            load_pixels((kt + 1) * GEMM_BK);
-            stage_glds(Wp, p.ldw, n0, (kt + 1) * GEMM_BK, nxt + GEMM_TILE_BYTES, wave, lane);
-        }
-        gemm_compute_tile(acc, cur, cur + GEMM_TILE_BYTES, wm, wn, lane);
-        if (kt + 1 < nk) write_tile(nxt, (kt + 1) * GEMM_BK);
-    }
-#pragma unroll
-    for (int i = 0; i < 4; ++i)
-        gemm_epilogue_row<EPI_F32>(acc[i], p, m0 + wm * 64 + i * 16 + (lane & 15), n0 + wn * 64, lane >> 4);
+#pragma unroll
+            for (int u = 0; u < 2; ++u) {
+                if (kt0 + u >= nk) break;
+                char* tile = panel + (kt0 + u) * PE_ATILE_BYTES;
+#pragma unroll
+                for (int h = 0; h < 2; ++h) {
+                    const int row = (tid >> 3) + 32 * h;
+                    uint64_t b = piece_bytes(raw[u][h][0], src[u][h][0]);
+                    if (n1[u] < 8) b = (b & ((1ull << (8 * n1[u])) - 1)) | (piece_bytes(raw[u][h][1], src[u][h][1]) << (8 * n1[u]));
+                    bf16x8 v;
+#pragma unroll
+                    for (int e = 0; e < 8; ++e) {
+                        const float f = ((float)(uint8_t)(b >> (8 * e)) / 255.0f - 0.5f) / 0.5f;
+                        v[e] = (rok[h] && e < nv[u]) ? f2bf(f) : (bf16_t)0.f;
+                    }
+                    *reinterpret_cast<bf16x8*>(tile + row * 128 + ((kc ^ (row & 7)) << 4)) = v;
+                }
+            }
+        }
+    }
+
+    const int fr = lane & 15, fq = lane >> 4;
+    int erow[2];
+    const float* rbrow[2] = {nullptr, nullptr};
+#pragma unroll
+    for (int i = 0; i < 2; ++i) {
+        erow[i] = m0 + wm * 32 + i * 16 + fr;
+        const int mc = min(erow[i], p.M - 1);
+        if constexpr (POS) rbrow[i] = p.rowbias + (size_t)(mc % p.rowbias_period) * p.rowbias_ld;
+    }
+    __syncthreads();
+    pe_acc_t acc;
+    f32x4 bias[4], rbv[2][4];
+    constexpr int EPI_LOADS = (BIAS ? 4 : 0) + (POS ? 8 : 0);
+    const int steps = tiles_n * nk;
+    int kt = 0, n0 = 0;
+    int pkt = PE_WSTAGES - 1, pn0 = 0;
+    for (int s = 0; s < steps; ++s) {
+        char* cur = wbuf + (s % PE_WSTAGES) * GEMM_TILE_BYTES;
+        if (s + 2 >= steps) {
+            if (s + 1 < steps) VR_WAIT_VM_BARRIER(4);
+            else VR_WAIT_VM_BARRIER(0);
+        } else if (kt == 1 || kt == 2) {
+            pe_wait_vm_barrier<8 + EPI_LOADS>();
+        } else {
+            VR_WAIT_VM_BARRIER(8);
+        }
+        if (kt == 0) {
+#pragma unroll
+            for (int i = 0; i < 2; ++i)
+#pragma unroll
+                for (int j = 0; j < 4; ++j) acc[i][j] = f32x4{0.f, 0.f, 0.f, 0.f};
+#pragma unroll
+            for (int j = 0; j < 4; ++j) {
+                const int n = n0 + wn * 64 + j * 16 + fq * 4;
+                if constexpr (BIAS) bias[j] = *reinterpret_cast<const f32x4*>(p.bias + n);
+                if constexpr (POS) {
+#pragma unroll
+                    for (int i = 0; i < 2; ++i) rbv[i][j] = *reinterpret_cast<const f32x4*>(rbrow[i] + min(n, p.rowbias_cols - 4));
+                }
+            }
+        }
+        if (s + PE_WSTAGES - 1 < steps) {
+            stage_glds(Wp, p.ldw, pn0, pkt * GEMM_BK, wbuf + ((s + PE_WSTAGES - 1) % PE_WSTAGES) * GEMM_TILE_BYTES, wave, lane);
+            if (++pkt == nk) { pkt = 0; pn0 += GEMM_BN; }
+        }
+        const bool last = kt + 1 == nk;
+        pe_compute_tile(acc, panel + kt * PE_ATILE_BYTES, cur, wm, wn, lane);
+        if (last) {
+#pragma unroll
+            for (int i = 0; i < 2; ++i)
+#pragma unroll
+                for (int j = 0; j < 4; ++j) {
+                    f32x4 v = acc[i][j];
+                    if constexpr (BIAS) v += bias[j];
+                    if constexpr (POS) {
+                        const f32x4 t = v + rbv[i][j];
+                        v = n0 + wn * 64 + j * 16 + fq * 4 < p.rowbias_cols ? t : v;
+                    }
+                    acc[i][j] = v;
+                }
+#pragma unroll
+            for (int i = 0; i < 2; ++i)
+                if (erow[i] < p.M) {
+                    float* orow = (float*)p.out + (size_t)erow[i] * p.ldo + n0 + wn * 64 + fq * 4;
+#pragma unroll
+                    for (int j = 0; j < 4; ++j) *reinterpret_cast<f32x4*>(orow + j * 16) = acc[i][j];
+                }
+            kt = 0;
+            n0 += GEMM_BN;
+        } else {
+            ++kt;
+        }
+    }
 }
 
 hipError_t launch_patch_embed(const uint8_t* const* imgs, int n_imgs, int H, int W, int P, const GemmArgs& g, int Kreal,
@@ -87,12 +211,19 @@
     if (n_imgs <= 0) return hipSuccess;
     if (H % P || W % P || g.N % GEMM_BN || g.K % GEMM_BK || Kreal != 3 * P * P || Kreal > g.K || g.rowmap || g.ksplit > 1)
         return hipErrorInvalidValue;
+    const int lds = (g.K / GEMM_BK) * PE_ATILE_BYTES + PE_WSTAGES * GEMM_TILE_BYTES;
+    if (3 * P < 8 || lds > PE_MAX_LDS || g.K / GEMM_BK < 4) return hipErrorInvalidValue;
     PatchArgs a{};
     a.imgs = imgs; a.H = H; a.W = W; a.P = P; a.gw = W / P; a.N = (H / P) * (W / P); a.g = g; a.Kreal = Kreal;
-    const int tiles = (g.N / GEMM_BN) * ((g.M + GEMM_BM - 1) / GEMM_BM);
-    static unsigned long long attr = 0;
-    set_max_dynamic_lds((const void*)patch_embed_kernel, GEMM_SMEM_BYTES, attr);
-    hipLaunchKernelGGL(patch_embed_kernel, dim3(tiles), dim3(256), GEMM_SMEM_BYTES, s, a);
+    static unsigned long long attr[4] = {0, 0, 0, 0};
+    auto launch = [&](auto kernel, unsigned long long& done) {
+        set_max_dynamic_lds((const void*)kernel, PE_MAX_LDS, done);
+        hipLaunchKernelGGL(kernel, dim3((g.M + PE_BM - 1) / PE_BM), dim3(256), lds, s, a);
+    };
+    if (g.bias && g.rowbias) launch(patch_embed_kernel<true, true>, attr[3]);
+    else if (g.bias) launch(patch_embed_kernel<true, false>, attr[2]);
+    else if (g.rowbias) launch(patch_embed_kernel<false, true>, attr[1]);
+    else launch(patch_embed_kernel<false, false>, attr[0]);
     return hipGetLastError();
 }
 
diff --git a/visrag_amd/csrc/search_exact.hip b/visrag_amd/csrc/search_exact.hip
--- a/visrag_amd/csrc/search_exact.hip
+++ b/visrag_amd/csrc/search_exact.hip
@@ -76,39 +76,6 @@
     return hipGetLastError();
 }
 
-__global__ __launch_bounds__(256) void row_norm_max_kernel(const float* __restrict__ rows, int64_t n, int dim,
-                                                           float* __restrict__ dmax) {
-    const int lane = threadIdx.x & 63, wave = threadIdx.x >> 6;
-    const int nv = dim >> 2;
-    float m = 0.f, mr = 0.f;
-    for (int64_t r = (int64_t)blockIdx.x * 4 + wave; r < n; r += (int64_t)gridDim.x * 4) {
-        const f32x4* x = reinterpret_cast<const f32x4*>(rows + (size_t)r * dim);
-        float ss = 0.f, rr = 0.f;
-        for (int c = lane; c < nv; c += 64) {
-            const f32x4 v = x[c];
-#pragma unroll
-            for (int e = 0; e < 4; ++e) {
-                const float d = bf16_resid(v[e]);
-                ss = __builtin_fmaf(v[e], v[e], ss);
-                rr = __builtin_fmaf(d, d, rr);
-            }
-        }
-        m = fmaxf(m, wave_sum(ss));
-        mr = fmaxf(mr, wave_sum(rr));
-    }
-    if (lane == 0 && m > 0.f) atomicMax(reinterpret_cast<unsigned*>(dmax), __float_as_uint(sqrtf(m) * 1.00001f));
-    if (lane == 0 && mr > 0.f) atomicMax(reinterpret_cast<unsigned*>(dmax) + 1, __float_as_uint(sqrtf(mr) * 1.00001f));
-}
-
-hipError_t launch_row_norm_max(const float* rows, int64_t n, int dim, float* dmax, hipStream_t s) {
-    if (n <= 0) return hipSuccess;
-    if (dim % 4) return hipErrorInvalidValue;
-    const int64_t nb4 = (n + 3) / 4;
-    const int blocks = (int)(nb4 < 2048 ? nb4 : 2048);
-    hipLaunchKernelGGL(row_norm_max_kernel, dim3(blocks), dim3(256), 0, s, rows, n, dim, dmax);
-    return hipGetLastError();
-}
-
 float search_acc_rel(int dim) { return (float)(2 * dim + 128) * 0x1p-24f; }
 float search_default_eps_rel(int dim) {
     return 0x1p-7f + 0x1p-16f + search_acc_rel(dim) * (1.f + 0x1p-8f) * (1.f + 0x1p-8f);
```

Measured after the change: 715.4 pages/s (median of 6 runs). Within noise of the previous version (+0.2%).
